# AlphacatPlus/VmambaIR

Measured on AMD Instinct MI355X. Metric: images/sec, x4 SR 64->256 training step (fwd+bwd+Adam+EMA), full VmambaIR UNet, higher is better.
Workload: dtype bf16; 1 GPU; BASELINE.json configs[1]: x4 SR 64x64 LQ, MambaSISR6 dim48 [15,1,1,1]+15, bf16 autocast (scan arithmetic f32), batch 8 per GPU; global_batch=8, per_gpu_batch=8, parallelism=dp1, step_launch=hipGraph replay, vendor_conv_solver_search=True, vendor_conv_solver_records=bench_data/miopen, optimizer=Adam 2e-4 (0.9,0.99) + EMA 0.999, loss=L1, rccl_ranks=1, allreduce_overlapped=False, allreduce_buckets=1, allreduce_bytes=0

## Files before the change

include/vmambair_oss.h:

```cpp
#ifndef VMAMBAIR_OSS_H
#define VMAMBAIR_OSS_H

#include <stddef.h>
#include <stdint.h>

#ifdef __cplusplus
extern "C" {
#endif

#define OSS_OK 0
#define OSS_ERR_NULL (-1)
#define OSS_ERR_SHAPE (-2)
#define OSS_ERR_DSTATE (-3)
#define OSS_ERR_WORKSPACE (-4)

#define OSS_MAX_DSTATE 256

typedef enum {
    OSS_F32 = 0, OSS_F16 = 1, OSS_BF16 = 2,
    OSS_F32_BF16X3 = 3
} oss_dtype;

typedef void *oss_stream_t;

// ... 36 lines not shown
    float *dD;
    float *ddelta_bias;
    void *workspace;
    size_t workspace_bytes;
    int dout_row_mod;
    int reserved_;
    int64_t dBC_group_stride;
    void *ddt;
    float *ddt_weight;
    int64_t ddt_batch_stride, ddt_group_stride, ddt_rank_stride;
    int tune_variant, tune_segments;
    int tune_partials, reserved3_;
    const float *finish_dt_weight;
    int finish_dt_rank, reserved4_;
} oss_scan_bwd_params;

int oss_scan_chunk(void);
int oss_scan_num_chunks(int seqlen);

size_t oss_scan_fwd_workspace_bytes(int batch, int dim, int seqlen, int dstate, int n_groups);
size_t oss_scan_lane_state_floats(int batch, int dim, int seqlen, int dstate);
int oss_scan_fwd(const oss_scan_fwd_params *p, oss_dtype io, oss_stream_t stream);

size_t oss_scan_bwd_workspace_bytes(int batch, int dim, int seqlen, int dstate, int n_groups);
int oss_scan_bwd(const oss_scan_bwd_params *p, oss_dtype io, oss_stream_t stream);

int oss_scan_bwd_finish_dt_ok(int seqlen, int dt_rank);

int oss_scan_fused_dt_ok(oss_dtype io, int batch, int D, int C, int R, int dstate, int seqlen);

void oss_scan_set_variant(int fwd_variant, int bwd_variant);
int oss_scan_last_variant(int which );
void oss_scan_set_segments(int fwd_segments, int bwd_segments);
int oss_scan_last_segments(int which );
void oss_scan_set_carry_split(int split);
int oss_scan_last_lane_states(void);

int oss_dwconv3x3_fwd(oss_dtype io, const void *x, const float *weight, const float *bias, void *y, void *pre_silu, int batch,
                      int channels, int height, int width, int64_t x_batch_stride, int64_t x_channel_stride,
                      int64_t y_batch_stride, int64_t y_channel_stride, int flip, oss_stream_t stream);
int oss_dwconv3x3_wgrad(oss_dtype io, const void *x, const void *dy, float *dweight, float *dbias, float *partials,
                        const void *pre_silu, void *dpre, int batch, int channels, int height, int width,
                        int64_t x_batch_stride, int64_t x_channel_stride, int64_t dy_batch_stride, int64_t dy_channel_stride,
                        oss_stream_t stream);

int oss_dwconv3x3_fused_ok(oss_dtype io, int height, int width, int channels_per_workgroup);
int oss_dwconv3x3_silu_fwd(oss_dtype io, const void *x, const float *weight, const float *bias, void *y, int batch, int channels,
                           int height, int width, int64_t x_batch_stride, int64_t x_channel_stride, int64_t y_batch_stride,
                           int64_t y_channel_stride, oss_stream_t stream);
int oss_dwconv3x3_silu_bwd(oss_dtype io, const void *x, const float *weight, const float *bias, const void *dy, void *dx,
                           float *dweight, float *dbias, float *partials, int batch, int channels, int height, int width,
                           int64_t x_batch_stride, int64_t x_channel_stride, int64_t dy_batch_stride, int64_t dy_channel_stride,
                           int64_t dx_batch_stride, int64_t dx_channel_stride, oss_stream_t stream);
int oss_dwgate_fwd_ok(oss_dtype io, int height, int width);

int oss_effn_fwd_ok(oss_dtype io, int channels, int hidden, int height, int width);
int oss_effn_round_weights(oss_dtype io, const float *project_in, const float *dwconv, const float *project_out, void *w_in, float *w_dw,
                           void *w_out, int channels, int hidden, oss_stream_t stream);
int oss_effn_fwd(oss_dtype io, const void *x, const float *norm_weight, const float *norm_bias, const void *w_in, const float *w_dw,
                 const void *w_out, void *out, int batch, int channels, int hidden, int height, int width, int64_t x_batch_stride,
                 int64_t x_channel_stride, int64_t out_batch_stride, int64_t out_channel_stride, float eps, oss_stream_t stream);
int oss_dwgate_fwd(oss_dtype io, const void *t, const float *weight, const float *bias, void *out, int batch, int hidden,
                   int height, int width, int64_t t_batch_stride, int64_t t_channel_stride, int64_t out_batch_stride,
                   int64_t out_channel_stride, oss_stream_t stream);
int oss_dwgate_bwd(oss_dtype io, const void *t, const float *weight, const float *bias, const void *dout, void *dt,
                   float *dweight, float *dbias, float *partials, int batch, int hidden, int height, int width,
                   int64_t t_batch_stride, int64_t t_channel_stride, int64_t dout_batch_stride, int64_t dout_channel_stride,
                   int64_t dt_batch_stride, int64_t dt_channel_stride, oss_stream_t stream);

int oss_dwconv3x3_flat2_ok(oss_dtype io, int height, int width);
int oss_dwconv3x3_silu_flat2_fwd(oss_dtype io, const void *x, const float *weight, const float *bias, void *x2, int batch, int channels,
                                 int height, int width, int64_t x_batch_stride, int64_t x_channel_stride, oss_stream_t stream);
int oss_dwconv3x3_silu_flat2_bwd(oss_dtype io, const void *x, const float *weight, const float *bias, const void *g2, void *dx,
                                 float *dweight, float *dbias, float *partials, int batch, int channels, int height, int width,
                                 int64_t x_batch_stride, int64_t x_channel_stride, int64_t dx_batch_stride, int64_t dx_channel_stride,
                                 oss_stream_t stream);

int oss_conv1x1_fwd(oss_dtype io, const void *x, const float *weight, const float *bias, const void *residual, void *y,
                    int batch, int cout, int cin, int pixels, int64_t x_batch_stride, int64_t x_channel_stride,
                    oss_stream_t stream);
int oss_conv1x1_dgrad(oss_dtype io, const void *dy, const float *weight, void *dx, int batch, int cout, int cin, int pixels,
                      int64_t dy_batch_stride, int64_t dy_channel_stride, oss_stream_t stream);
size_t oss_conv1x1_wgrad_partial_floats(int batch, int cout, int cin, int pixels);
int oss_conv1x1_wg(oss_dtype io, const void *x, const float *weight, const float *bias, void *y, int batch, int cout, int cin,
                   int pixels, int64_t x_batch_stride, int64_t x_channel_stride, int transposed_weight, oss_stream_t stream);
int oss_ln_conv1x1_ok(oss_dtype io, int cout, int cin, int pixels);
int oss_ln_conv1x1_fwd(oss_dtype io, const void *x, const float *ln_weight, const float *ln_bias, float eps, void *n, float *mean,
                       float *rstd, const float *weight, const float *bias, void *y, int batch, int cout, int cin, int pixels,
                       int64_t x_batch_stride, int64_t x_channel_stride, oss_stream_t stream);
int oss_conv1x1_dgrad_ln_bwd_ok(oss_dtype io, int cout, int cin, int pixels, int batch);
size_t oss_conv1x1_dgrad_ln_bwd_partial_floats(int batch, int cin, int pixels);
int oss_conv1x1_dgrad_ln_bwd(oss_dtype io, const void *dy, const float *weight, const void *x, const float *ln_weight, int ln_has_bias,
                             const float *mean, const float *rstd, const void *skip_grad, void *dx, float *dln_weight, float *dln_bias,
                             float *partials, int batch, int cout, int cin, int pixels, int64_t dy_batch_stride,
                             int64_t dy_channel_stride, oss_stream_t stream);
void oss_conv1x1_set_wg(int on, int pixels);
void oss_conv1x1_wgrad_set_tile(int mode);
void oss_conv1x1_wgrad_set_span(int mult);
int oss_conv1x1_wgrad(oss_dtype io, const void *dy, const void *x, float *dweight, float *dbias, float *partials, int batch,
                      int cout, int cin, int pixels, int64_t dy_batch_stride, int64_t dy_channel_stride,
                      int64_t x_batch_stride, int64_t x_channel_stride, oss_stream_t stream);

int oss_cross_scan2(oss_dtype in_type, oss_dtype out_type, const void *x, void *x2, int batch, int D, int height, int width,
                    int64_t x_batch_stride, int64_t x_channel_stride, oss_stream_t stream);
int oss_cross_merge2(oss_dtype io, const void *g2, void *dx, int batch, int D, int height, int width, oss_stream_t stream);
int oss_proj_fwd(oss_dtype io, const void *x2, const float *x_proj_weight, const float *dt_projs_weight, void *xdbl, void *dts,
                 int batch, int D, int C, int R, int seqlen, oss_stream_t stream);
int oss_proj_dgrad(oss_dtype io, const void *ddts, void *dxdbl, const void *du, const float *x_proj_weight,
                   const float *dt_projs_weight, void *dx2, int batch, int D, int C, int R, int seqlen, oss_stream_t stream);
size_t oss_proj_wgrad_partial_floats(int batch, int D, int C, int R, int seqlen);
void oss_proj_set_path(int force_vector_alu);
int oss_proj_rows_optional_ok(oss_dtype io, int batch, int D, int C, int R, int seqlen);
int oss_proj_wgrad(oss_dtype io, const void *x2, const void *xdbl, const void *dxdbl, const void *ddts, float *dx_proj_weight,
                   float *ddt_projs_weight, float *partials, int batch, int D, int C, int R, int seqlen, oss_stream_t stream);

typedef struct {
    int B, L, dc, Rc, Cc, reserved_;
    const float *pooled;
    const float *cin_w, *cin_b;
    const float *Wxc;
    const float *Wdtc;
    const float *dt_bias;
    const float *A_logs;
    const float *Dsc;
    const float *cout_w, *cout_b;
    const float *cn_w, *cn_b;
    float *zt;
    float *dts;
    float *hs;
    float *y;
    float *yc;
    float *stat;
    float *c;
    const float *pool_part;
    int n_part;
    float pool_scale;
} oss_chan_params;
int oss_chan_fwd(const oss_chan_params *p, oss_stream_t stream);
size_t oss_chan_grad_floats(int L, int dc, int Rc, int Cc);
size_t oss_chan_bwd_scratch_floats(int B, int L, int dc, int Rc, int Cc);
int oss_chan_bwd(const oss_chan_params *p, const float *gc, float *dpooled, float *grads, float *scratch, oss_stream_t stream);
int oss_rowsum(oss_dtype io, const void *a, const void *bmul, float *out, int batch, int channels, int pixels,
               int64_t a_batch_stride, int64_t a_channel_stride, int64_t b_batch_stride, int64_t b_channel_stride, float alpha,
               oss_stream_t stream);
int oss_row_affine(oss_dtype io, const void *x, const float *mul, const float *add, void *y, int batch, int channels,
                   int pixels, int64_t x_batch_stride, int64_t x_channel_stride, float alpha, oss_stream_t stream);

int oss_gelu_gate_fwd(oss_dtype io, const void *h, void *out, int batch, size_t half_elems, int64_t h_batch_stride,
                      oss_stream_t stream);
int oss_gelu_gate_bwd(oss_dtype io, const void *h, const void *dout, void *dh, int batch, size_t half_elems,
                      int64_t h_batch_stride, int64_t dout_batch_stride, oss_stream_t stream);

typedef struct {
    const void *src;
    void *dst;
    int64_t stride;
    int j0, n, K, reserved_;
} oss_sum_chunk;
void oss_set_defer_finish(int on);
size_t oss_deferred_chunks(void);
int oss_flush_finishes(void *host_table, void *device_table, size_t capacity_chunks, oss_stream_t stream);
int oss_flush_finishes_n(void *host_table, void *device_table, size_t capacity_chunks, size_t max_chunks, oss_stream_t stream);

void oss_set_defer_wgrad(int on);
size_t oss_deferred_wgrads(void);
size_t oss_deferred_wgrad_table_bytes(void);
// ... 25 lines not shown
                         const void *gate, void *y, float *mean, float *rstd, float *pool_part, int batch, int channels, int pixels,
                         int64_t x_batch_stride, int64_t x_channel_stride, int64_t gate_batch_stride,
                         int64_t gate_channel_stride, float eps, oss_stream_t stream);
int oss_ln_nchw_bwd(oss_dtype x_type, oss_dtype y_type, const void *x, const float *weight, const float *bias,
                    const void *gate, const void *dy, const float *mean, const float *rstd, void *dx, void *dgate,
                    float *dweight, float *dbias, float *partials, const void *skip_grad, int batch, int channels, int pixels,
                    int64_t x_batch_stride, int64_t x_channel_stride, int64_t gate_batch_stride,
                    int64_t gate_channel_stride, int64_t dgate_batch_stride, oss_stream_t stream);
int oss_ln_nchw_bwd_affine(oss_dtype x_type, oss_dtype y_type, const void *x, const float *weight, const float *bias,
                           const void *gate, const void *dy, const float *dy_mul, const float *dy_add, float add_scale,
                           const float *mean, const float *rstd, void *dx, void *dgate, float *dweight, float *dbias, float *partials,
                           const void *skip_grad, int batch, int channels, int pixels, int64_t x_batch_stride,
                           int64_t x_channel_stride, int64_t gate_batch_stride, int64_t gate_channel_stride,
                           int64_t dgate_batch_stride, oss_stream_t stream);

void oss_prof_enable(int on);
void oss_prof_reset(void);
int oss_prof_collect(int which, int variant, oss_dtype io, double *total_ms, long long *launches,
                     double *algorithmic_bytes);
int oss_prof_collect2(int which, int variant, oss_dtype io, double *total_ms, long long *launches, double *algorithmic_bytes,
                      double *own_bytes);

int oss_hbm_copy(const void *src, void *dst, size_t n_bytes, oss_stream_t stream);

int oss_prof_marker(int which, oss_stream_t stream);

const char *oss_scan_build_id(void);

const char *oss_version(void);

int oss_conv3x3_thin_ok(oss_dtype io, int cin, int cout, int height, int width);
int oss_conv3x3_thin_fwd(oss_dtype io, const void *x, const float *weight, const float *bias, void *y, int batch, int cin, int cout,
                         int height, int width, int64_t x_batch_stride, int64_t x_channel_stride, int64_t y_batch_stride,
                         int64_t y_channel_stride, oss_stream_t stream);
int oss_conv3x3_thin_dgrad(oss_dtype io, const void *dy, const float *weight, void *dx, int batch, int cin, int cout, int height,
                           int width, int64_t dy_batch_stride, int64_t dy_channel_stride, int64_t dx_batch_stride,
                           int64_t dx_channel_stride, oss_stream_t stream);
size_t oss_conv3x3_thin_wgrad_partial_floats(int batch, int cin, int cout);
int oss_conv3x3_thin_wgrad(oss_dtype io, const void *x, const void *dy, float *dweight, float *dbias, float *partial, int batch, int cin,
                           int cout, int height, int width, int64_t x_batch_stride, int64_t x_channel_stride, int64_t dy_batch_stride,
                           int64_t dy_channel_stride, oss_stream_t stream);

int oss_conv3x3_dense_ok(oss_dtype io, int cin, int cout, int height, int width);
int oss_conv3x3_dense_fwd(oss_dtype io, const void *x, const float *weight, const float *bias, void *y, int batch, int cin, int cout,
                          int height, int width, int64_t x_batch_stride, int64_t x_channel_stride, int64_t y_batch_stride,
                          int64_t y_channel_stride, oss_stream_t stream);
int oss_conv3x3_dense_dgrad(oss_dtype io, const void *dy, const float *weight, void *dx, int batch, int cin, int cout, int height,
                            int width, int64_t dy_batch_stride, int64_t dy_channel_stride, int64_t dx_batch_stride,
                            int64_t dx_channel_stride, oss_stream_t stream);
size_t oss_conv3x3_dense_wgrad_partial_floats(int batch, int cin, int cout, int height, int width);
int oss_conv3x3_dense_wgrad(oss_dtype io, const void *x, const void *dy, float *dweight, float *dbias, float *partial, int batch, int cin,
                            int cout, int height, int width, int64_t x_batch_stride, int64_t x_channel_stride, int64_t dy_batch_stride,
                            int64_t dy_channel_stride, oss_stream_t stream);

#define OSS_METRIC_QUANTISE 1
#define OSS_METRIC_Y 2
#define OSS_METRIC_REPLICATE 4
int oss_image_metrics_ok(oss_dtype io, int channels, int height, int width, int crop_border, int flags);
size_t oss_image_metrics_partial_doubles(int batch, int channels, int height, int width, int crop_border);
int oss_image_metrics(oss_dtype io, const void *a, const void *b, double *out, double *partials, int batch, int channels,
                      int height, int width, int64_t a_batch_stride, int64_t a_channel_stride, int64_t a_row_stride,
                      int64_t b_batch_stride, int64_t b_channel_stride, int64_t b_row_stride, int crop_border, int flags,
                      oss_stream_t stream);

#define OSS_PAIRS_HFLIP 1
#define OSS_PAIRS_ROT 2
int oss_pairs_philox(const uint32_t *counter, const uint32_t *key, uint32_t *out);
int oss_pairs_ok(int channels, int scale, int patch_h, int patch_w, int batch);
int oss_pairs_draw(const int64_t *table, int n_pairs, int64_t *counter, int *samples, int batch, int patch, int64_t seed, int rank,
                   int world, int flags, oss_stream_t stream);
int oss_pairs_gather(const void *pool, int64_t pool_bytes, const int64_t *table, int n_pairs, const int *samples, float *lq, float *gt,
                     int *clamped, int batch, int channels, int patch_h, int patch_w, int scale, int swap_rb, oss_stream_t stream);

void oss_prof_family_enable(int on);
int oss_prof_family_count(void);
int oss_prof_family(int family, const char **name, const char **kernel_patterns, double *algorithmic_bytes, long long *calls);

#define OSS_FEATURE_FUSED_DT 1
#define OSS_FEATURE_LANE_STATES 2
int oss_scan_features(void);

int oss_f32_matmul_modes(void);

#define OSS_ABI_VERSION 8
int oss_abi_version(void);
size_t oss_abi_struct_bytes(int which);

#ifdef __cplusplus
}
#endif
#endif
```

vmambair_amd/csrc/oss_capi.hip:

```cpp
#include <atomic>
#include <mutex>
#include <vector>
#include <cstring>
#include <algorithm>
#include "oss_device.h"
#include "oss_host.h"

namespace oss {

static std::atomic<int> g_force_fwd{-1}, g_force_bwd{-1};
static std::atomic<int> g_last_fwd{-1}, g_last_bwd{-1};
static std::atomic<int> g_force_fwd_seg{-1}, g_force_bwd_seg{-1};
std::atomic<int> g_last_fwd_segments{1}, g_last_bwd_segments{1}, g_last_bwd_lane_states{0};

int scan_pick_segments(long wgs, int n_chunks, int seg_req, double ovh) {
    if (seg_req == 0 || seg_req == 1 || n_chunks < 2 || wgs <= 0) return 1;
    if (seg_req > 1) return std::min(std::min(seg_req, n_chunks), kMaxSegments);
    if (wgs >= 256) return 1;
    int best = 1;
    double best_cost = (double)n_chunks;
    for (int s = 2; s <= std::min(n_chunks, 16); ++s) {
        const int cps = (n_chunks + s - 1) / s;
        if ((n_chunks + cps - 1) / cps != s) continue;
        const double rounds = (double)((wgs * s + 255) / 256);
// ... 39 lines not shown
static std::vector<unsigned char> g_wgrad_descs;
static std::vector<unsigned> g_wgrad_blocks;
bool defer_wgrad() { return g_defer_wgrad.load() != 0; }
void defer_wgrad_push(const void *desc, size_t bytes, unsigned blocks) {
    std::lock_guard<std::mutex> lk(g_defer_mu);
    const unsigned char *p = reinterpret_cast<const unsigned char *>(desc);
    g_wgrad_descs.insert(g_wgrad_descs.end(), p, p + bytes);
    g_wgrad_blocks.push_back(blocks);
}

int scan_fwd_pick_variant(int batch, int dim, int seqlen, int dstate, int n_groups, int elem_bytes) {
    (void)dstate; (void)elem_bytes;
    const int rows_per_group = dim / n_groups;
    const long rows = (long)batch * dim;
    if (seqlen <= 256 || rows_per_group < 8) return (rows_per_group >= 16 && rows >= 4096) ? 2 : 4;
    if (rows_per_group % 16 == 0 && rows / 4 >= 2048) return 2;
    if (rows_per_group % 16 == 0 && rows / 2 >= 2048) return 1;
    if (seqlen >= 4096 && rows_per_group % 12 == 0 && (long)batch * n_groups * (rows_per_group / 12) <= 128) return 6;
    if (seqlen >= 1024 && (long)batch * n_groups * ((rows_per_group + 7) / 8) <= 256) return 3;
    if (seqlen >= 1024 && rows_per_group >= 12 && (long)batch * n_groups * ((rows_per_group + 11) / 12) <= 256) return 6;
    return 0;
}

int scan_bwd_pick_variant(int batch, int dim, int seqlen, int dstate, int n_groups) {
    const int rows_per_group = dim / n_groups;
    if (seqlen <= 256 || rows_per_group < 8 || dstate > 64) return 1;
    const long wgs = (long)batch * n_groups * ((rows_per_group + 7) / 8);
    if (seqlen >= 2048 && rows_per_group % 12 == 0 && (long)batch * n_groups * (rows_per_group / 12) < 192) return 10;
    if (wgs <= 128 && rows_per_group % 4 == 0) return 13;
    if (wgs <= 256) return 11;
    return rows_per_group >= 12 ? 10 : 11;
}

constexpr int kProfVariants = 32;
struct ProfBucket {
    std::vector<std::pair<hipEvent_t, hipEvent_t>> pending;
    double ms = 0.0, bytes = 0.0, own = 0.0;
    long long launches = 0;
};
static std::mutex g_prof_mu;
static std::atomic<int> g_prof_on{0};
static ProfBucket g_prof[3][kProfVariants][3];
static std::vector<hipEvent_t> g_event_pool;

static hipEvent_t prof_event() {
    if (!g_event_pool.empty()) { hipEvent_t e = g_event_pool.back(); g_event_pool.pop_back(); return e; }
    hipEvent_t e; (void)hipEventCreate(&e); return e;
}

struct ProfTimer : LaunchTimer {
    bool on; int which, variant, io; double bytes, own; hipEvent_t e0{}, e1{};
    ProfTimer(int which_, int variant_, int io_, double bytes_, double own_ = 0.0)
        : on(g_prof_on.load() != 0 && variant_ >= 0 && variant_ < 16), which(which_), variant(variant_),
          io(io_), bytes(bytes_), own(own_) {}
    void segmented() override { if (variant < 16) variant += 16; }
    void begin(hipStream_t s) override {
        if (!on) return;
        {
            std::lock_guard<std::mutex> lk(g_prof_mu);
            e0 = prof_event(); e1 = prof_event();
        }
        (void)hipEventRecord(e0, s);
    }
    void end(hipStream_t s) override {
        if (!on) return;
        (void)hipEventRecord(e1, s);
        std::lock_guard<std::mutex> lk(g_prof_mu);
        ProfBucket &b = g_prof[which][variant][io];
        b.pending.emplace_back(e0, e1);
        b.bytes += bytes;
        b.own += own;
        b.launches += 1;
    }
};


enum Fam { FAM_CONV1X1 = 0, FAM_WGRAD, FAM_DWCONV, FAM_PROJ, FAM_LN, FAM_CHAN, FAM_MERGE, FAM_GATE, FAM_CONV3X3, FAM_FINISH, FAM_OPTIM, FAM_N };
static const char *const kFamName[FAM_N] = {"conv1x1 forward / input gradient (+ fused LayerNorm)", "1x1 / projection weight gradients",
                                            "depth-wise 3x3 (+ silu / gelu gate / flattenings)", "x_proj / dt_proj forward + input gradient",
                                            "LayerNorm (+ silu gate, pooled sums)", "channel branch (+ rowsum / row_affine)",
                                            "cross-scan / cross-merge / merge4", "gelu gate (unfused)", "thin 3x3 convolutions",
                                            "deferred partial-sum finishing", "Adam(W) + EMA"};
static const char *const kFamKernels[FAM_N] = {"oss_conv1x1_pair_kernel|oss_conv1x1_pairk_kernel|oss_conv1x1_pairw_kernel|oss_conv1x1_wg_kernel|"
                                               "oss_conv1x1_dgrad_lnbwd_kernel|oss_conv1x1_f32_kernel",
                                               "oss_conv1x1_wgrad|oss_rows_f32_wgrad|oss_proj_wgrad",
                                               "oss_dwconv3x3|oss_dwgate|oss_effn",
                                               "oss_proj_fwd|oss_proj_dgrad|oss_dt_fwd|oss_dt_dgrad|oss_proj_valu",
                                               "oss_ln_nchw",
                                               "oss_chan_|oss_rowsum|oss_row_affine",
                                               "oss_merge4|oss_cross_scan2|oss_cross_merge2",
                                               "oss_gelu_gate",
                                               "oss_conv3x3_",
                                               "oss_sum_partials",
                                               "oss_adam"};
static std::atomic<int> g_fam_on{0};
static double g_fam_bytes[FAM_N];
static long long g_fam_calls[FAM_N];
static inline bool is_f32_split(oss_dtype io) { return io == OSS_F32_BF16X3; }
static inline int take_f32_split(oss_dtype &io) {
    if (!is_f32_split(io)) return 0;
    io = OSS_F32;
    return 1;
}
static inline void fam_count(int fam, double bytes) {
    if (!g_fam_on.load(std::memory_order_relaxed)) return;
    std::lock_guard<std::mutex> lk(g_prof_mu);
    g_fam_bytes[fam] += bytes;
    g_fam_calls[fam] += 1;
}

static double fwd_alg_bytes(const oss_scan_fwd_params &p, int s) {
    const double BKL = (double)p.batch * p.dim * p.seqlen, BGNL = (double)p.batch * p.n_groups * p.dstate * p.seqlen;
    const double xb = 4.0 * p.batch * p.dim * oss_scan_num_chunks(p.seqlen) * 2 * p.dstate;
    return s * (3.0 * BKL + 2.0 * BGNL) + 4.0 * ((double)p.dim * p.dstate + 2.0 * p.dim) + xb;
}
static double bwd_alg_bytes(const oss_scan_fwd_params &p, int s) {
    const double BKL = (double)p.batch * p.dim * p.seqlen, BGNL = (double)p.batch * p.n_groups * p.dstate * p.seqlen;
    const double xb = 4.0 * p.batch * p.dim * oss_scan_num_chunks(p.seqlen) * 2 * p.dstate;
    return s * (5.0 * BKL + 4.0 * BGNL) + 4.0 * (2.0 * p.dim * p.dstate + 4.0 * p.dim) + xb;
}

static double fwd_own_bytes(const oss_scan_fwd_params &p, int s) {
    const double full = fwd_alg_bytes(p, s);
    if (p.u_row_mod <= 0) return full;
    return full - (double)s * p.batch * (p.dim - p.u_row_mod) * p.seqlen;
}
static double bwd_own_bytes(const oss_scan_bwd_params &q, int s) {
    const oss_scan_fwd_params &p = q.f;
    double v = bwd_alg_bytes(p, s);
    if (p.u_row_mod > 0) v -= (double)s * p.batch * (p.dim - p.u_row_mod) * p.seqlen;
    if (q.dout_row_mod > 0) v -= (double)s * p.batch * (p.dim - q.dout_row_mod) * p.seqlen;
    return v;
}

static int check_fwd(const oss_scan_fwd_params *p) {
    if (!p || !p->u || !p->delta || !p->A || !p->B || !p->C) return OSS_ERR_NULL;
    if (p->dt_weight && (p->dt_rank < 1 || p->dt_rank > kMaxDtRank)) return OSS_ERR_SHAPE;
    if (p->batch < 0 || p->dim <= 0 || p->seqlen < 0 || p->dstate <= 0 || p->n_groups <= 0) return OSS_ERR_SHAPE;
    if (p->dim % p->n_groups != 0) return OSS_ERR_SHAPE;
    if (p->dstate > OSS_MAX_DSTATE) return OSS_ERR_DSTATE;
    if (p->rev_group_start < 0 || p->u_row_mod < 0 || (p->u_row_mod > 0 && p->dim % p->u_row_mod != 0)) return OSS_ERR_SHAPE;
    return OSS_OK;
}

}

using namespace oss;

extern "C" {

int oss_scan_chunk(void) { return kScanChunk; }
int oss_scan_num_chunks(int seqlen) { return seqlen <= 0 ? 0 : (seqlen + kScanChunk - 1) / kScanChunk; }

int oss_scan_fwd(const oss_scan_fwd_params *p, oss_dtype io, oss_stream_t stream) {
    const int eb = io_bytes(io);
    if (!eb) return OSS_ERR_SHAPE;
    int rc = check_fwd(p);
    if (rc != OSS_OK) return rc;
    if (!p->out || !p->x) return OSS_ERR_NULL;
    if (p->batch == 0 || p->seqlen == 0) return OSS_OK;
    int v = p->tune_variant > 0 ? p->tune_variant - 1 : g_force_fwd.load();
    if (v < 0) v = scan_fwd_pick_variant(p->batch, p->dim, p->seqlen, p->dstate, p->n_groups, eb);
    g_last_fwd.store(v);
    g_last_fwd_segments.store(1);
    const int sr = p->tune_segments > 0 ? p->tune_segments : g_force_fwd_seg.load();
    hipStream_t s = reinterpret_cast<hipStream_t>(stream);
    ProfTimer prof(0, v, (int)io, fwd_alg_bytes(*p, eb), fwd_own_bytes(*p, eb));
// ... 114 lines not shown
    fam_count(FAM_DWCONV, (double)batch * channels * height * width * io_bytes(io) * 4.0 + 80.0 * channels);
    if (!x || !weight || !g2 || !dx || !dweight || !partials) return OSS_ERR_NULL;
    if (batch <= 0 || channels <= 0 || height <= 0 || width <= 0 || channels > 65535 || batch > 65535) return OSS_ERR_SHAPE;
    return dwconv3x3_silu_flat2_bwd(io, x, weight, bias, g2, dx, dweight, dbias, partials, batch, channels, height, width, xsb, xsc, dsb,
                                    dsc, reinterpret_cast<hipStream_t>(stream));
}

int oss_effn_fwd_ok(oss_dtype io, int channels, int hidden, int height, int width) {
    return effn_fwd_ok(io, channels, hidden, height, width);
}

int oss_effn_round_weights(oss_dtype io, const float *project_in, const float *dwconv, const float *project_out, void *w_in, float *w_dw,
                           void *w_out, int channels, int hidden, oss_stream_t stream) {
    if (is_f32_split(io)) return OSS_ERR_SHAPE;
    if (!project_in || !dwconv || !project_out || !w_in || !w_dw || !w_out) return OSS_ERR_NULL;
    return effn_round_weights(io, project_in, dwconv, project_out, w_in, w_dw, w_out, channels, hidden, reinterpret_cast<hipStream_t>(stream));
}

int oss_effn_fwd(oss_dtype io, const void *x, const float *norm_weight, const float *norm_bias, const void *w_in, const float *w_dw,
                 const void *w_out, void *out, int batch, int channels, int hidden, int height, int width, int64_t xsb, int64_t xsc,
                 int64_t osb, int64_t osc, float eps, oss_stream_t stream) {
    if (is_f32_split(io)) return OSS_ERR_SHAPE;
    fam_count(FAM_DWCONV, (double)batch * channels * height * width * io_bytes(io) * 3.0 + (double)hidden * (3.0 * channels * io_bytes(io) + 72.0));
    if (!x || !norm_weight || !w_in || !w_dw || !w_out || !out) return OSS_ERR_NULL;
    if (batch <= 0 || channels <= 0 || hidden <= 0 || height <= 0 || width <= 0) return OSS_ERR_SHAPE;
    return effn_fwd(io, x, norm_weight, norm_bias, w_in, w_dw, w_out, out, batch, channels, hidden, height, width, xsb, xsc, osb, osc, eps,
                    reinterpret_cast<hipStream_t>(stream));
}

int oss_dwgate_fwd_ok(oss_dtype io, int height, int width) {
    return dwgate_fwd_ok(io, height, width);
}

int oss_dwgate_fwd(oss_dtype io, const void *t, const float *weight, const float *bias, void *out, int batch, int hidden,
                   int height, int width, int64_t tsb, int64_t tsc, int64_t osb, int64_t osc, oss_stream_t stream) {
    if (is_f32_split(io)) return OSS_ERR_SHAPE;
    fam_count(FAM_DWCONV, (double)batch * hidden * height * width * io_bytes(io) * 3.0 + 80.0 * hidden);
    if (!t || !weight || !out) return OSS_ERR_NULL;
    if (batch <= 0 || hidden <= 0 || height <= 0 || width <= 0 || hidden > 32767 || batch > 65535) return OSS_ERR_SHAPE;
    return dwgate_fwd(io, t, weight, bias, out, batch, hidden, height, width, tsb, tsc, osb, osc, reinterpret_cast<hipStream_t>(stream));
}

int oss_dwgate_bwd(oss_dtype io, const void *t, const float *weight, const float *bias, const void *dout, void *dt,
                   float *dweight, float *dbias, float *partials, int batch, int hidden, int height, int width, int64_t tsb,
                   int64_t tsc, int64_t gsb, int64_t gsc, int64_t dsb, int64_t dsc, oss_stream_t stream) {
    if (is_f32_split(io)) return OSS_ERR_SHAPE;
    fam_count(FAM_DWCONV, (double)batch * hidden * height * width * io_bytes(io) * 5.0 + 160.0 * hidden);
    if (!t || !weight || !dout || !dt || !dweight || !partials) return OSS_ERR_NULL;
    if (batch <= 0 || hidden <= 0 || height <= 0 || width <= 0 || hidden > 32767 || batch > 65535) return OSS_ERR_SHAPE;
    return dwconv3x3_bwd_fused(io, 1, t, weight, bias, dout, dt, dweight, dbias, partials, batch, 2 * hidden, height, width, tsb,
                               tsc, gsb, gsc, dsb, dsc, reinterpret_cast<hipStream_t>(stream));
}

int oss_dwconv3x3_wgrad(oss_dtype io, const void *x, const void *dy, float *dweight, float *dbias, float *partials,
                        const void *pre_silu, void *dpre, int batch, int channels, int height, int width, int64_t xsb,
                        int64_t xsc, int64_t gsb, int64_t gsc, oss_stream_t stream) {
    if (is_f32_split(io)) return OSS_ERR_SHAPE;
    fam_count(FAM_DWCONV, (double)batch * channels * height * width * io_bytes(io) * (pre_silu ? 4.0 : 2.0));
    if (!x || !dy || !dweight || !partials) return OSS_ERR_NULL;
    if (batch <= 0 || channels <= 0 || height <= 0 || width <= 0 || batch > 65535) return OSS_ERR_SHAPE;
    return dwconv3x3_wgrad(io, x, dy, dweight, dbias, partials, batch, channels, height, width, xsb, xsc, gsb, gsc,
                           reinterpret_cast<hipStream_t>(stream), pre_silu, dpre);
}

int oss_conv1x1_fwd(oss_dtype io, const void *x, const float *weight, const float *bias, const void *residual, void *y,
                    int batch, int cout, int cin, int pixels, int64_t xsb, int64_t xsc, oss_stream_t stream) {
    const int x3 = take_f32_split(io);
    fam_count(FAM_CONV1X1, (double)batch * pixels * io_bytes(io) * ((double)cin + cout + (residual ? cout : 0)) + 4.0 * cin * cout);
    if (!x || !weight || !y) return OSS_ERR_NULL;
    if (batch <= 0 || cout <= 0 || cin <= 0 || pixels <= 0 || batch > 65535 || cout > 32 * 65535) return OSS_ERR_SHAPE;
    return conv1x1(io, x, weight, bias, y, batch, cout, cin, pixels, xsb, xsc, cin, 1, reinterpret_cast<hipStream_t>(stream),
                   residual, x3);
}

int oss_conv1x1_dgrad(oss_dtype io, const void *dy, const float *weight, void *dx, int batch, int cout, int cin, int pixels,
                      int64_t gsb, int64_t gsc, oss_stream_t stream) {
    const int x3 = take_f32_split(io);
    fam_count(FAM_CONV1X1, (double)batch * pixels * io_bytes(io) * ((double)cin + cout) + 4.0 * cin * cout);
    if (!dy || !weight || !dx) return OSS_ERR_NULL;
    if (batch <= 0 || cout <= 0 || cin <= 0 || pixels <= 0 || batch > 65535) return OSS_ERR_SHAPE;
    return conv1x1(io, dy, weight, nullptr, dx, batch, cin, cout, pixels, gsb, gsc, 1, cin, reinterpret_cast<hipStream_t>(stream), nullptr, x3);
}

size_t oss_conv1x1_wgrad_partial_floats(int batch, int cout, int cin, int pixels) {
    if (batch <= 0 || cout <= 0 || cin <= 0 || pixels <= 0) return 0;
    return (size_t)batch * conv1x1_wgrad_slabs(pixels) * cout * (cin + 1);
}

int oss_conv1x1_wgrad(oss_dtype io, const void *dy, const void *x, float *dweight, float *dbias, float *partials, int batch,
                      int cout, int cin, int pixels, int64_t gsb, int64_t gsc, int64_t xsb, int64_t xsc, oss_stream_t stream) {
    const int x3 = take_f32_split(io);
    fam_count(FAM_WGRAD, (double)batch * pixels * io_bytes(io) * ((double)cin + cout) + 4.0 * cin * cout);
    if (!dy || !x || !dweight || !partials) return OSS_ERR_NULL;
    if (batch <= 0 || cout <= 0 || cin <= 0 || pixels <= 0 || batch > 65535) return OSS_ERR_SHAPE;
    return conv1x1_wgrad(io, dy, x, dweight, partials, batch, cout, cin, pixels, gsb, gsc, xsb, xsc,
                         reinterpret_cast<hipStream_t>(stream), 1, 0, 0, 0, 0, dbias, x3);
}

size_t oss_proj_wgrad_partial_floats(int batch, int D, int C, int R, int seqlen) {
    if (batch <= 0 || D <= 0 || C <= 0 || R <= 0 || seqlen <= 0) return 0;
    const size_t slabs = (size_t)batch * conv1x1_wgrad_slabs(seqlen);
    const size_t a = slabs * 2 * (2 * (size_t)C) * D, b = slabs * 4 * (size_t)D * R;
    return a + b;
}

int oss_proj_fwd(oss_dtype io, const void *x2, const float *x_proj_weight, const float *dt_projs_weight, void *xdbl, void *dts,
                 int batch, int D, int C, int R, int seqlen, oss_stream_t stream) {
    const int x3 = take_f32_split(io);
    fam_count(FAM_PROJ, (double)batch * seqlen * io_bytes(io) * (2.0 * D + 4.0 * C + (dts ? 4.0 * R + 4.0 * D : 0.0)) + 16.0 * C * D + 16.0 * D * R);
    if (!x2 || !x_proj_weight || !dt_projs_weight || !xdbl) return OSS_ERR_NULL;
    if (batch <= 0 || D <= 0 || seqlen <= 0 || R <= 0 || C <= R) return OSS_ERR_SHAPE;
    return proj_fwd(io, x2, x_proj_weight, dt_projs_weight, xdbl, dts, batch, D, C, R, seqlen, reinterpret_cast<hipStream_t>(stream), x3);
}

int oss_proj_dgrad(oss_dtype io, const void *ddts, void *dxdbl, const void *du, const float *x_proj_weight,
                   const float *dt_projs_weight, void *dx2, int batch, int D, int C, int R, int seqlen, oss_stream_t stream) {
    const int x3 = take_f32_split(io);
    fam_count(FAM_PROJ, (double)batch * seqlen * io_bytes(io) * ((ddts ? 4.0 * D + 4.0 * R : 0.0) + 4.0 * C + (du ? 4.0 * D : 0.0) + 2.0 * D) + 16.0 * C * D);
    if (!dxdbl || !x_proj_weight || !dt_projs_weight || !dx2) return OSS_ERR_NULL;
    if (batch <= 0 || D <= 0 || seqlen <= 0 || R <= 0 || C <= R) return OSS_ERR_SHAPE;
    return proj_dgrad(io, ddts, dxdbl, du, x_proj_weight, dt_projs_weight, dx2, batch, D, C, R, seqlen,
                      reinterpret_cast<hipStream_t>(stream), x3);
}

void oss_proj_set_path(int force_vector_alu) { proj_force_valu(force_vector_alu); }
int oss_proj_rows_optional_ok(oss_dtype io, int batch, int D, int C, int R, int seqlen) {
    return proj_mfma_ok(io, batch, D, C, R, seqlen) ? 1 : 0;
}
int oss_scan_fused_dt_ok(oss_dtype io, int batch, int D, int C, int R, int dstate, int seqlen) {
    return proj_mfma_ok(io, batch, D, C, R, seqlen) && R >= 1 && R <= kMaxDtRank && dstate <= 64 && seqlen >= 512;
}
int oss_conv1x1_wg(oss_dtype io, const void *x, const float *weight, const float *bias, void *y, int batch, int cout, int cin,
                   int pixels, int64_t xsb, int64_t xsc, int transposed_weight, oss_stream_t stream) {
    if (is_f32_split(io)) return OSS_ERR_SHAPE;
    fam_count(FAM_CONV1X1, (double)batch * pixels * io_bytes(io) * ((double)cin + cout) + 4.0 * cin * cout);
    if (!x || !weight || !y) return OSS_ERR_NULL;
    if (batch <= 0 || batch > 65535) return OSS_ERR_SHAPE;
    return conv1x1_wg(io, x, weight, bias, y, batch, cout, cin, pixels, xsb, xsc, transposed_weight, reinterpret_cast<hipStream_t>(stream));
}

int oss_ln_conv1x1_ok(oss_dtype io, int cout, int cin, int pixels) {
    const void *a = reinterpret_cast<const void *>(uintptr_t(256));
    return conv1x1_wg_ok(io, cout, cin, pixels, (int64_t)cin * pixels, pixels, a, a, reinterpret_cast<const float *>(a), nullptr);
}

int oss_ln_conv1x1_fwd(oss_dtype io, const void *x, const float *ln_weight, const float *ln_bias, float eps, void *n, float *mean,
                       float *rstd, const float *weight, const float *bias, void *y, int batch, int cout, int cin, int pixels,
                       int64_t xsb, int64_t xsc, oss_stream_t stream) {
    if (is_f32_split(io)) return OSS_ERR_SHAPE;
    fam_count(FAM_CONV1X1, (double)batch * pixels * (io_bytes(io) * (2.0 * cin + cout) + 8.0) + 4.0 * cin * cout);
    if (!x || !ln_weight || !n || !mean || !rstd || !weight || !y) return OSS_ERR_NULL;
    if (batch <= 0 || batch > 65535) return OSS_ERR_SHAPE;
    return ln_conv1x1_wg(io, x, ln_weight, ln_bias, eps, n, mean, rstd, weight, bias, y, batch, cout, cin, pixels, xsb, xsc,
                         reinterpret_cast<hipStream_t>(stream));
}

int oss_conv1x1_dgrad_ln_bwd_ok(oss_dtype io, int cout, int cin, int pixels, int batch) {
    return conv1x1_dgrad_lnbwd_ok(io, cin, cout, pixels, batch);
}
size_t oss_conv1x1_dgrad_ln_bwd_partial_floats(int batch, int cin, int pixels) {
    if (batch <= 0 || cin <= 0 || pixels <= 0) return 0;
    return conv1x1_dgrad_lnbwd_partial_floats(batch, cin, pixels);
}
int oss_conv1x1_dgrad_ln_bwd(oss_dtype io, const void *dy, const float *weight, const void *x, const float *ln_weight, int ln_has_bias,
                             const float *mean, const float *rstd, const void *skip_grad, void *dx, float *dln_weight, float *dln_bias,
                             float *partials, int batch, int cout, int cin, int pixels, int64_t gsb, int64_t gsc, oss_stream_t stream) {
    if (is_f32_split(io)) return OSS_ERR_SHAPE;
    fam_count(FAM_CONV1X1, (double)batch * pixels * (io_bytes(io) * ((double)cout + 2.0 * cin + (skip_grad ? cin : 0)) + 8.0) + 4.0 * cin * cout);
    if (!dy || !weight || !x || !ln_weight || !mean || !rstd || !dx || !dln_weight || !partials) return OSS_ERR_NULL;
    if (batch <= 0 || batch > 65535) return OSS_ERR_SHAPE;
    return conv1x1_dgrad_lnbwd(io, dy, weight, x, ln_weight, ln_has_bias, mean, rstd, skip_grad, dx, dln_weight, dln_bias, partials, batch,
                               cin, cout, pixels, gsb, gsc, reinterpret_cast<hipStream_t>(stream));
}

void oss_conv1x1_set_wg(int on, int pixels) { conv1x1_set_wg(on); conv1x1_wg_set_pixels(pixels); }
void oss_conv1x1_wgrad_set_tile(int mode) { conv1x1_wgrad_set_tile(mode); }
void oss_conv1x1_wgrad_set_span(int mult) { conv1x1_wgrad_set_span(mult); }

int oss_proj_wgrad(oss_dtype io, const void *x2, const void *xdbl, const void *dxdbl, const void *ddts, float *dx_proj_weight,
                   float *ddt_projs_weight, float *partials, int batch, int D, int C, int R, int seqlen, oss_stream_t stream) {
    const int x3 = take_f32_split(io);
    fam_count(FAM_WGRAD, (double)batch * seqlen * io_bytes(io) * (2.0 * D + 8.0 * C + (ddts ? 4.0 * D : 0.0)));
    if (!x2 || !xdbl || !dxdbl || !dx_proj_weight || !partials) return OSS_ERR_NULL;
    if (ddts && !ddt_projs_weight) return OSS_ERR_NULL;
    if (batch <= 0 || D <= 0 || seqlen <= 0 || R <= 0 || C <= R) return OSS_ERR_SHAPE;
    hipStream_t s = reinterpret_cast<hipStream_t>(stream);
    const int64_t L = seqlen;
    if (io == OSS_F32) {
        int e = rows_f32_wgrad(reinterpret_cast<const float *>(dxdbl), reinterpret_cast<const float *>(x2), dx_proj_weight, partials, batch,
                               4, 2, C, D, seqlen, 4 * C * L, C * L, L, 2 * D * L, D * L, L, s, nullptr, x3);
        if (e || !ddts) return e;
        float *part2 = partials + (size_t)batch * conv1x1_wgrad_slabs(seqlen) * 2 * (2 * (size_t)C) * D;
        return rows_f32_wgrad(reinterpret_cast<const float *>(ddts), reinterpret_cast<const float *>(xdbl), ddt_projs_weight, part2, batch, 4,
                              4, D, R, seqlen, 4 * D * L, D * L, L, 4 * C * L, C * L, L, s, nullptr, x3);
    }
    int e = conv1x1_wgrad(io, dxdbl, x2, dx_proj_weight, partials, batch, 2 * C, D, seqlen, 4 * C * L, L, 2 * D * L, L, s,
                           2,  C * L,  D * L,  C,  2 * C * L);
    if (e || !ddts) return e;
    float *part2 = partials + (size_t)batch * conv1x1_wgrad_slabs(seqlen) * 2 * (2 * (size_t)C) * D;
    return conv1x1_wgrad(io, ddts, xdbl, ddt_projs_weight, part2, batch, D, R, seqlen, 4 * D * L, L, 4 * C * L, L, s,
                          4,  D * L,  C * L,  D, 0);
}

int oss_cross_scan2(oss_dtype in_type, oss_dtype out_type, const void *x, void *x2, int batch, int D, int height, int width,
                    int64_t x_batch_stride, int64_t x_channel_stride, oss_stream_t stream) {
    if (is_f32_split(in_type) || is_f32_split(out_type)) return OSS_ERR_SHAPE;
    fam_count(FAM_MERGE, (double)batch * D * height * width * (io_bytes(in_type) + 2.0 * io_bytes(out_type)));
    if (!x || !x2) return OSS_ERR_NULL;
    if (batch <= 0 || D <= 0 || height <= 0 || width <= 0) return OSS_ERR_SHAPE;
    return cross_scan2(in_type, out_type, x, x2, batch, D, height, width, x_batch_stride, x_channel_stride,
                       reinterpret_cast<hipStream_t>(stream));
}

int oss_cross_merge2(oss_dtype io, const void *g2, void *dx, int batch, int D, int height, int width, oss_stream_t stream) {
    if (is_f32_split(io)) return OSS_ERR_SHAPE;
    fam_count(FAM_MERGE, (double)batch * D * height * width * io_bytes(io) * 3.0);
    if (!g2 || !dx) return OSS_ERR_NULL;
    if (batch <= 0 || D <= 0 || height <= 0 || width <= 0) return OSS_ERR_SHAPE;
    return cross_merge2(io, g2, dx, batch, D, height, width, reinterpret_cast<hipStream_t>(stream));
}

int oss_chan_fwd(const oss_chan_params *p, oss_stream_t stream) {
    fam_count(FAM_CHAN, p ? 4.0 * p->B * ((double)p->L * (2.0 * p->Cc + 2.0 * p->dc * 18.0 + 3.0) + (p->pool_part ? (double)p->n_part * p->L : p->L)) : 0.0);
    if (!p) return OSS_ERR_NULL;
    return chan_fwd(*p, reinterpret_cast<hipStream_t>(stream));
}

size_t oss_chan_grad_floats(int L, int dc, int Rc, int Cc) { return chan_grad_floats(L, dc, Rc, Cc); }
size_t oss_chan_bwd_scratch_floats(int B, int L, int dc, int Rc, int Cc) { return chan_bwd_scratch_floats(B, L, dc, Rc, Cc); }

int oss_chan_bwd(const oss_chan_params *p, const float *gc, float *dpooled, float *grads, float *scratch, oss_stream_t stream) {
    fam_count(FAM_CHAN, p ? 4.0 * p->B * ((double)p->L * (2.0 * p->Cc + 2.0 * p->dc * 18.0 + 5.0)) : 0.0);
    if (!p) return OSS_ERR_NULL;
    return chan_bwd(*p, gc, dpooled, grads, scratch, reinterpret_cast<hipStream_t>(stream));
}

int oss_rowsum(oss_dtype io, const void *a, const void *bmul, float *out, int batch, int channels, int pixels, int64_t asb,
// ... 393 lines not shown
```

vmambair_amd/csrc/oss_conv1x1.hip:

```cpp
#include <atomic>
#include "oss_device.h"
#include "oss_global_ptr.h"
#include "oss_host.h"
#include "oss_mfma.h"

namespace oss {

template <typename T>
__global__ void __launch_bounds__(256)
oss_conv1x1_kernel(const T *__restrict__ x, const float *__restrict__ w, const float *__restrict__ bias, T *__restrict__ y,
                   int M, int K, int P, int64_t xsb, int64_t xsk, int64_t ws_m, int64_t ws_k, const T *__restrict__ res) {
    const int lane = threadIdx.x & 63, wave = threadIdx.x >> 6;
    const int b = blockIdx.y;
    const int m0 = blockIdx.z * 32;
    const int p0 = (blockIdx.x * 4 + wave) * 32;
    if (p0 >= P) return;
    const int col = lane & 31, kg = lane >> 5;
    const int p = p0 + col;
    const bool pok = p < P;
    const T *xb = x + b * xsb + (pok ? p : 0);
    T *yb = y + (size_t)b * M * P;
    const int mrow = m0 + col;
    const bool mok = mrow < M;
    const float *wrow = w + (mok ? mrow : 0) * ws_m;
// ... 172 lines not shown
        if (row < M && pok) yw[(size_t)row * psw] = pack2<T>(va, vb);
    }
}

template <int KS>
struct WRaw { f32x4 lo[KS], hi[KS]; };

template <int KS, bool WT, bool WVEC>
__device__ __forceinline__ void wraw_issue(WRaw<KS> &r, const float *__restrict__ w, int mrow, int M, int K, int kg) {
    const int mc = mrow < M ? mrow : 0;
#pragma unroll
    for (int ks = 0; ks < KS; ++ks) {
        const int k0 = ks * 16 + kg * 8;
        if constexpr (!WT && WVEC) {
            const float *wp = w + mc * K + (k0 + 8 <= K ? k0 : 0);
            r.lo[ks] = *reinterpret_cast<const f32x4 *>(wp);
            r.hi[ks] = *reinterpret_cast<const f32x4 *>(wp + 4);
        } else {
#pragma unroll
            for (int e = 0; e < 8; ++e) {
                const int k = k0 + e, kc = k < K ? k : K - 1;
                const float v = WT ? w[kc * M + mc] : w[mc * K + kc];
                if (e < 4) r.lo[ks][e] = v; else r.hi[ks][e - 4] = v;
            }
        }
    }
}

template <typename T, int KS, bool WT, bool WVEC>
__device__ __forceinline__ void wraw_narrow(const WRaw<KS> &r, s16x8 (&af)[KS], int mrow, int M, int K, int kg) {
    const bool mok = mrow < M;
#pragma unroll
    for (int ks = 0; ks < KS; ++ks) {
        const int k0 = ks * 16 + kg * 8;
        if constexpr (!WT && WVEC) {
            const s16x8 f = cvt8<T>(r.lo[ks], r.hi[ks]);
            af[ks] = (mok && k0 + 8 <= K) ? f : s16x8{0, 0, 0, 0, 0, 0, 0, 0};
        } else {
            f32x4 lo = r.lo[ks], hi = r.hi[ks];
#pragma unroll
            for (int e = 0; e < 4; ++e) {
                lo[e] = (mok && k0 + e < K) ? lo[e] : 0.f;
                hi[e] = (mok && k0 + 4 + e < K) ? hi[e] : 0.f;
            }
            af[ks] = cvt8<T>(lo, hi);
        }
    }
}

template <int KS>
__device__ __forceinline__ void wflat_issue(WRaw<KS> &r, const float *__restrict__ w, int m0, int M, int K, int lane) {
    const int lim = min(M - m0, 32) * K - 4;
    const float *base = w + (size_t)m0 * K;
#pragma unroll
    for (int i = 0; i < 2 * KS; ++i) {
        const f32x4 q = *reinterpret_cast<const f32x4 *>(base + min(256 * i + 4 * lane, lim));
        if (i < KS) r.lo[i] = q; else r.hi[i - KS] = q;
    }
}
template <typename T, int KS>
__device__ __forceinline__ void wflat_frags(const WRaw<KS> &r, T *__restrict__ myl, s16x8 (&af)[KS], int m0, int M, int K,
                                            int col, int kg, int row0, int k0, int sr, int sk) {
    constexpr int RS = 16 * KS + 8;
    const int nl = K >> 3;
    int rr = row0, kk = k0;
#pragma unroll
    for (int i = 0; i < 2 * KS; ++i) {
        const f32x4 q = i < KS ? r.lo[i] : r.hi[i < KS ? 0 : i - KS];
        if (i < nl) *reinterpret_cast<u32x2 *>(myl + rr * RS + kk) = u32x2{pack2<T>(q.x, q.y), pack2<T>(q.z, q.w)};
        kk += sk;
        rr += sr;
        if (kk >= K) { kk -= K; ++rr; }
    }
    __builtin_amdgcn_wave_barrier();
    const bool mok = m0 + col < M;
#pragma unroll
    for (int ks = 0; ks < KS; ++ks) {
        const u32x4 f = *reinterpret_cast<const u32x4 *>(myl + col * RS + ks * 16 + kg * 8);
        af[ks] = (mok && ks * 16 + kg * 8 + 8 <= K) ? __builtin_bit_cast(s16x8, f) : s16x8{0, 0, 0, 0, 0, 0, 0, 0};
    }
    __builtin_amdgcn_wave_barrier();
}

template <typename T, int KS, bool WT, bool WVEC, bool RES, bool PF>
__global__ void __launch_bounds__(256)
oss_conv1x1_pair_kernel(const T *__restrict__ x, const float *__restrict__ w, const float *__restrict__ bias,
                        T *__restrict__ y, int M, int K, int P, int64_t xsb, int xsk, int mt_per_wave, const T *__restrict__ res) {
    const int lane = threadIdx.x & 63, wave = threadIdx.x >> 6;
    const int b = blockIdx.y;
    const int p0 = (blockIdx.x * 4 + wave) * 64;
    if (p0 >= P) return;
    const int col = lane & 31, kg = lane >> 5;
    const int p = p0 + 2 * col;
    const bool pok = p < P;
    const int pc = pok ? p : 0;
    const uint32_t *xw = reinterpret_cast<const uint32_t *>(x + b * xsb + pc);
    const int xsw = xsk >> 1;
    const int psw = P >> 1;
    uint32_t *yw = reinterpret_cast<uint32_t *>(y + (size_t)b * M * P + pc);
    const uint32_t *rp = RES ? reinterpret_cast<const uint32_t *>(res + (size_t)b * M * P + pc) : nullptr;
    const float *bp = bias ? bias : w;
    const int ksteps = (K + 15) >> 4;
    const int mt_total = (M + 31) >> 5;
    const int mt_begin = blockIdx.z * mt_per_wave, mt_end = min(mt_total, mt_begin + mt_per_wave);
    if (mt_begin >= mt_end) return;

    constexpr bool WLDS = !WT && WVEC;
    __shared__ __attribute__((aligned(16))) T wlds[WLDS ? 4 * 32 * (16 * KS + 8) : 8];
    T *myl = wlds + (WLDS ? wave * 32 * (16 * KS + 8) : 0);
    const int wf_row0 = WLDS ? (4 * lane) / K : 0, wf_k0 = WLDS ? (4 * lane) % K : 0, wf_sr = WLDS ? 256 / K : 0, wf_sk = WLDS ? 256 % K : 0;
    WRaw<KS> wr;
    float bl;
    uint32_t rw[16];
    auto issue = [&](int mt) {
        const int m0 = mt * 32;
        if constexpr (WLDS) wflat_issue<KS>(wr, w, m0, M, K, lane);
        else                wraw_issue<KS, WT, WVEC>(wr, w, m0 + col, M, K, kg);
        bl = bp[min(m0 + col, M - 1)];
        if constexpr (RES) {
#pragma unroll
            for (int r = 0; r < 16; ++r) rw[r] = rp[(size_t)min(m0 + (r & 3) + 8 * (r >> 2) + 4 * kg, M - 1) * psw];
        }
    };
    issue(mt_begin);

    s16x8 bfa[KS], bfb[KS];
#pragma unroll
    for (int ks = 0; ks < KS; ++ks) {
#pragma unroll
        for (int e = 0; e < 8; ++e) {
            const int k = ks * 16 + kg * 8 + e;
            const bool kok = k < K;
            const uint32_t raw = xw[(kok ? k : K - 1) * xsw];
            const uint32_t v = (pok && kok) ? raw : 0u;
            bfa[ks][e] = (short)(v & 0xffffu);
            bfb[ks][e] = (short)(v >> 16);
        }
    }

    for (int mt = mt_begin; mt < mt_end; ++mt) {
        const int m0 = mt * 32;
        s16x8 af[KS];
        if constexpr (WLDS) wflat_frags<T, KS>(wr, myl, af, m0, M, K, col, kg, wf_row0, wf_k0, wf_sr, wf_sk);
        else                wraw_narrow<T, KS, WT, WVEC>(wr, af, m0 + col, M, K, kg);
        const float bcur = bias ? bl : 0.f;
        uint32_t rcur[16];
        if constexpr (RES) {
#pragma unroll
            for (int r = 0; r < 16; ++r) rcur[r] = rw[r];
        }
        if constexpr (PF) issue(min(mt + 1, mt_total - 1));
        f32x16 acca, accb;
#pragma unroll
        for (int r = 0; r < 16; ++r) { acca[r] = 0.f; accb[r] = 0.f; }
#pragma unroll
        for (int ks = 0; ks < KS; ++ks) {
            if (ks < ksteps) {
                acca = Mfma<T>::run(af[ks], bfa[ks], acca);
                accb = Mfma<T>::run(af[ks], bfb[ks], accb);
            }
        }
#pragma unroll
        for (int r = 0; r < 16; ++r) {
            const int rin = (r & 3) + 8 * (r >> 2) + 4 * kg, row = m0 + rin;
            const float bv = __int_as_float(__builtin_amdgcn_ds_bpermute(rin << 2, __float_as_int(bcur)));
            float va = acca[r] + bv, vb = accb[r] + bv;
            if constexpr (RES) {
                float r0, r1;
                unpack2<T>(rcur[r], r0, r1);
                va += r0;
                vb += r1;
            }
            if (row < M && pok) yw[(size_t)row * psw] = pack2<T>(va, vb);
        }
        if constexpr (!PF) {
            if (mt + 1 < mt_end) issue(mt + 1);
        }
    }
}

template <typename T>
__global__ void __launch_bounds__(256)
oss_conv1x1_pairw_kernel(const T *__restrict__ x, const float *__restrict__ w, const float *__restrict__ bias,
                         T *__restrict__ y, int M, int K, int P, int64_t xsb, int xsk, const T *__restrict__ res) {
    constexpr int KS = 8, CH = KS * 16, KMAX = 512, NI = 32 * KMAX / 4 / 256;
    __shared__ __attribute__((aligned(16))) T wl[32 * (KMAX + 8)];
    const int tid = threadIdx.x, lane = tid & 63, wave = tid >> 6;
    const int b = blockIdx.y;
    const int p0 = (blockIdx.x * 4 + wave) * 64;
    const bool active = p0 < P;
    const int col = lane & 31, kg = lane >> 5;
    const int p = p0 + 2 * col;
    const bool pok = active && p < P;
    const uint32_t *xw = reinterpret_cast<const uint32_t *>(x + b * xsb + (pok ? p : 0));
    const int xsw = xsk >> 1;
    const int m0 = blockIdx.z * 32;
    const int RS = ((K + 7) & ~7) + 8;

    auto load_x = [&](int kc, s16x8 (&fa)[KS], s16x8 (&fb)[KS]) {
#pragma unroll
        for (int ks = 0; ks < KS; ++ks) {
#pragma unroll
            for (int e = 0; e < 8; ++e) {
                const int k = kc + ks * 16 + kg * 8 + e;
                const bool kok = k < K;
                const uint32_t raw = xw[(kok ? k : K - 1) * xsw];
                const uint32_t v = (pok && kok) ? raw : 0u;
                fa[ks][e] = (short)(v & 0xffffu);
                fb[ks][e] = (short)(v >> 16);
            }
        }
    };
    s16x8 fa[KS], fb[KS];
    load_x(0, fa, fb);

    const int have = min(M - m0, 32) * K, total = 32 * K, lim = max(have - 4, 0);
    const float *base = w + (size_t)m0 * K;
    f32x4 q[NI];
#pragma unroll
    for (int i = 0; i < NI; ++i) q[i] = *reinterpret_cast<const f32x4 *>(base + min(4 * (i * 256 + tid), lim));
    int r = (4 * tid) / K, k = (4 * tid) - r * K;
    const int sr = 1024 / K, sk = 1024 - sr * K;
#pragma unroll
    for (int i = 0; i < NI; ++i) {
        const int off = 4 * (i * 256 + tid);
        if (off < total) {
            const int d = max(off - lim, 0);
            float v4[4] = {q[i][0], q[i][1], q[i][2], q[i][3]};
            if (d == 1) { v4[0] = v4[1]; v4[1] = v4[2]; v4[2] = v4[3]; }
            else if (d == 2) { v4[0] = v4[2]; v4[1] = v4[3]; }
            else if (d >= 3) { v4[0] = v4[3]; }
            int rr = r, kk = k;
#pragma unroll
            for (int e = 0; e < 4; ++e) {
                if (rr < 32 && off + e < have) wl[rr * RS + kk] = from_f32<T>(v4[e]);
                if (++kk == K) { kk = 0; ++rr; }
            }
        }
        k += sk;
        r += sr;
        if (k >= K) { k -= K; ++r; }
    }
    __syncthreads();
    if (!active) return;

    f32x16 acca, accb;
#pragma unroll
    for (int r = 0; r < 16; ++r) { acca[r] = 0.f; accb[r] = 0.f; }
    const bool mok = m0 + col < M;
    for (int kc = 0; kc < K; kc += CH) {
        if (kc) load_x(kc, fa, fb);
        s16x8 af[KS];
#pragma unroll
        for (int ks = 0; ks < KS; ++ks) {
            const int k0 = kc + ks * 16 + kg * 8;
            const u32x4 f = *reinterpret_cast<const u32x4 *>(wl + col * RS + min(k0, RS - 8));
            s16x8 v = __builtin_bit_cast(s16x8, f);
#pragma unroll
            for (int e = 0; e < 8; ++e) v[e] = (mok && k0 + e < K) ? v[e] : (short)0;
            af[ks] = v;
        }
#pragma unroll
        for (int ks = 0; ks < KS; ++ks) {
            if (kc + ks * 16 < K) {
                acca = Mfma<T>::run(af[ks], fa[ks], acca);
                accb = Mfma<T>::run(af[ks], fb[ks], accb);
            }
        }
    }
    T *yb = y + (size_t)b * M * P;
    pair_epilogue<T>(acca, accb, bias, res ? res + (size_t)b * M * P + (pok ? p : 0) : nullptr, yb + p, m0, kg, M, P, pok);
}

template <typename T, int KS, int MT, bool WT, bool WVEC>
__global__ void __launch_bounds__(256)
oss_conv1x1_pairk_kernel(const T *__restrict__ x, const float *__restrict__ w, const float *__restrict__ bias,
                        T *__restrict__ y, int M, int K, int P, int64_t xsb, int xsk, const T *__restrict__ res) {
    const int lane = threadIdx.x & 63, wave = threadIdx.x >> 6;
    const int b = blockIdx.y;
    const int p0 = (blockIdx.x * 4 + wave) * 64;
    if (p0 >= P) return;
    const int col = lane & 31, kg = lane >> 5;
    const int p = p0 + 2 * col;
    const bool pok = p < P;
    const uint32_t *xw = reinterpret_cast<const uint32_t *>(x + b * xsb + (pok ? p : 0));
    const int xsw = xsk >> 1;
    T *yb = y + (size_t)b * M * P;
    const int mt0 = blockIdx.z * MT;
    f32x16 acca[MT], accb[MT];
#pragma unroll
    for (int t = 0; t < MT; ++t)
#pragma unroll
        for (int r = 0; r < 16; ++r) { acca[t][r] = 0.f; accb[t][r] = 0.f; }

    for (int kc = 0; kc < K; kc += KS * 16) {
        s16x8 bfa[KS], bfb[KS];
#pragma unroll
        for (int ks = 0; ks < KS; ++ks) {
#pragma unroll
            for (int e = 0; e < 8; ++e) {
                const int k = kc + ks * 16 + kg * 8 + e;
                const bool kok = k < K;
                const uint32_t raw = xw[(kok ? k : K - 1) * xsw];
                const uint32_t v = (pok && kok) ? raw : 0u;
                bfa[ks][e] = (short)(v & 0xffffu);
                bfb[ks][e] = (short)(v >> 16);
            }
        }
#pragma unroll
        for (int t = 0; t < MT; ++t) {
            s16x8 af[KS];
#pragma unroll
            for (int ks = 0; ks < KS; ++ks) af[ks] = load_wfrag<T, WT, WVEC>(w, (mt0 + t) * 32 + col, M, K, kc + ks * 16 + kg * 8);
            if ((mt0 + t) * 32 < M) {
#pragma unroll
                for (int ks = 0; ks < KS; ++ks) {
                    if (kc + ks * 16 < K) {
                        acca[t] = Mfma<T>::run(af[ks], bfa[ks], acca[t]);
                        accb[t] = Mfma<T>::run(af[ks], bfb[ks], accb[t]);
                    }
                }
            }
        }
    }
#pragma unroll
    for (int t = 0; t < MT; ++t)
        pair_epilogue<T>(acca[t], accb[t], bias, res ? res + (size_t)b * M * P + (pok ? p : 0) : nullptr, yb + p, (mt0 + t) * 32, kg, M, P, pok);
}

constexpr int kWgradSlab = 512;
template <typename T>
__device__ __forceinline__ void
wgrad_body(const T *__restrict__ dy, const T *__restrict__ x, float *__restrict__ part, int M, int N, int P,
           int64_t gsb, int64_t gsm, int64_t xsb, int64_t xsn, int G, int64_t gsg, int64_t xsg, int Mh,
           int64_t gs_hi, int NB ,
           int slab, int nslabs, int by, int bz, int span ) {
    const int lane = threadIdx.x & 63, wave = threadIdx.x >> 6;
    const int b = by / G, g = by - b * G;
    const int pbeg = slab * span, pend = min(P, pbeg + span);
    const int col = lane & 31, kg = lane >> 5;
    const int mt = (M + 31) >> 5, nt = (NB + 31) >> 5;
    const T *gb = dy + b * gsb + g * gsg;
    const T *xb = x + b * xsb + g * xsg;
    const size_t pvec = (size_t)G * M * N + (NB > N ? M : 0);
    float *pb = part + (size_t)(b * nslabs + slab) * pvec;
    const short kOne = (short)from_f32<T>(1.0f).v;
    const s16x8 zero8 = {0, 0, 0, 0, 0, 0, 0, 0}, ones8 = {kOne, kOne, kOne, kOne, kOne, kOne, kOne, kOne};
    const bool aligned = (((reinterpret_cast<uintptr_t>(gb) | reinterpret_cast<uintptr_t>(xb)) & 15u) == 0) &&
                         (gsm % 8 == 0) && (xsn % 8 == 0) && (pbeg % 8 == 0) && (gs_hi % 8 == 0);
    {
        const int tile = bz * 4 + wave;
        if (tile >= mt * nt) return;
        const int m0 = (tile / nt) * 32, n0 = (tile % nt) * 32;
        const int mrow = m0 + col, nrow = n0 + col;
        const bool mok = mrow < M, nok = nrow < N, one = nrow == N && NB > N;
        const int mr = mok ? mrow : 0;
        const T *ga = gb + (mr / Mh) * gs_hi + (mr % Mh) * gsm;
        const T *xa = xb + (nok ? nrow : 0) * xsn;
        f32x16 acc;
#pragma unroll
        for (int r = 0; r < 16; ++r) acc[r] = 0.f;

        int pk = pbeg;
        for (; aligned && pend - pk >= kWgradSlab; pk += kWgradSlab) {
            constexpr int PIECES = kWgradSlab / 64, RS = 72;
            __shared__ __attribute__((aligned(16))) T stage[4][2][32 * RS];
            T *sa = stage[wave][0], *sb = stage[wave][1];
            const int r8 = lane >> 3, q = lane & 7;
            const T *pa[4], *px[4];
#pragma unroll
            for (int j = 0; j < 4; ++j) {
                const int mr2 = min(m0 + r8 + 8 * j, M - 1), nr2 = min(n0 + r8 + 8 * j, N - 1);
                pa[j] = gb + (mr2 / Mh) * gs_hi + (mr2 % Mh) * gsm + pk + q * 8;
                px[j] = xb + nr2 * xsn + pk + q * 8;
            }
            constexpr int WIN = PIECES < 4 ? PIECES : 4;
            u32x4 qa[WIN][4], qb[WIN][4];
#pragma unroll
            for (int pc = 0; pc < WIN; ++pc)
#pragma unroll
                for (int j = 0; j < 4; ++j) {
                    qa[pc][j] = *reinterpret_cast<const u32x4 *>(pa[j] + pc * 64);
                    qb[pc][j] = *reinterpret_cast<const u32x4 *>(px[j] + pc * 64);
                }
#pragma unroll
            for (int pc = 0; pc < PIECES; ++pc) {
#pragma unroll
                for (int j = 0; j < 4; ++j) {
                    *reinterpret_cast<u32x4 *>(sa + (r8 + 8 * j) * RS + q * 8) = qa[pc % WIN][j];
                    *reinterpret_cast<u32x4 *>(sb + (r8 + 8 * j) * RS + q * 8) = qb[pc % WIN][j];
                }
                if (pc + WIN < PIECES) {
#pragma unroll
                    for (int j = 0; j < 4; ++j) {
                        qa[pc % WIN][j] = *reinterpret_cast<const u32x4 *>(pa[j] + (pc + WIN) * 64);
                        qb[pc % WIN][j] = *reinterpret_cast<const u32x4 *>(px[j] + (pc + WIN) * 64);
// ... 49 lines not shown
                    af[e] = (mok && kok) ? av : (short)0;
                    bf[e] = kok ? (nok ? bv : (one ? kOne : (short)0)) : (short)0;
                }
            }
            acc = Mfma<T>::run(af, bf, acc);
        }
#pragma unroll
        for (int r = 0; r < 16; ++r) {
            const int row = m0 + (r & 3) + 8 * (r >> 2) + 4 * kg;
            const int cn = n0 + col;
            if (row < M && cn < NB) {
                const size_t drow = ((size_t)(row / Mh) * G + g) * Mh + row % Mh;
                if (cn < N) pb[drow * N + cn] = acc[r];
                else pb[(size_t)G * M * N + row] = acc[r];
            }
        }
    }
}

template <typename T>
__global__ void __launch_bounds__(256)
oss_conv1x1_wgrad_kernel(const T *__restrict__ dy, const T *__restrict__ x, float *__restrict__ part, int M, int N, int P,
                         int64_t gsb, int64_t gsm, int64_t xsb, int64_t xsn, int G, int64_t gsg, int64_t xsg, int Mh,
                         int64_t gs_hi, int NB) {
    wgrad_body<T>(dy, x, part, M, N, P, gsb, gsm, xsb, xsn, G, gsg, xsg, Mh, gs_hi, NB, (int)blockIdx.x, (int)gridDim.x, (int)blockIdx.y,
                  (int)blockIdx.z, kWgradSlab);
}

struct WgradDesc {
    const void *dy, *x;
    float *part;
    int64_t gsb, gsm, xsb, xsn, gsg, xsg, gs_hi;
    int M, N, P, G, Mh, NB, slabs, bgs ;
    unsigned first_block;
    int io;
    int span, reserved_;
};
template <typename T>
__global__ void __launch_bounds__(256)
oss_conv1x1_wgrad_grouped_kernel(const WgradDesc *__restrict__ descs, const uint16_t *__restrict__ block_problem) {
    const WgradDesc d = descs[block_problem[blockIdx.x]];
    const unsigned local = blockIdx.x - d.first_block;
    const int slab = (int)(local % (unsigned)d.slabs);
    const unsigned r = local / (unsigned)d.slabs;
    const int by = (int)(r % (unsigned)d.bgs), bz = (int)(r / (unsigned)d.bgs);
    const WgradDesc *dt = descs + block_problem[blockIdx.x];
    wgrad_body<T>(table_ptr<const T>(&dt->dy), table_ptr<const T>(&dt->x), table_ptr<float>(&dt->part), d.M, d.N, d.P, d.gsb, d.gsm, d.xsb,
                  d.xsn, d.G, d.gsg, d.xsg, d.Mh, d.gs_hi, d.NB, slab, d.slabs, by, bz, d.span);
}

__global__ void __launch_bounds__(256)
oss_conv1x1_wgrad_finish(const float *__restrict__ part, float *__restrict__ dw, float *__restrict__ db, int nslab, size_t pvec,
                         size_t nw) {
    __shared__ float red[4][64];
    const int colx = threadIdx.x & 63, slice = threadIdx.x >> 6;
    const size_t i = (size_t)blockIdx.x * 64 + colx;
    float s = 0.f;
    if (i < pvec) {
        const float *pp = part + i;
        int k = slice;
        float s0 = 0.f, s1 = 0.f, s2 = 0.f, s3 = 0.f;
        for (; k + 12 < nslab; k += 16) {
            s0 += pp[(size_t)k * pvec];
            s1 += pp[(size_t)(k + 4) * pvec];
            s2 += pp[(size_t)(k + 8) * pvec];
            s3 += pp[(size_t)(k + 12) * pvec];
        }
        for (; k < nslab; k += 4) s0 += pp[(size_t)k * pvec];
        s = (s0 + s1) + (s2 + s3);
    }
    red[slice][colx] = s;
    __syncthreads();
    if (slice == 0 && i < pvec) {
        const float t = (red[0][colx] + red[1][colx]) + (red[2][colx] + red[3][colx]);
        if (i < nw) dw[i] = t;
        else db[i - nw] = t;
    }
}

constexpr long kConv1x1TargetWaves = 1024;

template <typename T>
static void conv1x1_launch(const T *x, const float *w, const float *bias, T *y, int B, int M, int K, int P, int64_t xsb,
                           int64_t xsk, int64_t ws_m, int64_t ws_k, hipStream_t s, const T *res) {
    const int pblocks = (P + 127) / 128, mt = (M + 31) / 32;
    const bool wt = (ws_m == 1 && ws_k == M);
    const bool plain = (ws_k == 1 && ws_m == K);
    const bool pair_ok = P % 2 == 0 && xsk % 2 == 0 && xsb % 2 == 0 && xsk < (1 << 24) && (size_t)M * K < (1u << 30) &&
                         (wt || plain) && ((reinterpret_cast<uintptr_t>(x) | reinterpret_cast<uintptr_t>(y)) & 3u) == 0;
    if (pair_ok) {
        const bool wvec = plain && K % 8 == 0 && (reinterpret_cast<uintptr_t>(w) & 15u) == 0;
        const int pb = (P + 255) / 256;
        const long waves_p = (long)B * ((P + 63) / 64);
        const int xk = (int)xsk;
        if (plain && !wvec && K > 16 * 3 && K <= 512 && (reinterpret_cast<uintptr_t>(w) & 15u) == 0) {
            hipLaunchKernelGGL(oss_conv1x1_pairw_kernel<T>, dim3(pb, B, mt), dim3(256), 0, s, x, w, bias, y, M, K, P, xsb, xk, res);
            return;
        }
        if (K <= 16 * 12) {
            int split = (int)((kConv1x1TargetWaves + waves_p - 1) / waves_p);
            if (split < 1) split = 1;
            if (split > mt) split = mt;
            const int per = (mt + split - 1) / split;
            dim3 grid(pb, B, (mt + per - 1) / per);
#define OSS_PAIR2(KS_, WT_, WV_, PF_) do { if (res) hipLaunchKernelGGL((oss_conv1x1_pair_kernel<T, KS_, WT_, WV_, true, PF_>), grid, dim3(256), 0, s, x, w, bias, y, M, K, P, xsb, xk, per, res); \
                                           else     hipLaunchKernelGGL((oss_conv1x1_pair_kernel<T, KS_, WT_, WV_, false, PF_>), grid, dim3(256), 0, s, x, w, bias, y, M, K, P, xsb, xk, per, res); } while (0)
#define OSS_PAIR(KS_, PF_) do { if (wt) OSS_PAIR2(KS_, true, false, PF_); else if (wvec) OSS_PAIR2(KS_, false, true, PF_); else OSS_PAIR2(KS_, false, false, PF_); } while (0)
            if (K <= 16 * 3)      OSS_PAIR(3, true);
            else if (K <= 16 * 6) OSS_PAIR(6, true);
            else if (K <= 16 * 8) OSS_PAIR(8, false);
            else                  OSS_PAIR(12, false);
#undef OSS_PAIR2
#undef OSS_PAIR
#undef OSS_PAIR1
        } else {
            int per = 3;
            while (per > 1 && waves_p * ((mt + per - 1) / per) < 4096) --per;
            if (per > mt) per = mt;
            if (per == 1 && K <= 512 && (reinterpret_cast<uintptr_t>(w) & 15u) == 0 && plain) {
                hipLaunchKernelGGL(oss_conv1x1_pairw_kernel<T>, dim3(pb, B, mt), dim3(256), 0, s, x, w, bias, y, M, K, P, xsb, xk, res);
                return;
            }
            dim3 grid(pb, B, (mt + per - 1) / per);
#define OSS_PAIR1(MT_, WT_, WV_) hipLaunchKernelGGL((oss_conv1x1_pairk_kernel<T, 8, MT_, WT_, WV_>), grid, dim3(256), 0, s, x, w, bias, y, M, K, P, xsb, xk, res)
#define OSS_PAIR(MT_) do { if (wt) OSS_PAIR1(MT_, true, false); else if (wvec) OSS_PAIR1(MT_, false, true); else OSS_PAIR1(MT_, false, false); } while (0)
            if (per == 1) OSS_PAIR(1); else if (per == 2) OSS_PAIR(2); else OSS_PAIR(3);
#undef OSS_PAIR
#undef OSS_PAIR1
        }
        return;
    }
    const bool reuse_ok = K <= 16 * 12 && xsk < (1 << 24) && (size_t)M * K < (1u << 30) &&
                          (wt || (plain && K % 8 == 0 && (reinterpret_cast<uintptr_t>(w) & 15u) == 0));
    if (reuse_ok) {
        const long waves_p = (long)B * ((P + 31) / 32);
        int split = (int)((2048 + waves_p - 1) / waves_p);
        if (split < 1) split = 1;
        if (split > mt) split = mt;
        const int per = (mt + split - 1) / split;
        dim3 grid(pblocks, B, (mt + per - 1) / per);
        const int xk = (int)xsk;
        if (K <= 16 * 6) {
            if (wt) hipLaunchKernelGGL((oss_conv1x1_reuse_kernel<T, 6, true>), grid, dim3(256), 0, s, x, w, bias, y, M, K, P, xsb, xk, per, res);
            else    hipLaunchKernelGGL((oss_conv1x1_reuse_kernel<T, 6, false>), grid, dim3(256), 0, s, x, w, bias, y, M, K, P, xsb, xk, per, res);
        } else {
            if (wt) hipLaunchKernelGGL((oss_conv1x1_reuse_kernel<T, 12, true>), grid, dim3(256), 0, s, x, w, bias, y, M, K, P, xsb, xk, per, res);
            else    hipLaunchKernelGGL((oss_conv1x1_reuse_kernel<T, 12, false>), grid, dim3(256), 0, s, x, w, bias, y, M, K, P, xsb, xk, per, res);
        }
    } else {
        dim3 grid(pblocks, B, mt);
        hipLaunchKernelGGL(oss_conv1x1_kernel<T>, grid, dim3(256), 0, s, x, w, bias, y, M, K, P, xsb, xsk, ws_m, ws_k, res);
    }
}

static std::atomic<int> g_conv_wg{1};

void conv1x1_set_wg(int on) { g_conv_wg.store(on ? 1 : 0); }

int conv1x1(oss_dtype io, const void *x, const float *w, const float *bias, void *y, int B, int M, int K, int P, int64_t xsb,
            int64_t xsk, int64_t ws_m, int64_t ws_k, hipStream_t s, const void *res, int f32_split) {
    {
        const bool wt = (ws_m == 1 && ws_k == M), plain = (ws_k == 1 && ws_m == K);
        if ((wt || plain) && g_conv_wg.load() != 0 && conv1x1_wg_ok(io, M, K, P, xsb, xsk, x, y, w, res))
            return conv1x1_wg(io, x, w, bias, y, B, M, K, P, xsb, xsk, wt ? 1 : 0, s, res);
    }
    return io_dispatch(io, [&](auto tag) {
        using T = typename decltype(tag)::type;
        const T *xp = reinterpret_cast<const T *>(x), *rp = reinterpret_cast<const T *>(res);
        T *yp = reinterpret_cast<T *>(y);
        if constexpr (sizeof(T) == 4) {
            return conv1x1_f32(xp, w, bias, yp, B, M, K, P, xsb, xsk, ws_m, ws_k, s, rp, f32_split);
        } else {
            conv1x1_launch<T>(xp, w, bias, yp, B, M, K, P, xsb, xsk, ws_m, ws_k, s, rp);
            return (int)hipGetLastError();
        }
    });
}

template <typename T, int TM, int TN>
__global__ void __launch_bounds__(256)
oss_conv1x1_wgrad_tiles_kernel(const T *__restrict__ dy, const T *__restrict__ x, float *__restrict__ part, int M, int N, int P,
                               int64_t gsb, int64_t gsm, int64_t xsb, int64_t xsn, int G, int64_t gsg, int64_t xsg, int Mh,
                               int64_t gs_hi, int NB) {
    const int lane = threadIdx.x & 63, wave = threadIdx.x >> 6;
    const int b = blockIdx.y / G, g = blockIdx.y - b * G, slab = blockIdx.x;
    const int pbeg = slab * kWgradSlab, pend = min(P, pbeg + kWgradSlab);
    const int col = lane & 31, kg = lane >> 5;
    const int mt = (M + 32 * TM - 1) / (32 * TM), nt = (NB + 32 * TN - 1) / (32 * TN);
    const T *gb = dy + b * gsb + g * gsg;
    const T *xb = x + b * xsb + g * xsg;
    const size_t pvec = (size_t)G * M * N + (NB > N ? M : 0);
    float *pb = part + (size_t)(b * gridDim.x + slab) * pvec;
    const short kOne = (short)from_f32<T>(1.0f).v;
    const s16x8 zero8 = {0, 0, 0, 0, 0, 0, 0, 0}, ones8 = {kOne, kOne, kOne, kOne, kOne, kOne, kOne, kOne};
    const bool aligned = (((reinterpret_cast<uintptr_t>(gb) | reinterpret_cast<uintptr_t>(xb)) & 15u) == 0) &&
                         (gsm % 8 == 0) && (xsn % 8 == 0) && (pbeg % 8 == 0) && (gs_hi % 8 == 0);
    const int tile = blockIdx.z * 4 + wave;
    if (tile >= mt * nt) return;
    const int m0 = (tile / nt) * 32 * TM, n0 = (tile % nt) * 32 * TN;
    const T *ga[TM];
    const T *xa[TN];
    bool mok[TM], nok[TN], one[TN];
#pragma unroll
    for (int i = 0; i < TM; ++i) {
        const int mrow = m0 + 32 * i + col;
        mok[i] = mrow < M;
        const int mr = mok[i] ? mrow : 0;
        ga[i] = gb + (mr / Mh) * gs_hi + (mr % Mh) * gsm;
    }
#pragma unroll
    for (int j = 0; j < TN; ++j) {
        const int nrow = n0 + 32 * j + col;
        nok[j] = nrow < N;
        one[j] = nrow == N && NB > N;
        xa[j] = xb + (nok[j] ? nrow : 0) * xsn;
    }
    f32x16 acc[TM][TN];
#pragma unroll
    for (int i = 0; i < TM; ++i)
#pragma unroll
        for (int j = 0; j < TN; ++j)
#pragma unroll
            for (int r = 0; r < 16; ++r) acc[i][j][r] = 0.f;

    auto frag = [&](const T *row, int k0, bool ok, bool ones, bool fast) -> s16x8 {
        if (fast) {
            const u32x4 q = *reinterpret_cast<const u32x4 *>(row + k0);
            return ok ? __builtin_bit_cast(s16x8, q) : (ones ? ones8 : zero8);
        }
        s16x8 f;
#pragma unroll
        for (int e = 0; e < 8; ++e) {
            const bool kok = (k0 + e) < pend;
            const int kc = kok ? k0 + e : pend - 1;
            const short v = (short)row[kc].v;
            f[e] = kok ? (ok ? v : (ones ? kOne : (short)0)) : (short)0;
        }
        return f;
    };
    int pk = pbeg;
    if (aligned && pend - pbeg == kWgradSlab) {
        constexpr int IT = kWgradSlab / 16;
        u32x4 qa[IT][TM], qb[IT][TN];
#pragma unroll
        for (int u = 0; u < IT; ++u) {
#pragma unroll
            for (int i = 0; i < TM; ++i) qa[u][i] = *reinterpret_cast<const u32x4 *>(ga[i] + pbeg + u * 16 + kg * 8);
#pragma unroll
            for (int j = 0; j < TN; ++j) qb[u][j] = *reinterpret_cast<const u32x4 *>(xa[j] + pbeg + u * 16 + kg * 8);
        }
#pragma unroll
        for (int u = 0; u < IT; ++u)
#pragma unroll
            for (int i = 0; i < TM; ++i)
#pragma unroll
                for (int j = 0; j < TN; ++j) {
                    const s16x8 af = mok[i] ? __builtin_bit_cast(s16x8, qa[u][i]) : zero8;
                    const s16x8 bf = nok[j] ? __builtin_bit_cast(s16x8, qb[u][j]) : (one[j] ? ones8 : zero8);
// ... 130 lines not shown
```

vmambair_amd/csrc/oss_conv1x1_wg.hip:

```cpp
#include <algorithm>
#include <atomic>
#include <type_traits>
#include "oss_device.h"
#include "oss_host.h"
#include "oss_mfma.h"

namespace oss {

typedef short s16x4 __attribute__((ext_vector_type(4)));

template <typename T, int K, int PT, int PITCH, int GROUP = 6>
__device__ __forceinline__ void copy_tile_to_lds(const T *__restrict__ src, int64_t xsk, T *__restrict__ dst, int tid) {
    constexpr int CPR = PT / 8, TOTAL = K * CPR, NCP = (TOTAL + 255) / 256;
#pragma unroll
    for (int i0 = 0; i0 < NCP; i0 += GROUP) {
        u32x4 q[GROUP];
#pragma unroll
        for (int i = 0; i < GROUP; ++i) {
            if (i0 + i < NCP) {
                const int idx = min(tid + (i0 + i) * 256, TOTAL - 1);
                const int c = idx / CPR, pc = idx - c * CPR;
                q[i] = *reinterpret_cast<const u32x4 *>(src + c * xsk + 8 * pc);
            }
        }
#pragma unroll
        for (int i = 0; i < GROUP; ++i) {
            if (i0 + i < NCP) {
                const int idx = tid + (i0 + i) * 256;
                const int c = idx / CPR, pc = idx - c * CPR;
                if (TOTAL % 256 == 0 || idx < TOTAL) *reinterpret_cast<u32x4 *>(dst + c * PITCH + 8 * pc) = q[i];
            }
        }
    }
}

template <typename T>
struct WgLnArgs {
    const float *w, *b;
    T *n;
    float *mean, *rstd;
    float eps;
};

template <typename T, int KS, bool WT, int PT, bool RES, bool PF, bool LN>
__global__ void __launch_bounds__(256)
oss_conv1x1_wg_kernel(const T *__restrict__ x, const float *__restrict__ w, const float *__restrict__ bias, T *__restrict__ y,
                      int M, int P, int64_t xsb, int64_t xsk, const T *__restrict__ res, WgLnArgs<T> ln) {
    constexpr int K = 16 * KS, NCT = PT / 32;
    constexpr int PX = PT + 32;
    constexpr bool kPairEpi = !RES && PT == 128;
    constexpr int PITCH = kPairEpi ? PT + 16 : PT + 8;
    using OT = typename std::conditional<RES, float, T>::type;
    extern __shared__ __attribute__((aligned(16))) unsigned char wg_smem[];
    T *xs = reinterpret_cast<T *>(wg_smem);
    OT *os = reinterpret_cast<OT *>(xs + K * PX);
    const int tid = threadIdx.x, lane = tid & 63, wave = tid >> 6;
    const int b = blockIdx.y, p0 = blockIdx.x * PT;
    const T *xb = x + b * xsb + p0;
    const int col = lane & 31, kg = lane >> 5;
    const int mt_total = (M + 31) >> 5;
    struct WRaw { f32x4 lo[KS], hi[KS]; float bl; };
    auto issue = [&](int mt, WRaw &r) {
        const int mrow = min(mt * 32 + col, M - 1);
#pragma unroll
        for (int ks = 0; ks < KS; ++ks) {
            const int k0 = ks * 16 + kg * 8;
            if constexpr (!WT) {
                r.lo[ks] = *reinterpret_cast<const f32x4 *>(w + (size_t)mrow * K + k0);
                r.hi[ks] = *reinterpret_cast<const f32x4 *>(w + (size_t)mrow * K + k0 + 4);
            } else {
#pragma unroll
                for (int e = 0; e < 4; ++e) {
                    r.lo[ks][e] = w[(size_t)(k0 + e) * M + mrow];
                    r.hi[ks][e] = w[(size_t)(k0 + 4 + e) * M + mrow];
                }
            }
        }
        r.bl = bias ? bias[mrow] : 0.f;
    };
    WRaw cur;
    const int nz = gridDim.z, zi = blockIdx.z;
    if (wave * nz + zi < mt_total) issue(wave * nz + zi, cur);
    float *lnw_s = reinterpret_cast<float *>(os + 4 * 32 * PITCH), *lnb_s = lnw_s + K;
    float lnw_r = 0.f, lnb_r = 0.f;
    if constexpr (LN) {
        const int c = min(tid, K - 1);
        lnw_r = ln.w[c];
        lnb_r = ln.b ? ln.b[c] : 0.f;
    }
    constexpr int CPR = PT / 8;
    copy_tile_to_lds<T, K, PT, PX>(xb, xsk, xs, tid);
    if constexpr (LN) {
        if (tid < K) { lnw_s[tid] = lnw_r; lnb_s[tid] = lnb_r; }
    }
    __syncthreads();
    if constexpr (LN) {
        constexpr int QPT = PT / 4, NPART = 256 / QPT, CPT = (K + NPART - 1) / NPART;
        float *red = reinterpret_cast<float *>(os);
        const int quad = tid % QPT, part = tid / QPT, px = 4 * quad;
        float v[CPT][4];
#pragma unroll
        for (int i = 0; i < CPT; ++i) {
            const int c = part + i * NPART;
            if (c < K) {
                const u32x2 q = *reinterpret_cast<const u32x2 *>(xs + c * PX + px);
                unpack2<T>(q.x, v[i][0], v[i][1]); unpack2<T>(q.y, v[i][2], v[i][3]);
            } else {
                v[i][0] = v[i][1] = v[i][2] = v[i][3] = 0.f;
            }
        }
        float sum[4] = {0.f, 0.f, 0.f, 0.f};
#pragma unroll
        for (int i = 0; i < CPT; ++i)
#pragma unroll
            for (int u = 0; u < 4; ++u) sum[u] += v[i][u];
        *reinterpret_cast<f32x4 *>(red + part * PT + px) = f32x4{sum[0], sum[1], sum[2], sum[3]};
        __syncthreads();
        float mu[4] = {0.f, 0.f, 0.f, 0.f};
#pragma unroll
        for (int q = 0; q < NPART; ++q) {
            const f32x4 t = *reinterpret_cast<const f32x4 *>(red + q * PT + px);
            mu[0] += t.x; mu[1] += t.y; mu[2] += t.z; mu[3] += t.w;
        }
#pragma unroll
        for (int u = 0; u < 4; ++u) mu[u] /= (float)K;
        __syncthreads();
        float sq[4] = {0.f, 0.f, 0.f, 0.f};
#pragma unroll
        for (int i = 0; i < CPT; ++i) {
            if (part + i * NPART < K) {
#pragma unroll
                for (int u = 0; u < 4; ++u) { const float d = v[i][u] - mu[u]; sq[u] = __builtin_fmaf(d, d, sq[u]); }
            }
        }
        *reinterpret_cast<f32x4 *>(red + part * PT + px) = f32x4{sq[0], sq[1], sq[2], sq[3]};
        __syncthreads();
        float rstd[4] = {0.f, 0.f, 0.f, 0.f};
#pragma unroll
        for (int q = 0; q < NPART; ++q) {
            const f32x4 t = *reinterpret_cast<const f32x4 *>(red + q * PT + px);
            rstd[0] += t.x; rstd[1] += t.y; rstd[2] += t.z; rstd[3] += t.w;
        }
#pragma unroll
        for (int u = 0; u < 4; ++u) rstd[u] = 1.0f / sqrtf(rstd[u] / (float)K + ln.eps);
        if (part == 0 && zi == 0) {
            *reinterpret_cast<f32x4 *>(ln.mean + (size_t)b * P + p0 + px) = f32x4{mu[0], mu[1], mu[2], mu[3]};
            *reinterpret_cast<f32x4 *>(ln.rstd + (size_t)b * P + p0 + px) = f32x4{rstd[0], rstd[1], rstd[2], rstd[3]};
        }
        const bool with_bias = ln.b != nullptr;
        float mu_c[4];
#pragma unroll
        for (int u = 0; u < 4; ++u) mu_c[u] = with_bias ? mu[u] : 0.f;
#pragma unroll
        for (int i = 0; i < CPT; ++i) {
            const int c = part + i * NPART;
            if (c < K) {
                const float wc = lnw_s[c], bc = lnb_s[c];
                float o[4];
#pragma unroll
                for (int u = 0; u < 4; ++u) o[u] = (v[i][u] - mu_c[u]) * rstd[u] * wc + bc;
                *reinterpret_cast<u32x2 *>(xs + c * PX + px) = u32x2{pack2<T>(o[0], o[1]), pack2<T>(o[2], o[3])};
            }
        }
        __syncthreads();
        T *nb = ln.n + (size_t)b * K * P + p0;
        for (int idx = tid; zi == 0 && idx < K * CPR; idx += 256) {
            const int c = idx / CPR, pc = idx - c * CPR;
            *reinterpret_cast<u32x4 *>(nb + (size_t)c * P + 8 * pc) = *reinterpret_cast<const u32x4 *>(xs + c * PX + 8 * pc);
        }
    }
    const int i16 = lane & 15, g = lane >> 4;
    const int tr_off = (8 * (g >> 1) + (i16 >> 2)) * PX + 16 * (g & 1) + 4 * (i16 & 3);
    OT *ow = os + wave * 32 * PITCH;
    for (int mt = wave * nz + zi; mt < mt_total; mt += 4 * nz) {
        const int m0 = mt * 32;
        WRaw nxt;
        if constexpr (PF) { if (mt + 4 * nz < mt_total) issue(mt + 4 * nz, nxt); }
        f32x16 acc[NCT];
#pragma unroll
        for (int ct = 0; ct < NCT; ++ct)
#pragma unroll
            for (int r = 0; r < 16; ++r) acc[ct][r] = 0.f;
#pragma unroll
        for (int ks = 0; ks < KS; ++ks) {
            const s16x8 af = m0 + col < M ? cvt8<T>(cur.lo[ks], cur.hi[ks]) : s16x8{0, 0, 0, 0, 0, 0, 0, 0};
#pragma unroll
            for (int ct = 0; ct < NCT; ++ct) {
                const T *bp = xs + ks * 16 * PX + ct * 32 + tr_off;
                const s16x4 lo = __builtin_amdgcn_ds_read_tr16_b64_v4i16((__attribute__((address_space(3))) s16x4 *)(bp));
                const s16x4 hi = __builtin_amdgcn_ds_read_tr16_b64_v4i16((__attribute__((address_space(3))) s16x4 *)(bp + 4 * PX));
                const s16x8 bf = {lo.x, lo.y, lo.z, lo.w, hi.x, hi.y, hi.z, hi.w};
                acc[ct] = Mfma<T>::run(af, bf, acc[ct]);
            }
        }
        if constexpr (!kPairEpi) {
#pragma unroll
            for (int r = 0; r < 16; ++r) {
                const int row = (r & 3) + 8 * (r >> 2) + 4 * kg;
                const float bv = __int_as_float(__builtin_amdgcn_ds_bpermute(row << 2, __float_as_int(cur.bl)));
#pragma unroll
                for (int ct = 0; ct < NCT; ++ct) {
                    if constexpr (RES) ow[row * PITCH + ct * 32 + col] = acc[ct][r] + bv;
                    else               ow[row * PITCH + ct * 32 + col] = from_f32<T>(acc[ct][r] + bv);
                }
            }
        } else {
            const bool odd = lane & 1;
#pragma unroll
            for (int rr = 0; rr < 8; ++rr) {
                const int r = (rr & 1) + 4 * (rr >> 1);
                constexpr int kPairStep = 2;
                const int rowA = (r & 3) + 8 * (r >> 2) + 4 * kg, rowB = rowA + 2;
                const float bvA = __int_as_float(__builtin_amdgcn_ds_bpermute(rowA << 2, __float_as_int(cur.bl)));
                const float bvB = __int_as_float(__builtin_amdgcn_ds_bpermute(rowB << 2, __float_as_int(cur.bl)));
                T *dst = ow + (odd ? rowB : rowA) * PITCH + (col & ~1);
#pragma unroll
                for (int ct = 0; ct < NCT; ++ct) {
                    const float va = acc[ct][r] + bvA, vb = acc[ct][r + kPairStep] + bvB;
                    const float give = odd ? va : vb;
                    const float recv = __int_as_float(__builtin_amdgcn_update_dpp(0, __float_as_int(give), 0xB1, 0xf, 0xf, false));
                    *reinterpret_cast<uint32_t *>(dst + ct * 32) = odd ? pack2<T>(recv, vb) : pack2<T>(va, recv);
                }
            }
        }
        __builtin_amdgcn_wave_barrier();
#pragma unroll
        for (int q = 0; q < 32 * CPR / 64; ++q) {
            const int chunk = q * 64 + lane, row = chunk / CPR;
            const int pc = kPairEpi ? ((chunk - row * CPR) - 2 * row) & (CPR - 1) : chunk - row * CPR;
            if (m0 + row < M) {
                const size_t o = ((size_t)b * M + m0 + row) * P + p0 + 8 * pc;
                if constexpr (RES) {
                    const f32x4 v0 = *reinterpret_cast<const f32x4 *>(ow + row * PITCH + 8 * pc);
                    const f32x4 v1 = *reinterpret_cast<const f32x4 *>(ow + row * PITCH + 8 * pc + 4);
                    const u32x4 rq = *reinterpret_cast<const u32x4 *>(res + o);
                    float r8[8];
                    unpack2<T>(rq.x, r8[0], r8[1]); unpack2<T>(rq.y, r8[2], r8[3]); unpack2<T>(rq.z, r8[4], r8[5]); unpack2<T>(rq.w, r8[6], r8[7]);
                    *reinterpret_cast<u32x4 *>(y + o) = u32x4{pack2<T>(v0.x + r8[0], v0.y + r8[1]), pack2<T>(v0.z + r8[2], v0.w + r8[3]),
                                                              pack2<T>(v1.x + r8[4], v1.y + r8[5]), pack2<T>(v1.z + r8[6], v1.w + r8[7])};
                } else {
                    *reinterpret_cast<u32x4 *>(y + o) = *reinterpret_cast<const u32x4 *>(ow + row * PITCH + 8 * pc);
                }
            }
        }
        __builtin_amdgcn_wave_barrier();
        if constexpr (PF) { cur = nxt; } else { if (mt + 4 * nz < mt_total) issue(mt + 4 * nz, cur); }
    }
}

constexpr int kWgXPad = 32;
static size_t wg_lds_bytes(int K, int pt, bool res) { return (size_t)K * 2 * (pt + kWgXPad) + (size_t)4 * 32 * (res ? 4 : 2) * (pt + 16) + 2 * (size_t)K * sizeof(float); }
static std::atomic<int> g_wg_pixels{0};
void conv1x1_wg_set_pixels(int pt) { g_wg_pixels.store(pt == 64 || pt == 128 ? pt : 0); }
static void wg_shape(int B, int M, int K, int P, int &pt, int &nz) {
    const int f = g_wg_pixels.load();
    const long t128 = (long)B * (P / 128);
    pt = f ? f : ((K <= 48 && t128 < 1024) || t128 < 256 ? 64 : 128);
    const long wgs = (long)B * (P / pt);
    const int groups = ((M + 31) / 32 + 3) / 4;
    nz = (int)std::min<long>(groups, (256 + wgs - 1) / wgs);
    if (nz < 1) nz = 1;
}

static constexpr bool wg_ks_built(int ks) { return ks == 1 || ks == 2 || ks == 3 || ks == 4 || ks == 6 || ks == 8 || ks == 12; }
int conv1x1_wg_ok(oss_dtype io, int M, int K, int P, int64_t xsb, int64_t xsk, const void *x, const void *y, const float *w,
                  const void *res) {
    if (res) return 0;
    if (!io_ok<IO_16>(io)) return 0;
    if (K % 16 != 0 || K < 16 || K > 192 || P % 128 != 0 || M < 1) return 0;
    if (!wg_ks_built(K / 16)) return 0;
    if (xsb % 8 != 0 || xsk % 8 != 0) return 0;
    if ((reinterpret_cast<uintptr_t>(x) | reinterpret_cast<uintptr_t>(y) | reinterpret_cast<uintptr_t>(w) | reinterpret_cast<uintptr_t>(res)) & 15u)
        return 0;
    return wg_lds_bytes(K, 128, res != nullptr) <= kMaxLdsBytes ? 1 : 0;
}

template <typename T, bool WT, bool LN = false>
static int wg_launch(const T *x, const float *w, const float *bias, T *y, int B, int M, int K, int P, int64_t xsb, int64_t xsk,
                     const T *res, hipStream_t s, WgLnArgs<T> ln = WgLnArgs<T>{}) {
    int pt, nz;
    wg_shape(B, M, K, P, pt, nz);
    const size_t smem = wg_lds_bytes(K, pt, res != nullptr);
    dim3 grid(P / pt, B, nz);
#define OSS_WG3(KS_, PT_, RES_)                                                                                      \
    do {                                                                                                             \
        static LdsGate gate;                                                                                         \
        auto kern = oss_conv1x1_wg_kernel<T, KS_, WT, PT_, RES_, (KS_ <= 6), LN>;                                        \
        if (const int e = gate.ensure(reinterpret_cast<const void *>(kern), smem)) return e;                         \
        hipLaunchKernelGGL(kern, grid, dim3(256), smem, s, x, w, bias, y, M, P, xsb, xsk, res, ln);                      \
    } while (0)
#define OSS_WG(KS_)                                                                                                  \
    do {                                                                                                             \
        if (pt == 128) OSS_WG3(KS_, 128, false); else OSS_WG3(KS_, 64, false);                                       \
    } while (0)
    switch (K / 16) {
        case 1: OSS_WG(1); break;
        case 2: OSS_WG(2); break;
        case 3: OSS_WG(3); break;
        case 4: OSS_WG(4); break;
        case 6: OSS_WG(6); break;
        case 8: OSS_WG(8); break;
        case 12: OSS_WG(12); break;
        default: return OSS_ERR_SHAPE;
    }
#undef OSS_WG
#undef OSS_WG3
    return (int)hipGetLastError();
}

int conv1x1_wg(oss_dtype io, const void *x, const float *w, const float *bias, void *y, int B, int M, int K, int P, int64_t xsb,
               int64_t xsk, int wt, hipStream_t s, const void *res) {
    if (!conv1x1_wg_ok(io, M, K, P, xsb, xsk, x, y, w, res)) return OSS_ERR_SHAPE;
    return io_dispatch<IO_16>(io, [&](auto tag) {
        using T = typename decltype(tag)::type;
        const T *xp = reinterpret_cast<const T *>(x), *rp = reinterpret_cast<const T *>(res);
        T *yp = reinterpret_cast<T *>(y);
        return wt ? wg_launch<T, true>(xp, w, bias, yp, B, M, K, P, xsb, xsk, rp, s)
                  : wg_launch<T, false>(xp, w, bias, yp, B, M, K, P, xsb, xsk, rp, s);
    });
}

template <typename T>
struct WgLnBwdArgs {
    const T *x;
    const float *w;
    const float *mean, *rstd;
    const T *skip;
    T *dx;
    float *part;
    int with_bias;
};

template <typename T, int PT>
__device__ __forceinline__ void wg_lnbwd_stage(const WgLnBwdArgs<T> &a, const T *os, const T *xt, const T *st, float *red, int M, int P,
                                               int b, int p0, int tid, int lane) {
    constexpr int PITCH = PT + 8;
    constexpr int QPT = PT / 4, NPART = 256 / QPT, CMAX = (128 + NPART - 1) / NPART;
    const int quad = tid % QPT, part = tid / QPT, px = 4 * quad;
    const bool with_bias = a.with_bias != 0, has_skip = a.skip != nullptr;
    float mu[4], rs[4];
    {
        const f32x4 m4 = *reinterpret_cast<const f32x4 *>(a.mean + (size_t)b * P + p0 + px);
        const f32x4 r4 = *reinterpret_cast<const f32x4 *>(a.rstd + (size_t)b * P + p0 + px);
        mu[0] = m4.x; mu[1] = m4.y; mu[2] = m4.z; mu[3] = m4.w;
        rs[0] = r4.x; rs[1] = r4.y; rs[2] = r4.z; rs[3] = r4.w;
    }
    float gv[CMAX][4], xv[CMAX][4], s1[4] = {0.f, 0.f, 0.f, 0.f}, s2[4] = {0.f, 0.f, 0.f, 0.f};
    float wcs[CMAX];
#pragma unroll
    for (int i = 0; i < CMAX; ++i) wcs[i] = a.w[min(part + i * NPART, M - 1)];
    float *pw = a.part + (size_t)(blockIdx.y * gridDim.x + blockIdx.x) * 2 * M;
#pragma unroll
    for (int i = 0; i < CMAX; ++i) {
        const int c = part + i * NPART;
        float aw = 0.f, ab = 0.f;
        if (c < M) {
            const u32x2 gq = *reinterpret_cast<const u32x2 *>(os + ((c >> 5) * 32 + (c & 31)) * PITCH + px);
            const u32x2 xq2 = *reinterpret_cast<const u32x2 *>(xt + c * PITCH + px);
            unpack2<T>(gq.x, gv[i][0], gv[i][1]); unpack2<T>(gq.y, gv[i][2], gv[i][3]);
            unpack2<T>(xq2.x, xv[i][0], xv[i][1]); unpack2<T>(xq2.y, xv[i][2], xv[i][3]);
            const float wc = wcs[i];
#pragma unroll
            for (int u = 0; u < 4; ++u) {
                const float xh = with_bias ? (xv[i][u] - mu[u]) * rs[u] : xv[i][u] * rs[u];
                const float gg = gv[i][u];
                aw = __builtin_fmaf(gg, xh, aw);
                ab += gg;
                const float gw = gg * wc;
                s1[u] += gw;
                s2[u] = __builtin_fmaf(gw, with_bias ? xh : xv[i][u], s2[u]);
            }
        } else {
#pragma unroll
            for (int u = 0; u < 4; ++u) { gv[i][u] = 0.f; xv[i][u] = 0.f; }
        }
        const float tw = segment_sum_to_last<QPT>(aw), tb = segment_sum_to_last<QPT>(ab);
        if ((lane & (QPT - 1)) == QPT - 1 && c < M) { pw[c] = tw; pw[M + c] = tb; }
    }
    *reinterpret_cast<f32x4 *>(red + part * PT + px) = f32x4{s1[0], s1[1], s1[2], s1[3]};
    *reinterpret_cast<f32x4 *>(red + (NPART + part) * PT + px) = f32x4{s2[0], s2[1], s2[2], s2[3]};
    __syncthreads();
    float m1[4] = {0.f, 0.f, 0.f, 0.f}, m2[4] = {0.f, 0.f, 0.f, 0.f};
#pragma unroll
    for (int q = 0; q < NPART; ++q) {
        const f32x4 t1 = *reinterpret_cast<const f32x4 *>(red + q * PT + px), t2 = *reinterpret_cast<const f32x4 *>(red + (NPART + q) * PT + px);
        m1[0] += t1.x; m1[1] += t1.y; m1[2] += t1.z; m1[3] += t1.w;
        m2[0] += t2.x; m2[1] += t2.y; m2[2] += t2.z; m2[3] += t2.w;
    }
#pragma unroll
    for (int u = 0; u < 4; ++u) { m1[u] /= (float)M; m2[u] /= (float)M; }
    T *dxb = a.dx + (size_t)b * M * P + p0;
#pragma unroll
    for (int i = 0; i < CMAX; ++i) {
        const int c = part + i * NPART;
        if (c < M) {
            const float wc = wcs[i];
            float sk[4] = {0.f, 0.f, 0.f, 0.f};
            if (has_skip) {
                const u32x2 s2q = *reinterpret_cast<const u32x2 *>(st + c * PITCH + px);
                unpack2<T>(s2q.x, sk[0], sk[1]); unpack2<T>(s2q.y, sk[2], sk[3]);
            }
// ... 79 lines not shown
    __syncthreads();
    T *xt = xs, *st = xs + M * PITCH;
#pragma unroll
    for (int q = 0; q < NLD; ++q) {
        const int idx = q * 256 + tid;
        if (idx < M * CPR) {
            const int c = idx / CPR, pc = idx - c * CPR;
            *reinterpret_cast<u32x4 *>(xt + c * PITCH + 8 * pc) = xq[q];
            *reinterpret_cast<u32x4 *>(st + c * PITCH + 8 * pc) = sq[q];
        }
    }
    __syncthreads();
    wg_lnbwd_stage<T, PT>(a, os, xt, st, red, M, P, b, p0, tid, lane);
}

__global__ void __launch_bounds__(256)
oss_wg_lnbwd_finish(const float *__restrict__ part, float *__restrict__ dw, float *__restrict__ db, int nblk, int C) {
    const int i = blockIdx.x * 256 + threadIdx.x;
    if (i >= 2 * C) return;
    float sum = 0.f;
    for (int k = 0; k < nblk; ++k) sum += part[(size_t)k * 2 * C + i];
    if (i < C) dw[i] = sum;
    else if (db) db[i - C] = sum;
}

size_t conv1x1_dgrad_lnbwd_partial_floats(int B, int M, int P) { return (size_t)B * (P / 64) * 2 * M; }

int conv1x1_dgrad_lnbwd_ok(oss_dtype io, int M, int K, int P, int B) {
    if (!io_ok<IO_16>(io)) return 0;
    if (K % 16 != 0 || K < 2 * M || K > 192 || M < 1 || M > 128 || P % 128 != 0) return 0;
    const int ks = K / 16;
    return (ks == 2 || ks == 3 || ks == 4 || ks == 6 || ks == 8 || ks == 12) ? 1 : 0;
}

template <typename T>
static int lnbwd_launch(const T *dy, const float *w, int B, int M, int K, int P, int64_t xsb, int64_t xsk, WgLnBwdArgs<T> a, float *dlw,
                        float *dlb, hipStream_t s) {
    const int pt = (long)B * (P / 128) >= 256 ? 128 : 64;
    const size_t smem = sizeof(uint16_t) * ((size_t)K + 4 * 32) * (pt + 8) + sizeof(float) * 2 * 8 * 128;
    dim3 grid(P / pt, B);
#define OSS_LNB(KS_, PT_)                                                                                   \
    do {                                                                                                    \
        static LdsGate gate;                                                                                \
        auto kern = oss_conv1x1_dgrad_lnbwd_kernel<T, KS_, PT_>;                                            \
        if (const int e = gate.ensure(reinterpret_cast<const void *>(kern), smem)) return e;                \
        hipLaunchKernelGGL(kern, grid, dim3(256), smem, s, dy, w, M, P, xsb, xsk, a);                       \
    } while (0)
#define OSS_LNB2(KS_) do { if (pt == 128) OSS_LNB(KS_, 128); else OSS_LNB(KS_, 64); } while (0)
    switch (K / 16) {
        case 2: OSS_LNB2(2); break;
        case 3: OSS_LNB2(3); break;
        case 4: OSS_LNB2(4); break;
        case 6: OSS_LNB2(6); break;
        case 8: OSS_LNB2(8); break;
        case 12: OSS_LNB2(12); break;
        default: return OSS_ERR_SHAPE;
    }
#undef OSS_LNB2
#undef OSS_LNB
    const int nblk = (int)(grid.x * grid.y);
    if (defer_finish())
        defer_sum(a.part, nblk, (size_t)2 * M, (size_t)(dlb ? 2 : 1) * M, dlw, (size_t)M, dlb);
    else
        hipLaunchKernelGGL(oss_wg_lnbwd_finish, dim3((2 * M + 255) / 256), dim3(256), 0, s, a.part, dlw, dlb, nblk, M);
    return (int)hipGetLastError();
}

int conv1x1_dgrad_lnbwd(oss_dtype io, const void *dy, const float *w, const void *x, const float *ln_w, int with_bias, const float *mean,
                        const float *rstd, const void *skip, void *dx, float *dlw, float *dlb, float *part, int B, int M, int K, int P,
                        int64_t xsb, int64_t xsk, hipStream_t s) {
    if (!conv1x1_dgrad_lnbwd_ok(io, M, K, P, B) || xsb % 8 != 0 || xsk % 8 != 0) return OSS_ERR_SHAPE;
    if ((reinterpret_cast<uintptr_t>(dy) | reinterpret_cast<uintptr_t>(x) | reinterpret_cast<uintptr_t>(skip) | reinterpret_cast<uintptr_t>(dx) |
         reinterpret_cast<uintptr_t>(mean) | reinterpret_cast<uintptr_t>(rstd)) & 15u)
        return OSS_ERR_SHAPE;
    return io_dispatch<IO_16>(io, [&](auto tag) {
        using T = typename decltype(tag)::type;
        WgLnBwdArgs<T> a{reinterpret_cast<const T *>(x), ln_w, mean, rstd, reinterpret_cast<const T *>(skip), reinterpret_cast<T *>(dx), part,
                         with_bias};
        return lnbwd_launch<T>(reinterpret_cast<const T *>(dy), w, B, M, K, P, xsb, xsk, a, dlw, dlb, s);
    });
}

int ln_conv1x1_wg(oss_dtype io, const void *x, const float *ln_w, const float *ln_b, float eps, void *n, float *mean, float *rstd,
                  const float *w, const float *bias, void *y, int B, int M, int K, int P, int64_t xsb, int64_t xsk, hipStream_t s) {
    if (!conv1x1_wg_ok(io, M, K, P, xsb, xsk, x, y, w, nullptr) || (reinterpret_cast<uintptr_t>(n) & 15u)) return OSS_ERR_SHAPE;
    return io_dispatch<IO_16>(io, [&](auto tag) {
        using T = typename decltype(tag)::type;
        WgLnArgs<T> a{ln_w, ln_b, reinterpret_cast<T *>(n), mean, rstd, eps};
        return wg_launch<T, false, true>(reinterpret_cast<const T *>(x), w, bias, reinterpret_cast<T *>(y), B, M, K, P, xsb, xsk, nullptr, s, a);
    });
}

}
```

vmambair_amd/csrc/oss_host.h:

```cpp
#pragma once
#include <hip/hip_runtime.h>
#include "../../include/vmambair_oss.h"

#include <atomic>
#include <initializer_list>

namespace oss {
struct bf16_t;
struct f16_t;

template <typename T> struct IoTag { using type = T; };
enum IoSet { IO_ALL, IO_16 };
template <IoSet S = IO_ALL, typename F> int io_dispatch(oss_dtype io, F &&f) {
    switch ((int)io) {
        case OSS_F32: if constexpr (S == IO_ALL) return f(IoTag<float>{}); else break;
        case OSS_F16: return f(IoTag<f16_t>{});
        case OSS_BF16: return f(IoTag<bf16_t>{});
    }
    return OSS_ERR_SHAPE;
}
template <IoSet S = IO_ALL> bool io_ok(oss_dtype io) { return io_dispatch<S>(io, [](auto) { return 0; }) == 0; }
inline int io_bytes(oss_dtype io) { return io == OSS_F32 ? 4 : io_ok<IO_16>(io) ? 2 : 0; }

constexpr size_t kMaxLdsBytes = 160 * 1024;
// ... 18 lines not shown
constexpr int kMaxSegments = 64;
int scan_pick_segments(long wgs, int n_chunks, int seg_req, double ovh);
inline size_t scan_carry_bytes(int batch, int dim, int dstate, int n_seg) {
    return sizeof(float) * 2 * (size_t)batch * dim * dstate * n_seg;
}
extern std::atomic<int> g_last_fwd_segments, g_last_bwd_segments, g_last_bwd_lane_states;
int scan_carry_split(long wgs, int n_seg, int cps, int n_chunks, int per_call = 0);
inline bool scan_finish_dt_ok(int seqlen, int rank) { return seqlen > 0 && seqlen % 4 == 0 && rank >= 1 && rank <= 8; }
template <typename T> int scan_fwd_dispatch(const oss_scan_fwd_params &p, int variant, int seg_req, hipStream_t stream);
struct LaunchTimer {
    virtual void begin(hipStream_t) = 0;
    virtual void end(hipStream_t) = 0;
    virtual void segmented() {}
    virtual ~LaunchTimer() = default;
};
template <typename T>
int scan_bwd_dispatch(const oss_scan_bwd_params &p, int variant, int seg_req, hipStream_t stream, LaunchTimer *timer,
                      LaunchTimer *finish_timer = nullptr);

int scan_bwd_rows_per_wg(int variant);
int scan_bwd_pick_variant(int batch, int dim, int seqlen, int dstate, int n_groups);
int dwconv3x3(oss_dtype io, const void *x, const float *w, const float *bias, void *y, int B, int C, int H, int W,
              int64_t xsb, int64_t xsc, int64_t ysb, int64_t ysc, int flip, hipStream_t s, void *pre = nullptr, int act = 0);
int dwconv3x3_fused_ok(oss_dtype io, int H, int W, int nch);
int effn_fwd_ok(oss_dtype io, int D, int hidden, int H, int W);
int effn_round_weights(oss_dtype io, const float *pin, const float *pdw, const float *pout, void *w_in, float *w_dw, void *w_out, int D,
                       int hidden, hipStream_t s);
int effn_fwd(oss_dtype io, const void *x, const float *ln_w, const float *ln_b, const void *w_in, const float *w_dw, const void *w_out,
             void *out, int B, int D, int hidden, int H, int W, int64_t xsb, int64_t xsc, int64_t osb, int64_t osc, float eps,
             hipStream_t s);
int dwgate_fwd_ok(oss_dtype io, int H, int W);
int dwgate_fwd(oss_dtype io, const void *t, const float *w, const float *bias, void *out, int B, int Hd, int H, int W,
               int64_t tsb, int64_t tsc, int64_t osb, int64_t osc, hipStream_t s);
int dwconv3x3_bwd_fused(oss_dtype io, int mode, const void *x, const float *w, const float *bias, const void *dy, void *dx,
                        float *dw, float *db, float *part, int B, int C, int H, int W, int64_t xsb, int64_t xsc, int64_t gsb,
                        int64_t gsc, int64_t dsb, int64_t dsc, hipStream_t s);
int dwconv3x3_flat2_ok(oss_dtype io, int H, int W);
int dwconv3x3_silu_flat2_fwd(oss_dtype io, const void *x, const float *w, const float *bias, void *x2, int B, int C, int H, int W,
                             int64_t xsb, int64_t xsc, hipStream_t s);
int dwconv3x3_silu_flat2_bwd(oss_dtype io, const void *x, const float *w, const float *bias, const void *g2, void *dx, float *dw,
                             float *db, float *part, int B, int C, int H, int W, int64_t xsb, int64_t xsc, int64_t dsb, int64_t dsc,
                             hipStream_t s);
int dwconv3x3_wgrad(oss_dtype io, const void *x, const void *dy, float *dw, float *db, float *part, int B, int C, int H,
                    int W, int64_t xsb, int64_t xsc, int64_t gsb, int64_t gsc, hipStream_t s, const void *pre = nullptr,
                    void *dpre = nullptr);
int conv1x1_f32(const float *x, const float *w, const float *bias, float *y, int B, int M, int K, int P, int64_t xsb, int64_t xsk,
                int64_t wsm, int64_t wsk, hipStream_t s, const float *res, int split = 0);
int proj_f32_ok(int B, int D, int C, int R, int L, std::initializer_list<const void *> ptrs);
int proj_fwd_f32(const float *x2, const float *Wx, const float *Wdt, float *xdbl, float *dts, int B, int D, int C, int R, int L,
                 hipStream_t s, int split = 0);
int proj_dgrad_f32(const float *ddts, float *dxdbl, const float *du, const float *Wx, const float *Wdt, float *dx2, int B, int D, int C,
                   int R, int L, hipStream_t s, int split = 0);
size_t rows_f32_wgrad_partial_floats(int B, int G, int M, int N, int P);
int rows_f32_wgrad(const float *a, const float *bm, float *out, float *part, int B, int G, int GB, int M, int N, int P, int64_t asb,
                   int64_t asg, int64_t asm_, int64_t bsb, int64_t bsg, int64_t bsn, hipStream_t s, float *db = nullptr, int split = 0);
int conv3x3_thin_ok(oss_dtype io, int Cin, int Cout, int H, int W);
int conv3x3_thin_fwd(oss_dtype io, const void *x, const float *w, const float *bias, void *y, int B, int Cin, int Cout, int H, int W,
                     int64_t xsb, int64_t xsc, int64_t ysb, int64_t ysc, hipStream_t s);
int conv3x3_thin_dgrad(oss_dtype io, const void *dy, const float *w, void *dx, int B, int Cin, int Cout, int H, int W, int64_t gsb,
                       int64_t gsc, int64_t dsb, int64_t dsc, hipStream_t s);
size_t conv3x3_thin_wgrad_partial_floats(int B, int Cin, int Cout);
int conv3x3_thin_wgrad(oss_dtype io, const void *x, const void *dy, float *dw, float *db, float *part, int B, int Cin, int Cout, int H,
                       int W, int64_t xsb, int64_t xsc, int64_t gsb, int64_t gsc, hipStream_t s);
int conv3x3_dense_ok(oss_dtype io, int Cin, int Cout, int H, int W);
int conv3x3_dense_fwd(oss_dtype io, const void *x, const float *w, const float *bias, void *y, int B, int Cin, int Cout, int H, int W,
                      int64_t xsb, int64_t xsc, int64_t ysb, int64_t ysc, hipStream_t s);
int conv3x3_dense_dgrad(oss_dtype io, const void *dy, const float *w, void *dx, int B, int Cin, int Cout, int H, int W, int64_t gsb,
                        int64_t gsc, int64_t dsb, int64_t dsc, hipStream_t s);
size_t conv3x3_dense_wgrad_partial_floats(int B, int Cin, int Cout, int H, int W);
int conv3x3_dense_wgrad(oss_dtype io, const void *x, const void *dy, float *dw, float *db, float *part, int B, int Cin, int Cout, int H,
                        int W, int64_t xsb, int64_t xsc, int64_t gsb, int64_t gsc, hipStream_t s);
int ln_nchw_fwd(oss_dtype xt, oss_dtype yt, const void *x, const float *w, const float *bias, const void *gate, void *y,
                float *mean, float *rstd, int B, int C, int P, int64_t xsb, int64_t xsc, int64_t gsb, int64_t gsc, float eps,
                hipStream_t s, float *pool_part = nullptr);
int ln_nchw_fwd_pool_tiles(int C, int P, int64_t xsb, int64_t xsc, int64_t gsb, int64_t gsc);
size_t ln_nchw_bwd_partial_floats(int B, int C, int P);
int ln_nchw_bwd(oss_dtype xt, oss_dtype yt, const void *x, const float *w, const float *bias, const void *gate,
                const void *dy, const float *mean, const float *rstd, void *dx, void *dgate, float *dw, float *db,
                float *part, int B, int C, int P, int64_t xsb, int64_t xsc, int64_t gsb, int64_t gsc, hipStream_t s,
                const void *res = nullptr, int64_t dgsb = 0, const float *dy_mul = nullptr, const float *dy_add = nullptr,
                float add_scale = 1.f);
int merge4(oss_dtype io, const void *out, float *y, int B, int D, int H, int W, hipStream_t s);
int ln_conv1x1_wg(oss_dtype io, const void *x, const float *ln_w, const float *ln_b, float eps, void *n, float *mean, float *rstd,
                  const float *w, const float *bias, void *y, int B, int M, int K, int P, int64_t xsb, int64_t xsk, hipStream_t s);
size_t conv1x1_dgrad_lnbwd_partial_floats(int B, int M, int P);
int conv1x1_dgrad_lnbwd_ok(oss_dtype io, int M, int K, int P, int B);
int conv1x1_dgrad_lnbwd(oss_dtype io, const void *dy, const float *w, const void *x, const float *ln_w, int with_bias, const float *mean,
                        const float *rstd, const void *skip, void *dx, float *dlw, float *dlb, float *part, int B, int M, int K, int P,
                        int64_t xsb, int64_t xsk, hipStream_t s);
void conv1x1_set_wg(int on);
void conv1x1_wg_set_pixels(int pt);
int conv1x1_wg_ok(oss_dtype io, int M, int K, int P, int64_t xsb, int64_t xsk, const void *x, const void *y, const float *w,
                  const void *res = nullptr);
int conv1x1_wg(oss_dtype io, const void *x, const float *w, const float *bias, void *y, int B, int M, int K, int P, int64_t xsb,
               int64_t xsk, int wt, hipStream_t s, const void *res = nullptr);
int conv1x1(oss_dtype io, const void *x, const float *w, const float *bias, void *y, int B, int M, int K, int P, int64_t xsb,
            int64_t xsk, int64_t ws_m, int64_t ws_k, hipStream_t s, const void *res = nullptr, int f32_split = 0);
int conv1x1_wgrad_slabs(int P);
void conv1x1_wgrad_set_tile(int mode);
void conv1x1_wgrad_set_span(int mult);
int conv1x1_wgrad(oss_dtype io, const void *dy, const void *x, float *dw, float *part, int B, int M, int N, int P,
                  int64_t gsb, int64_t gsm, int64_t xsb, int64_t xsn, hipStream_t s, int G = 1, int64_t gsg = 0, int64_t xsg = 0,
                  int Mh = 0, int64_t gs_hi = 0, float *db = nullptr, int f32_split = 0);
int proj_fwd(oss_dtype io, const void *x2, const float *Wx, const float *Wdt, void *xdbl, void *dts, int B, int D, int C, int R,
             int L, hipStream_t s, int f32_split = 0);
int proj_dgrad(oss_dtype io, const void *ddts, void *dxdbl, const void *du, const float *Wx, const float *Wdt, void *dx2, int B,
               int D, int C, int R, int L, hipStream_t s, int f32_split = 0);
void proj_force_valu(int on);
bool proj_mfma_ok(oss_dtype io, int B, int D, int C, int R, int L);
int cross_scan2(oss_dtype it, oss_dtype ot, const void *x, void *x2, int B, int D, int H, int W, int64_t xsb, int64_t xsc,
                hipStream_t s);
int cross_merge2(oss_dtype io, const void *g2, void *dx, int B, int D, int H, int W, hipStream_t s);
size_t chan_grad_floats(int L, int dc, int Rc, int Cc);
size_t chan_bwd_scratch_floats(int B, int L, int dc, int Rc, int Cc);
int chan_fwd(const oss_chan_params &p, hipStream_t s);
int chan_bwd(const oss_chan_params &p, const float *gc, float *dpool, float *gsum, float *scratch, hipStream_t s);
int rowsum(oss_dtype io, const void *a, const void *bmul, float *out, int B, int C, int P, int64_t asb, int64_t asc, int64_t bsb,
           int64_t bsc, float alpha, hipStream_t s);
int row_affine(oss_dtype io, const void *x, const float *mul, const float *add, void *y, int B, int C, int P, int64_t xsb,
               int64_t xsc, float alpha, hipStream_t s);
int gelu_gate_fwd(oss_dtype io, const void *h, void *out, int B, size_t n, int64_t hsb, hipStream_t s);
int gelu_gate_bwd(oss_dtype io, const void *h, const void *dout, void *dh, int B, size_t n, int64_t hsb, int64_t gsb, hipStream_t s);
bool defer_wgrad();
void defer_wgrad_push(const void *desc, size_t bytes, unsigned blocks);
size_t wgrad_desc_bytes();
int wgrad_grouped_launch(int io, const void *d_descs, const void *d_map, unsigned total_blocks, hipStream_t s);
void wgrad_desc_set_first_block(void *desc, unsigned first);
int wgrad_desc_io(const void *desc);
bool defer_finish();
void defer_sum(const float *src, int K, size_t stride, size_t V, float *dst0, size_t n0, float *dst1);
int sum_partials_multi(const oss_sum_chunk *chunks, int n_chunks, hipStream_t s);
int adam_ema_step(const oss_adam_chunk *chunks, int n_chunks, float *state, float lr, float beta1, float beta2, float eps,
                  float ema_decay, hipStream_t s, float weight_decay = 0.f, const float *grad_scale = nullptr);
int image_metrics_ok(oss_dtype io, int C, int H, int W, int crop, int flags);
size_t image_metrics_partial_doubles(int B, int C, int H, int W, int crop);
int image_metrics(oss_dtype io, const void *a, const void *b, double *out, double *part, int B, int C, int H, int W, int64_t asb,
                  int64_t asc, int64_t ars, int64_t bsb, int64_t bsc, int64_t brs, int crop, int flags, hipStream_t s);
int scan_fwd_pick_variant(int batch, int dim, int seqlen, int dstate, int n_groups, int elem_bytes);
}
```

vmambair_amd/ops/pointwise.py:

```python
from __future__ import annotations

import contextlib
import os
from typing import List, Optional

import torch

from .. import _capi, _precision
from ._common import (_keep_operands, _recorded_before,
                      _DT, _LIB, _check, _f32c, _fork_for_wgrad, _keep, _keep_views, _planes, _ptr)


def conv1x1_fwd(x: torch.Tensor, weight: torch.Tensor, bias: Optional[torch.Tensor],
                residual: Optional[torch.Tensor] = None) -> torch.Tensor:
    _check(x.is_cuda and x.dim() == 4 and x.dtype in _DT, "conv1x1: x must be bf16 / fp16 / fp32 on the GPU")
    B, Cin, H, W = x.shape
    Cout = weight.shape[0]
    _check(tuple(weight.shape) == (Cout, Cin, 1, 1), "conv1x1: weight must be (Cout, Cin, 1, 1)")
    x = _planes(x)
    if x.dtype == torch.float32 and not f32_ok(x):
        x = x.contiguous()
    w = weight.detach().float().reshape(Cout, Cin).contiguous()
    b = None if bias is None else bias.detach().float().contiguous()
    if residual is not None:
        _check(tuple(residual.shape) == (B, Cout, H, W), "conv1x1: residual must have the output's shape")
        residual = residual.to(x.dtype).contiguous()
    if x.dtype == torch.float32 and CONV1X1_F32_WGRAD_ONLY:
        y = torch.nn.functional.conv2d(x, weight.detach().float(), b)
        return y if residual is None else y + residual
    y = torch.empty((B, Cout, H, W), dtype=x.dtype, device=x.device)
    if x.numel() == 0:
        return y
    lib = _capi.load()
    with torch.cuda.device(x.device):
        _capi.check(lib.oss_conv1x1_fwd(_precision.io_code(x.dtype), x.data_ptr(), w.data_ptr(), _ptr(b), _ptr(residual), y.data_ptr(), B, Cout, Cin,
                                        H * W, x.stride(0), x.stride(1), torch.cuda.current_stream().cuda_stream), "oss_conv1x1_fwd")
    return y


def conv1x1_bwd(x: torch.Tensor, weight: torch.Tensor, dy: torch.Tensor, has_bias: bool = False) -> List[torch.Tensor]:
    B, Cin, H, W = x.shape
    Cout = weight.shape[0]
    P = H * W
    x, dy = _planes(x), _planes(dy)
    if dy.dtype != x.dtype:
        dy = dy.to(x.dtype)
    f32 = x.dtype == torch.float32
    if f32:
        x = x if f32_ok(x) else x.contiguous()
        dy = dy if f32_ok(dy) else dy.contiguous()
    w = weight.detach().float().reshape(Cout, Cin).contiguous()
    dx = torch.empty((B, Cin, H, W), dtype=x.dtype, device=x.device)
    lib = _capi.load()
    with torch.cuda.device(x.device):
        with _fork_for_wgrad(x, dy):
            dw = torch.empty((Cout, Cin), dtype=torch.float32, device=x.device)
            db = torch.empty((Cout,), dtype=torch.float32, device=x.device) if has_bias else None
            part = torch.empty(int(lib.oss_conv1x1_wgrad_partial_floats(B, Cout, Cin, P)), dtype=torch.float32, device=x.device)
            rec0 = _recorded_before()
            _capi.check(lib.oss_conv1x1_wgrad(_precision.io_code(x.dtype), dy.data_ptr(), x.data_ptr(), dw.data_ptr(), _ptr(db), part.data_ptr(), B,
                                              Cout, Cin, P, dy.stride(0), dy.stride(1), x.stride(0), x.stride(1),
                                              torch.cuda.current_stream().cuda_stream), "oss_conv1x1_wgrad")
            _keep(part, dw, db)
            _keep_operands(rec0, dy, x)
        if f32 and CONV1X1_F32_WGRAD_ONLY:
            dx = torch.nn.functional.conv_transpose2d(dy, weight.detach().float())
        else:
            _capi.check(lib.oss_conv1x1_dgrad(_precision.io_code(x.dtype), dy.data_ptr(), w.data_ptr(), dx.data_ptr(), B, Cout, Cin, P,
                                              dy.stride(0), dy.stride(1), torch.cuda.current_stream().cuda_stream), "oss_conv1x1_dgrad")
    return [dx, dw.view(Cout, Cin, 1, 1), db if db is not None else x.new_empty(0, dtype=torch.float32)]


_LIB.define("conv1x1_fwd(Tensor x, Tensor weight, Tensor? bias, Tensor? residual) -> Tensor")
_LIB.define("conv1x1_bwd(Tensor x, Tensor weight, Tensor dy, bool has_bias) -> Tensor[]")
_LIB.impl("conv1x1_fwd", conv1x1_fwd, "CUDA")
_LIB.impl("conv1x1_bwd", conv1x1_bwd, "CUDA")


class Conv1x1Fn(torch.autograd.Function):
    @staticmethod
    def forward(ctx, x, weight, bias, residual=None):
        ctx.has_bias, ctx.has_res = bias is not None, residual is not None
        ctx.save_for_backward(x, weight)
        return torch.ops.vmambair.conv1x1_fwd(x, weight, bias, residual)

    @staticmethod
    def backward(ctx, dy):
        x, weight = ctx.saved_tensors
        dx, dw, db = torch.ops.vmambair.conv1x1_bwd(x, weight, dy, ctx.has_bias)
        return dx, dw.to(weight.dtype), (db if ctx.has_bias else None), (dy if ctx.has_res else None)


def f32_ok(t: torch.Tensor) -> bool:
    return (t.shape[2] * t.shape[3]) % 4 == 0 and t.data_ptr() % 16 == 0 and t.stride(0) % 4 == 0 and t.stride(1) % 4 == 0


CONV1X1_F32 = os.environ.get("VMAMBAIR_CONV1X1_F32", "1") != "0"
CONV1X1_F32_WGRAD_ONLY = os.environ.get("VMAMBAIR_CONV1X1_F32", "1") == "wgrad"

CONV1X1_IMPL = os.environ.get("VMAMBAIR_CONV1X1", "mfma")


def conv1x1(x: torch.Tensor, conv: torch.nn.Conv2d, residual: Optional[torch.Tensor] = None) -> torch.Tensor:
    if CONV1X1_IMPL == "mfma" and x.is_cuda:
        if torch.is_autocast_enabled("cuda") and x.dtype == torch.float32:
            x = x.to(torch.get_autocast_dtype("cuda"))
        if x.dtype in (torch.bfloat16, torch.float16) or (x.dtype == torch.float32 and CONV1X1_F32 and x.dim() == 4 and
                                                          (x.shape[2] * x.shape[3]) % 4 == 0 and not torch.is_autocast_enabled("cuda")):
            if residual is not None and residual.dtype != x.dtype:
                return residual + Conv1x1Fn.apply(x, conv.weight, conv.bias, None)
            return Conv1x1Fn.apply(x, conv.weight, conv.bias, residual)
    y = conv(x)
    return y if residual is None else residual + y


LN_CONV_FUSED = os.environ.get("VMAMBAIR_LN_CONV_FUSED", "1") == "1"


def ln_conv1x1_ok(x: torch.Tensor, weight: torch.Tensor) -> bool:
    if not (LN_CONV_FUSED and CONV1X1_IMPL == "mfma" and x.is_cuda and x.dim() == 4 and x.dtype in (torch.bfloat16, torch.float16)
            and x.numel() and weight.dim() == 4 and weight.shape[2] == 1 and weight.shape[3] == 1):
        return False
    B, Cin, H, W = x.shape
    if not (x.stride(3) == 1 and x.stride(2) == W and x.stride(1) % 8 == 0 and x.stride(0) % 8 == 0 and x.data_ptr() % 16 == 0):
        return False
    return bool(_capi.load().oss_ln_conv1x1_ok(_DT[x.dtype], weight.shape[0], Cin, H * W))


def ln_conv1x1_fwd(x: torch.Tensor, ln_weight: torch.Tensor, ln_bias: Optional[torch.Tensor], weight: torch.Tensor,
                   bias: Optional[torch.Tensor]) -> List[torch.Tensor]:
    B, Cin, H, W = x.shape
    Cout, P = weight.shape[0], H * W
    w = weight.detach().float().reshape(Cout, Cin).contiguous()
    b = None if bias is None else bias.detach().float().contiguous()
    lw = ln_weight.detach().float().contiguous()
    lb = None if ln_bias is None else ln_bias.detach().float().contiguous()
    y = torch.empty((B, Cout, H, W), dtype=x.dtype, device=x.device)
    n = torch.empty((B, Cin, H, W), dtype=x.dtype, device=x.device)
    mean = torch.empty((B, P), dtype=torch.float32, device=x.device)
    rstd = torch.empty((B, P), dtype=torch.float32, device=x.device)
    with torch.cuda.device(x.device):
        _capi.check(_capi.load().oss_ln_conv1x1_fwd(_DT[x.dtype], x.data_ptr(), lw.data_ptr(), _ptr(lb), 1e-5, n.data_ptr(), mean.data_ptr(),
                                                    rstd.data_ptr(), w.data_ptr(), _ptr(b), y.data_ptr(), B, Cout, Cin, P, x.stride(0),
                                                    x.stride(1), torch.cuda.current_stream().cuda_stream), "oss_ln_conv1x1_fwd")
    return [y, n, mean, rstd]


_LIB.define("ln_conv1x1_fwd(Tensor x, Tensor ln_weight, Tensor? ln_bias, Tensor weight, Tensor? bias) -> Tensor[]")
_LIB.impl("ln_conv1x1_fwd", ln_conv1x1_fwd, "CUDA")


class LNConv1x1Fn(torch.autograd.Function):

    @staticmethod
    def forward(ctx, x, ln_weight, ln_bias, weight, bias):
        y, n, mean, rstd = torch.ops.vmambair.ln_conv1x1_fwd(x, ln_weight, ln_bias, weight, bias)
        ctx.has_bias, ctx.has_lnb = bias is not None, ln_bias is not None
        ctx.save_for_backward(x, ln_weight, ln_bias, n, mean, rstd, weight)
        return y, x.view_as(x)

    @staticmethod
    def backward(ctx, dy, dskip=None):
        x, ln_weight, ln_bias, n, mean, rstd, weight = ctx.saved_tensors
        if dy is None:
            return dskip, None, None, None, None
        dx, dlw, dlb, dw, db = torch.ops.vmambair.ln_conv1x1_bwd(x, ln_weight, ln_bias, n, mean, rstd, weight, dy, dskip, ctx.has_bias)
        return (dx, dlw.to(ln_weight.dtype), dlb.to(ln_bias.dtype) if ctx.has_lnb else None, dw.to(weight.dtype),
                db if ctx.has_bias else None)


LN_BWD_FUSED = os.environ.get("VMAMBAIR_LN_BWD_FUSED", "1") == "1"


def ln_conv1x1_bwd(x: torch.Tensor, ln_weight: torch.Tensor, ln_bias: Optional[torch.Tensor], n: torch.Tensor, mean: torch.Tensor,
                   rstd: torch.Tensor, weight: torch.Tensor, dy: torch.Tensor, dskip: Optional[torch.Tensor],
                   has_bias: bool) -> List[torch.Tensor]:
    B, Cin, H, W = x.shape
    Cout, P = weight.shape[0], H * W
    lib = _capi.load()
    dyp = _planes(dy)
    if dyp.dtype != x.dtype:
        dyp = dyp.to(x.dtype)
    fused = LN_BWD_FUSED and x.is_contiguous() and (dskip is None or dskip.dtype == x.dtype) and dyp.data_ptr() % 16 == 0 and \
        dyp.stride(0) % 8 == 0 and dyp.stride(1) % 8 == 0 and bool(lib.oss_conv1x1_dgrad_ln_bwd_ok(_DT[x.dtype], Cout, Cin, P, B))
    if not fused:
        dn, dw, db = conv1x1_bwd(n, weight, dyp, has_bias)
        from .layernorm import ln_nchw_bwd
        dx, _, dlw, dlb = ln_nchw_bwd(x, ln_weight, ln_bias, None, dn, mean, rstd, dskip, None)
        return [dx, dlw, dlb, dw, db]
    w = weight.detach().float().reshape(Cout, Cin).contiguous()
    lw = ln_weight.detach().float().contiguous()
    n = _planes(n)
    if dskip is not None:
        dskip = dskip.contiguous()
    dx = torch.empty((B, Cin, H, W), dtype=x.dtype, device=x.device)
    f = dict(dtype=torch.float32, device=x.device)
    with torch.cuda.device(x.device):
        with _fork_for_wgrad(n, dyp):
            dw = torch.empty((Cout, Cin), **f)
            db = torch.empty((Cout,), **f) if has_bias else None
            part = torch.empty(int(lib.oss_conv1x1_wgrad_partial_floats(B, Cout, Cin, P)), **f)
            rec0 = _recorded_before()
            _capi.check(lib.oss_conv1x1_wgrad(_DT[x.dtype], dyp.data_ptr(), n.data_ptr(), dw.data_ptr(), _ptr(db), part.data_ptr(), B,
                                              Cout, Cin, P, dyp.stride(0), dyp.stride(1), n.stride(0), n.stride(1),
                                              torch.cuda.current_stream().cuda_stream), "oss_conv1x1_wgrad")
            _keep(part, dw, db)
            _keep_operands(rec0, dyp, n)
        dlw = torch.empty((Cin,), **f)
        dlb = torch.empty((Cin,), **f) if ln_bias is not None else None
        lpart = torch.empty(int(lib.oss_conv1x1_dgrad_ln_bwd_partial_floats(B, Cin, P)), **f)
        _capi.check(lib.oss_conv1x1_dgrad_ln_bwd(_DT[x.dtype], dyp.data_ptr(), w.data_ptr(), x.data_ptr(), lw.data_ptr(),
                                                 1 if ln_bias is not None else 0, mean.data_ptr(), rstd.data_ptr(), _ptr(dskip),
                                                 dx.data_ptr(), dlw.data_ptr(), _ptr(dlb), lpart.data_ptr(), B, Cout, Cin, P,
                                                 dyp.stride(0), dyp.stride(1), torch.cuda.current_stream().cuda_stream),
                    "oss_conv1x1_dgrad_ln_bwd")
        _keep(lpart, dlw, dlb)
    e = x.new_empty(0, dtype=torch.float32)
    return [dx, dlw, dlb if dlb is not None else e, dw.view(Cout, Cin, 1, 1), db if db is not None else e]


_LIB.define("ln_conv1x1_bwd(Tensor x, Tensor ln_weight, Tensor? ln_bias, Tensor n, Tensor mean, Tensor rstd, Tensor weight, Tensor dy, "
            "Tensor? dskip, bool has_bias) -> Tensor[]")
_LIB.impl("ln_conv1x1_bwd", ln_conv1x1_bwd, "CUDA")


def ln_conv1x1(x: torch.Tensor, ln_weight: torch.Tensor, ln_bias: Optional[torch.Tensor], conv: torch.nn.Conv2d):
    return LNConv1x1Fn.apply(x, ln_weight, ln_bias, conv.weight, conv.bias)
# ... 1 lines not shown
```

vmambair_amd/train_graph.py:

```python
from __future__ import annotations

import os

from typing import Callable, Optional

import torch
import torch.distributed as dist

from . import ops as _ops


class GraphedTrainStep:
    def __init__(self, net: torch.nn.Module, lr: float = 2e-4, betas=(0.9, 0.99), ema_decay: float = 0.999,
                 autocast_dtype: Optional[torch.dtype] = torch.bfloat16,
                 loss_fn: Callable = torch.nn.functional.l1_loss, warmup: int = 3, shadow_weights: bool = True,
                 fused_optimizer: bool = True, split_graphs: bool = False, overlap_wgrads: bool = False,
                 defer_finishes: bool = True, micro_streams: int = 1, weight_decay: float = 0.0,
                 clip_grad_norm: Optional[float] = None, multi_shape: bool = False, grad_buckets: int = 1,
                 allreduce_via_host: bool = False):
        self.net = net
        self.params = [p for p in net.parameters() if p.requires_grad]
        self.device = self.params[0].device
        assert self.device.type == "cuda", "graph capture needs a GPU"
        self.world = dist.get_world_size() if (dist.is_available() and dist.is_initialized()) else 1
        self.multi_shape = multi_shape
        self.nbuckets = max(1, int(grad_buckets))
        self.allreduce_via_host = bool(allreduce_via_host)
        self.split = self.world > 1 or split_graphs or multi_shape or self.nbuckets > 1
        self._flat = None
        self.autocast_dtype = autocast_dtype
        self.loss_fn = loss_fn
        self.ema_decay = ema_decay
        self.warmup = warmup
        self.shadow = {}
        if shadow_weights and autocast_dtype is not None:
            mods = dict(net.named_modules())
            for name, p in net.named_parameters():
                owner, leaf = name.rsplit(".", 1) if "." in name else ("", name)
                m = mods.get(owner)
                if ".conv_cin." in name or ".conv_cout." in name:
                    continue
                dense_conv = isinstance(m, torch.nn.Conv2d) and m.groups == 1
                if dense_conv and m.kernel_size == (1, 1) and _ops.pointwise.CONV1X1_IMPL == "mfma" and owner.rsplit(".", 1)[-1] in (
                        "in_conv", "out_conv", "project_in", "project_out", "reduce_chan_level2", "reduce_chan_level3"):
                    continue
                if dense_conv and m.kernel_size == (3, 3) and min(m.in_channels, m.out_channels) <= 4 and _ops.conv3x3.THIN_IMPL:
                    continue
                if dense_conv and m.kernel_size == (3, 3) and _ops.conv3x3.DENSE_IMPL and m.in_channels % 16 == 0 and m.out_channels >= 5 \
                        and m.stride == (1, 1) and m.padding == (1, 1) and m.dilation == (1, 1) and m.padding_mode == "zeros":
                    continue
                fused_proj = getattr(m, "fused_core", False) and getattr(m, "omni", False)
                if dense_conv or (leaf in ("x_proj_weight", "dt_projs_weight") and not fused_proj):
                    self.shadow[name] = (p, torch.empty_like(p, dtype=autocast_dtype).requires_grad_())
        self._masters = [m for m, _ in self.shadow.values()]
        self._shadows = [s for _, s in self.shadow.values()]
        self._master_grads = [torch.zeros_like(m) for m in self._masters]
        self._shadow_map = {n: s for n, (_, s) in self.shadow.items()}
        self.ema = [p.detach().clone() for p in self.params] if ema_decay > 0 else None
        self.fopt = None
        self.opt = None
        if fused_optimizer and all(p.dtype == torch.float32 and p.is_contiguous() for p in self.params):
            from .optim import FusedAdamEMA
            self.fopt = FusedAdamEMA(self.params, self.ema, lr=lr, betas=betas, ema_decay=ema_decay,
                                     weight_decay=weight_decay, clip_grad_norm=clip_grad_norm)
        else:
            assert clip_grad_norm is None, "gradient clipping is implemented in the fused optimizer launch only"
            cls = torch.optim.AdamW if weight_decay > 0 else torch.optim.Adam
            kw = dict(weight_decay=weight_decay) if weight_decay > 0 else {}
            self.opt = cls(self.params, lr=torch.tensor(float(lr), dtype=torch.float32, device=self.device), betas=betas,
                           fused=True, capturable=True, **kw)
        self.lr = float(lr)
        self.iteration = 0
        self.wside = torch.cuda.Stream(device=self.device) if overlap_wgrads else None
        self.defer = defer_finishes
        self.nmicro = max(1, int(micro_streams))
        assert not (self.nmicro > 1 and overlap_wgrads), "micro_streams and overlap_wgrads are alternatives"
        self.mstreams = [torch.cuda.Stream(device=self.device) for _ in range(self.nmicro)] if self.nmicro > 1 else []
        self._names = [n for n, p in net.named_parameters() if p.requires_grad]
        self._leaf_sets = []
        if self.nmicro > 1:
            named = dict(net.named_parameters())
            for _ in range(self.nmicro):
                self._leaf_sets.append({n: self._shadow_map.get(n, named[n]).detach().requires_grad_() for n in self._names})
            self._shadow_tmp = [torch.zeros_like(m) for m in self._masters]
        self.ftables = [None] * self.nmicro
        self.wtables = [None] * self.nmicro
        self.wgrad_stats = None
        if self.nbuckets > 1:
            assert self.nmicro == 1 and not overlap_wgrads and defer_finishes, "grad_buckets needs the deferred single-branch step"
            assert not multi_shape, "grad_buckets: the bucket cuts are record counts of ONE input shape (use grad_buckets=1 with multi_shape)"
            self.warmup = max(self.warmup, 2)
        self._cuts = None
        self._defer_ctx = None
        self._flushed = (0, 0)
        self.btables = None
        self.graph_flush = []
        self.ar_stream = torch.cuda.Stream(device=self.device) if self.nbuckets > 1 else None
        self.graph_fb: Optional[torch.cuda.CUDAGraph] = None
        self.graph_opt: Optional[torch.cuda.CUDAGraph] = None
        self.static_lq = self.static_gt = self.static_loss = None
        self._shapes = {}
        self._active = None
        self.allreduce_ms = None

    def _backward_open(self, loss, leaves):
        assert self._defer_ctx is None, "the previous step's buckets were not all flushed"
        marks, handles = [], []
        if self._cuts is None:
            from . import _capi
            lib = _capi.load()
            owner = {id(p): i for i, p in enumerate(self.params)}
            for name, (m, sh) in self.shadow.items():
                owner[id(sh)] = owner[id(m)]
            for t in leaves:
                handles.append(t.register_post_accumulate_grad_hook(
                    lambda t_, i=owner[id(t)]: marks.append((i, int(lib.oss_deferred_wgrads()), int(lib.oss_deferred_chunks())))))
        self._defer_ctx = _ops.deferred_finishes(wgrad_flusher=None)
        self._defer_ctx.__enter__()
        self._flushed = (0, 0)
        try:
            loss.backward()
        except BaseException:
            self._defer_ctx.__exit__(None, None, None)
            self._defer_ctx = None
            raise
        finally:
            for h in handles:
                h.remove()
        if self._cuts is None:
            self._probe = marks

    def _make_buckets(self):
        from .ddp import FlatGrads
        seen, order, at = set(), [], {}
        for i, nw, nc in self._probe:
            if i not in seen:
# ... 27 lines not shown
            if _ops.pending_wgrads():
                need = _ops.pending_wgrad_table_bytes()
                if wt is None or wt.capacity < need:
                    assert not torch.cuda.is_current_stream_capturing(), "the weight-gradient tables must exist before the capture"
                    wt = self.btables[k][0] = _ops.WgradTable(self.device, need)
                _ops.flush_wgrads(wt, count=nw)
        if last or nc > 0:
            n = _ops.pending_finish_chunks()
            if n:
                if ft is None or ft.capacity < n:
                    assert not torch.cuda.is_current_stream_capturing(), "the finish tables must exist before the capture"
                    ft = self.btables[k][1] = _ops.FinishTable(self.device, n)
                _ops.flush_finishes(ft, count=nc)
        if not last:
            self._flushed = (self._cuts[k][0], self._cuts[k][1])
        trip = self._bucket_shadows[k]
        if trip:
            with torch.no_grad():
                torch._foreach_copy_([g for _, _, g in trip], [sh.grad for _, sh, _ in trip])
            for m, _, g in trip:
                m.grad = g
        self._flat.pack_bucket(k)
        if last:
            self._defer_ctx.__exit__(None, None, None)
            self._defer_ctx = None

    def _allreduce_bucket(self, k: int):
        if self.world == 1:
            return
        ev = torch.cuda.Event()
        ev.record()
        with torch.cuda.stream(self.ar_stream):
            self.ar_stream.wait_event(ev)
            if self.allreduce_ms is not None:
                e0, e1 = torch.cuda.Event(enable_timing=True), torch.cuda.Event(enable_timing=True)
                e0.record()
                self._flat.allreduce_bucket(k)
                e1.record()
                self._ar_events.append((e0, e1))
            else:
                self._flat.allreduce_bucket(k)

    def _backward(self, loss, leaves, slot: int = 0):
        if self.nbuckets > 1:
            return self._backward_open(loss, leaves)
        if not self.defer:
            with _ops.wgrad_side_stream(self.wside):
                loss.backward()
            return
        tables = self.wtables[slot] if self.wtables[slot] is not None else []
        self.wtables[slot] = tables
        used = [0]

        def flush_wgrads_now():
            nb = _ops.pending_wgrad_table_bytes()
            k = used[0]
            if k == len(tables):
                tables.append(None)
            if tables[k] is None or tables[k].capacity < nb:
                assert not torch.cuda.is_current_stream_capturing(), "the weight-gradient tables must exist before the capture"
                tables[k] = _ops.WgradTable(self.device, nb)
            _ops.flush_wgrads(tables[k])
            used[0] = k + 1

        with _ops.deferred_finishes(wgrad_flusher=flush_wgrads_now if self.wside is None else None):
            with _ops.wgrad_side_stream(self.wside):
                loss.backward()
            if self.wside is not None:
                torch.cuda.current_stream().wait_stream(self.wside)
            if not torch.cuda.is_current_stream_capturing():
                lost = _ops.orphaned_deferred_outputs(leaves)
                if lost:
                    raise RuntimeError(f"{lost} deferred weight gradients were copied before the flush (see ops.py CONTRACT)")
            if _ops.pending_wgrads():
                flush_wgrads_now()
            self.wgrad_stats = dict(_ops.WGRAD_STATS, grouped_launches=used[0])
            n = _ops.pending_finish_chunks()
            if self.ftables[slot] is None or self.ftables[slot].capacity < n:
                assert not torch.cuda.is_current_stream_capturing(), "the finish table must exist before the capture"
                self.ftables[slot] = _ops.FinishTable(self.device, n)
            _ops.flush_finishes(self.ftables[slot])

    def _fwd_bwd(self):
        if self.nmicro > 1:
            return self._fwd_bwd_micro()
        for p in self.params:
            p.grad = None
        for s_ in self._shadows:
            s_.grad = None
        if self._shadows:
            with torch.no_grad():
                torch._foreach_copy_(self._shadows, self._masters)
        with torch.autocast("cuda", dtype=self.autocast_dtype, enabled=self.autocast_dtype is not None):
            if self._shadows:
                out = torch.func.functional_call(self.net, self._shadow_map, (self.static_lq,))
            else:
                out = self.net(self.static_lq)
        loss = self.loss_fn(out.float(), self.static_gt)
        self._backward(loss, list(self.params) + self._shadows)
        if self.nbuckets > 1:
            return loss.detach()
        if self.wside is not None:
            torch.cuda.current_stream().wait_stream(self.wside)
        if self._shadows:
            with torch.no_grad():
                torch._foreach_copy_(self._master_grads, [s_.grad for s_ in self._shadows])
            for m, g in zip(self._masters, self._master_grads):
                m.grad = g
        if self.split:
            self._pack_grads()
        return loss.detach()

    def _fwd_bwd_micro(self):
        cur = torch.cuda.current_stream()
        M = self.nmicro
        B = self.static_lq.shape[0]
        assert B % M == 0, f"batch {B} does not split into {M} micro-batches"
        mb = B // M
        if self._shadows:
            with torch.no_grad():
                torch._foreach_copy_(self._shadows, self._masters)
        losses = []
        for m, st in enumerate(self.mstreams):
            leaves = self._leaf_sets[m]
            for t in leaves.values():
                t.grad = None
            st.wait_stream(cur)
            with torch.cuda.stream(st):
                lq, gt = self.static_lq[m * mb:(m + 1) * mb], self.static_gt[m * mb:(m + 1) * mb]
                with torch.autocast("cuda", dtype=self.autocast_dtype, enabled=self.autocast_dtype is not None):
                    out = torch.func.functional_call(self.net, leaves, (lq,))
                loss = self.loss_fn(out.float(), gt) / M
                self._backward(loss, list(leaves.values()), m)
                losses.append(loss.detach())
        for st in self.mstreams:
            cur.wait_stream(st)
        shadowed = set(self._shadow_map)
        with torch.no_grad():
            plain = [n for n in self._names if n not in shadowed]
            g0 = [self._leaf_sets[0][n].grad for n in plain]
            for m in range(1, M):
                torch._foreach_add_(g0, [self._leaf_sets[m][n].grad for n in plain])
            if self._shadows:
                sn = list(self._shadow_map)
                torch._foreach_copy_(self._master_grads, [self._leaf_sets[0][n].grad for n in sn])
                for m in range(1, M):
                    torch._foreach_copy_(self._shadow_tmp, [self._leaf_sets[m][n].grad for n in sn])
                    torch._foreach_add_(self._master_grads, self._shadow_tmp)
            total = losses[0]
            for l_ in losses[1:]:
                total = total + l_
        named = dict(zip(plain, g0))
        mg = dict(zip(self._shadow_map, self._master_grads))
        for n, p in zip(self._names, self.params):
            p.grad = mg[n] if n in mg else named[n]
        if self.split:
            self._pack_grads()
        return total

    def _first_bucket_pass(self):
        wt = _ops.WgradTable(self.device, _ops.pending_wgrad_table_bytes()) if _ops.pending_wgrads() else None
        if wt is not None:
            _ops.flush_wgrads(wt)
        n = _ops.pending_finish_chunks()
        if n:
            _ops.flush_finishes(_ops.FinishTable(self.device, n))
        self._defer_ctx.__exit__(None, None, None)
        self._defer_ctx = None
# ... 220 lines not shown
```

Measured before the change: 244.5 images/s.

## Pre-pack 1x1 conv weights into MFMA fragment images once per step

Adds a per-step packing kernel that converts the fp32 1x1 conv weights into 16-bit, MFMA-fragment-ordered images for both the forward and the input-gradient directions. The pair/pairk conv kernels and the fused LN+conv1x1 forward then load fragments straight from these images, skipping the per-block fp32-to-16-bit conversion, LDS staging and transposed loads. The trainer builds the pack table at init and refreshes it before every fwd/bwd. The cost is one extra launch per step and extra memory for the images.

```diff
diff --git a/include/vmambair_oss.h b/include/vmambair_oss.h
--- a/include/vmambair_oss.h
+++ b/include/vmambair_oss.h
@@ -142,6 +142,21 @@
 int oss_conv1x1_dgrad(oss_dtype io, const void *dy, const float *weight, void *dx, int batch, int cout, int cin, int pixels,
                       int64_t dy_batch_stride, int64_t dy_channel_stride, oss_stream_t stream);
 size_t oss_conv1x1_wgrad_partial_floats(int batch, int cout, int cin, int pixels);
+size_t oss_conv1x1_fwd_image_bytes(int cout, int cin);
+size_t oss_conv1x1_dgrad_image_bytes(int cout, int cin);
+size_t oss_conv1x1_pack_row_bytes(void);
+int oss_conv1x1_pack_rows(int cout, int cin);
+int oss_conv1x1_pack_fill(void *rows, const float *weight, void *fwd_image, void *dgrad_image, int cout, int cin);
+int oss_conv1x1_pack_weights(oss_dtype io, const void *table, int n_rows, oss_stream_t stream);
+int oss_conv1x1_fwd_packed(oss_dtype io, const void *x, const float *weight, const void *fwd_image, const float *bias,
+                           const void *residual, void *y, int batch, int cout, int cin, int pixels, int64_t x_batch_stride,
+                           int64_t x_channel_stride, oss_stream_t stream);
+int oss_conv1x1_dgrad_packed(oss_dtype io, const void *dy, const float *weight, const void *dgrad_image, void *dx, int batch,
+                             int cout, int cin, int pixels, int64_t dy_batch_stride, int64_t dy_channel_stride,
+                             oss_stream_t stream);
+int oss_ln_conv1x1_fwd_packed(oss_dtype io, const void *x, const float *ln_weight, const float *ln_bias, float eps, void *n, float *mean,
+                              float *rstd, const float *weight, const void *fwd_image, const float *bias, void *y, int batch, int cout,
+                              int cin, int pixels, int64_t x_batch_stride, int64_t x_channel_stride, oss_stream_t stream);
 int oss_conv1x1_wg(oss_dtype io, const void *x, const float *weight, const float *bias, void *y, int batch, int cout, int cin,
                    int pixels, int64_t x_batch_stride, int64_t x_channel_stride, int transposed_weight, oss_stream_t stream);
 int oss_ln_conv1x1_ok(oss_dtype io, int cout, int cin, int pixels);
@@ -333,7 +348,7 @@
 
 int oss_f32_matmul_modes(void);
 
-#define OSS_ABI_VERSION 8
+#define OSS_ABI_VERSION 9
 int oss_abi_version(void);
 size_t oss_abi_struct_bytes(int which);
 
diff --git a/vmambair_amd/csrc/oss_capi.hip b/vmambair_amd/csrc/oss_capi.hip
--- a/vmambair_amd/csrc/oss_capi.hip
+++ b/vmambair_amd/csrc/oss_capi.hip
@@ -145,7 +145,7 @@
                                             "cross-scan / cross-merge / merge4", "gelu gate (unfused)", "thin 3x3 convolutions",
                                             "deferred partial-sum finishing", "Adam(W) + EMA"};
 static const char *const kFamKernels[FAM_N] = {"oss_conv1x1_pair_kernel|oss_conv1x1_pairk_kernel|oss_conv1x1_pairw_kernel|oss_conv1x1_wg_kernel|"
-                                               "oss_conv1x1_dgrad_lnbwd_kernel|oss_conv1x1_f32_kernel",
+                                               "oss_conv1x1_dgrad_lnbwd_kernel|oss_conv1x1_f32_kernel|oss_conv1x1_pack_kernel",
                                                "oss_conv1x1_wgrad|oss_rows_f32_wgrad|oss_proj_wgrad",
                                                "oss_dwconv3x3|oss_dwgate|oss_effn",
                                                "oss_proj_fwd|oss_proj_dgrad|oss_dt_fwd|oss_dt_dgrad|oss_proj_valu",
@@ -426,6 +426,45 @@
     return conv1x1(io, dy, weight, nullptr, dx, batch, cin, cout, pixels, gsb, gsc, 1, cin, reinterpret_cast<hipStream_t>(stream), nullptr, x3);
 }
 
+size_t oss_conv1x1_fwd_image_bytes(int cout, int cin) { return cout > 0 && cin > 0 ? conv1x1_image_bytes(cout, cin) : 0; }
+size_t oss_conv1x1_dgrad_image_bytes(int cout, int cin) { return cout > 0 && cin > 0 ? conv1x1_image_bytes(cin, cout) : 0; }
+size_t oss_conv1x1_pack_row_bytes(void) { return conv1x1_pack_row_bytes(); }
+int oss_conv1x1_pack_rows(int cout, int cin) { return cout > 0 && cin > 0 ? conv1x1_pack_rows(cout, cin) : 0; }
+int oss_conv1x1_pack_fill(void *rows, const float *weight, void *fwd_image, void *dgrad_image, int cout, int cin) {
+    if (!rows || !weight || !fwd_image || !dgrad_image) return OSS_ERR_NULL;
+    if (cout <= 0 || cin <= 0 || (size_t)cout * cin >= (1u << 30)) return OSS_ERR_SHAPE;
+    if ((reinterpret_cast<uintptr_t>(fwd_image) | reinterpret_cast<uintptr_t>(dgrad_image)) & 15u) return OSS_ERR_SHAPE;
+    return conv1x1_pack_fill(rows, weight, fwd_image, dgrad_image, cout, cin);
+}
+int oss_conv1x1_pack_weights(oss_dtype io, const void *table, int n_rows, oss_stream_t stream) {
+    if (is_f32_split(io)) return OSS_ERR_SHAPE;
+    fam_count(FAM_CONV1X1, (double)n_rows * 256.0 * 16.0 * 3.0);
+    if (!table) return OSS_ERR_NULL;
+    if (n_rows <= 0) return OSS_ERR_SHAPE;
+    return conv1x1_pack(io, table, n_rows, reinterpret_cast<hipStream_t>(stream));
+}
+int oss_conv1x1_fwd_packed(oss_dtype io, const void *x, const float *weight, const void *fwd_image, const float *bias,
+                           const void *residual, void *y, int batch, int cout, int cin, int pixels, int64_t xsb, int64_t xsc,
+                           oss_stream_t stream) {
+    if (!fwd_image || !io_ok<IO_16>(io)) return oss_conv1x1_fwd(io, x, weight, bias, residual, y, batch, cout, cin, pixels, xsb, xsc, stream);
+    fam_count(FAM_CONV1X1, (double)batch * pixels * io_bytes(io) * ((double)cin + cout + (residual ? cout : 0)) + 2.0 * cin * cout);
+    if (!x || !weight || !y) return OSS_ERR_NULL;
+    if (batch <= 0 || cout <= 0 || cin <= 0 || pixels <= 0 || batch > 65535 || cout > 32 * 65535) return OSS_ERR_SHAPE;
+    if (reinterpret_cast<uintptr_t>(fwd_image) & 15u) return OSS_ERR_SHAPE;
+    return conv1x1(io, x, weight, bias, y, batch, cout, cin, pixels, xsb, xsc, cin, 1, reinterpret_cast<hipStream_t>(stream),
+                   residual, 0, fwd_image);
+}
+int oss_conv1x1_dgrad_packed(oss_dtype io, const void *dy, const float *weight, const void *dgrad_image, void *dx, int batch,
+                             int cout, int cin, int pixels, int64_t gsb, int64_t gsc, oss_stream_t stream) {
+    if (!dgrad_image || !io_ok<IO_16>(io)) return oss_conv1x1_dgrad(io, dy, weight, dx, batch, cout, cin, pixels, gsb, gsc, stream);
+    fam_count(FAM_CONV1X1, (double)batch * pixels * io_bytes(io) * ((double)cin + cout) + 2.0 * cin * cout);
+    if (!dy || !weight || !dx) return OSS_ERR_NULL;
+    if (batch <= 0 || cout <= 0 || cin <= 0 || pixels <= 0 || batch > 65535) return OSS_ERR_SHAPE;
+    if (reinterpret_cast<uintptr_t>(dgrad_image) & 15u) return OSS_ERR_SHAPE;
+    return conv1x1(io, dy, weight, nullptr, dx, batch, cin, cout, pixels, gsb, gsc, 1, cin, reinterpret_cast<hipStream_t>(stream), nullptr, 0,
+                   dgrad_image);
+}
+
 size_t oss_conv1x1_wgrad_partial_floats(int batch, int cout, int cin, int pixels) {
     if (batch <= 0 || cout <= 0 || cin <= 0 || pixels <= 0) return 0;
     return (size_t)batch * conv1x1_wgrad_slabs(pixels) * cout * (cin + 1);
@@ -497,6 +536,19 @@
     if (batch <= 0 || batch > 65535) return OSS_ERR_SHAPE;
     return ln_conv1x1_wg(io, x, ln_weight, ln_bias, eps, n, mean, rstd, weight, bias, y, batch, cout, cin, pixels, xsb, xsc,
                          reinterpret_cast<hipStream_t>(stream));
+}
+
+int oss_ln_conv1x1_fwd_packed(oss_dtype io, const void *x, const float *ln_weight, const float *ln_bias, float eps, void *n, float *mean,
+                              float *rstd, const float *weight, const void *fwd_image, const float *bias, void *y, int batch, int cout,
+                              int cin, int pixels, int64_t xsb, int64_t xsc, oss_stream_t stream) {
+    if (!fwd_image)
+        return oss_ln_conv1x1_fwd(io, x, ln_weight, ln_bias, eps, n, mean, rstd, weight, bias, y, batch, cout, cin, pixels, xsb, xsc, stream);
+    if (is_f32_split(io)) return OSS_ERR_SHAPE;
+    fam_count(FAM_CONV1X1, (double)batch * pixels * (io_bytes(io) * (2.0 * cin + cout) + 8.0) + 2.0 * cin * cout);
+    if (!x || !ln_weight || !n || !mean || !rstd || !weight || !y) return OSS_ERR_NULL;
+    if (batch <= 0 || batch > 65535) return OSS_ERR_SHAPE;
+    return ln_conv1x1_wg(io, x, ln_weight, ln_bias, eps, n, mean, rstd, weight, bias, y, batch, cout, cin, pixels, xsb, xsc,
+                         reinterpret_cast<hipStream_t>(stream), fwd_image);
 }
 
 int oss_conv1x1_dgrad_ln_bwd_ok(oss_dtype io, int cout, int cin, int pixels, int batch) {
diff --git a/vmambair_amd/csrc/oss_conv1x1.hip b/vmambair_amd/csrc/oss_conv1x1.hip
--- a/vmambair_amd/csrc/oss_conv1x1.hip
+++ b/vmambair_amd/csrc/oss_conv1x1.hip
@@ -278,10 +278,11 @@
     __builtin_amdgcn_wave_barrier();
 }
 
-template <typename T, int KS, bool WT, bool WVEC, bool RES, bool PF>
+template <typename T, int KS, bool WT, bool WVEC, bool RES, bool PF, bool WIMG = false>
 __global__ void __launch_bounds__(256)
 oss_conv1x1_pair_kernel(const T *__restrict__ x, const float *__restrict__ w, const float *__restrict__ bias,
-                        T *__restrict__ y, int M, int K, int P, int64_t xsb, int xsk, int mt_per_wave, const T *__restrict__ res) {
+                        T *__restrict__ y, int M, int K, int P, int64_t xsb, int xsk, int mt_per_wave, const T *__restrict__ res,
+                        const u32x4 *__restrict__ wimg = nullptr) {
     const int lane = threadIdx.x & 63, wave = threadIdx.x >> 6;
     const int b = blockIdx.y;
     const int p0 = (blockIdx.x * 4 + wave) * 64;
@@ -301,16 +302,20 @@
     const int mt_begin = blockIdx.z * mt_per_wave, mt_end = min(mt_total, mt_begin + mt_per_wave);
     if (mt_begin >= mt_end) return;
 
-    constexpr bool WLDS = !WT && WVEC;
+    constexpr bool WLDS = !WIMG && !WT && WVEC;
     __shared__ __attribute__((aligned(16))) T wlds[WLDS ? 4 * 32 * (16 * KS + 8) : 8];
     T *myl = wlds + (WLDS ? wave * 32 * (16 * KS + 8) : 0);
     const int wf_row0 = WLDS ? (4 * lane) / K : 0, wf_k0 = WLDS ? (4 * lane) % K : 0, wf_sr = WLDS ? 256 / K : 0, wf_sk = WLDS ? 256 % K : 0;
-    WRaw<KS> wr;
+    WRaw<WIMG ? 1 : KS> wr;
+    u32x4 wq[WIMG ? KS : 1];
     float bl;
     uint32_t rw[16];
     auto issue = [&](int mt) {
         const int m0 = mt * 32;
-        if constexpr (WLDS) wflat_issue<KS>(wr, w, m0, M, K, lane);
+        if constexpr (WIMG) {
+#pragma unroll
+            for (int ks = 0; ks < KS; ++ks) wq[ks] = wimg[((size_t)mt * ksteps + min(ks, ksteps - 1)) * 64 + lane];
+        } else if constexpr (WLDS) wflat_issue<KS>(wr, w, m0, M, K, lane);
         else                wraw_issue<KS, WT, WVEC>(wr, w, m0 + col, M, K, kg);
         bl = bp[min(m0 + col, M - 1)];
         if constexpr (RES) {
@@ -337,7 +342,10 @@
     for (int mt = mt_begin; mt < mt_end; ++mt) {
         const int m0 = mt * 32;
         s16x8 af[KS];
-        if constexpr (WLDS) wflat_frags<T, KS>(wr, myl, af, m0, M, K, col, kg, wf_row0, wf_k0, wf_sr, wf_sk);
+        if constexpr (WIMG) {
+#pragma unroll
+            for (int ks = 0; ks < KS; ++ks) af[ks] = __builtin_bit_cast(s16x8, wq[ks]);
+        } else if constexpr (WLDS) wflat_frags<T, KS>(wr, myl, af, m0, M, K, col, kg, wf_row0, wf_k0, wf_sr, wf_sk);
         else                wraw_narrow<T, KS, WT, WVEC>(wr, af, m0 + col, M, K, kg);
         const float bcur = bias ? bl : 0.f;
         uint32_t rcur[16];
@@ -468,10 +476,11 @@
     pair_epilogue<T>(acca, accb, bias, res ? res + (size_t)b * M * P + (pok ? p : 0) : nullptr, yb + p, m0, kg, M, P, pok);
 }
 
-template <typename T, int KS, int MT, bool WT, bool WVEC>
+template <typename T, int KS, int MT, bool WT, bool WVEC, bool WIMG = false>
 __global__ void __launch_bounds__(256)
 oss_conv1x1_pairk_kernel(const T *__restrict__ x, const float *__restrict__ w, const float *__restrict__ bias,
-                        T *__restrict__ y, int M, int K, int P, int64_t xsb, int xsk, const T *__restrict__ res) {
+                        T *__restrict__ y, int M, int K, int P, int64_t xsb, int xsk, const T *__restrict__ res,
+                        const u32x4 *__restrict__ wimg = nullptr) {
     const int lane = threadIdx.x & 63, wave = threadIdx.x >> 6;
     const int b = blockIdx.y;
     const int p0 = (blockIdx.x * 4 + wave) * 64;
@@ -506,8 +515,15 @@
 #pragma unroll
         for (int t = 0; t < MT; ++t) {
             s16x8 af[KS];
-#pragma unroll
-            for (int ks = 0; ks < KS; ++ks) af[ks] = load_wfrag<T, WT, WVEC>(w, (mt0 + t) * 32 + col, M, K, kc + ks * 16 + kg * 8);
+            if constexpr (WIMG) {
+                const int ksteps = (K + 15) >> 4;
+                const u32x4 *wt_ = wimg + (size_t)min(mt0 + t, ((M + 31) >> 5) - 1) * ksteps * 64 + lane;
+#pragma unroll
+                for (int ks = 0; ks < KS; ++ks) af[ks] = __builtin_bit_cast(s16x8, wt_[(size_t)min((kc >> 4) + ks, ksteps - 1) * 64]);
+            } else {
+#pragma unroll
+                for (int ks = 0; ks < KS; ++ks) af[ks] = load_wfrag<T, WT, WVEC>(w, (mt0 + t) * 32 + col, M, K, kc + ks * 16 + kg * 8);
+            }
             if ((mt0 + t) * 32 < M) {
 #pragma unroll
                 for (int ks = 0; ks < KS; ++ks) {
@@ -723,7 +739,7 @@
 
 template <typename T>
 static void conv1x1_launch(const T *x, const float *w, const float *bias, T *y, int B, int M, int K, int P, int64_t xsb,
-                           int64_t xsk, int64_t ws_m, int64_t ws_k, hipStream_t s, const T *res) {
+                           int64_t xsk, int64_t ws_m, int64_t ws_k, hipStream_t s, const T *res, const void *wimg = nullptr) {
     const int pblocks = (P + 127) / 128, mt = (M + 31) / 32;
     const bool wt = (ws_m == 1 && ws_k == M);
     const bool plain = (ws_k == 1 && ws_m == K);
@@ -734,7 +750,8 @@
         const int pb = (P + 255) / 256;
         const long waves_p = (long)B * ((P + 63) / 64);
         const int xk = (int)xsk;
-        if (plain && !wvec && K > 16 * 3 && K <= 512 && (reinterpret_cast<uintptr_t>(w) & 15u) == 0) {
+        const u32x4 *img = reinterpret_cast<const u32x4 *>(wimg);
+        if (!img && plain && !wvec && K > 16 * 3 && K <= 512 && (reinterpret_cast<uintptr_t>(w) & 15u) == 0) {
             hipLaunchKernelGGL(oss_conv1x1_pairw_kernel<T>, dim3(pb, B, mt), dim3(256), 0, s, x, w, bias, y, M, K, P, xsb, xk, res);
             return;
         }
@@ -747,25 +764,36 @@
 #define OSS_PAIR2(KS_, WT_, WV_, PF_) do { if (res) hipLaunchKernelGGL((oss_conv1x1_pair_kernel<T, KS_, WT_, WV_, true, PF_>), grid, dim3(256), 0, s, x, w, bias, y, M, K, P, xsb, xk, per, res); \
                                            else     hipLaunchKernelGGL((oss_conv1x1_pair_kernel<T, KS_, WT_, WV_, false, PF_>), grid, dim3(256), 0, s, x, w, bias, y, M, K, P, xsb, xk, per, res); } while (0)
 #define OSS_PAIR(KS_, PF_) do { if (wt) OSS_PAIR2(KS_, true, false, PF_); else if (wvec) OSS_PAIR2(KS_, false, true, PF_); else OSS_PAIR2(KS_, false, false, PF_); } while (0)
-            if (K <= 16 * 3)      OSS_PAIR(3, true);
+#define OSS_PAIRI(KS_, PF_) do { if (res) hipLaunchKernelGGL((oss_conv1x1_pair_kernel<T, KS_, false, false, true, PF_, true>), grid, dim3(256), 0, s, x, w, bias, y, M, K, P, xsb, xk, per, res, img); \
+                                 else     hipLaunchKernelGGL((oss_conv1x1_pair_kernel<T, KS_, false, false, false, PF_, true>), grid, dim3(256), 0, s, x, w, bias, y, M, K, P, xsb, xk, per, res, img); } while (0)
+            if (img) {
+                if (K <= 16 * 3)      OSS_PAIRI(3, true);
+                else if (K <= 16 * 6) OSS_PAIRI(6, true);
+                else if (K <= 16 * 8) OSS_PAIRI(8, true);
+                else                  OSS_PAIRI(12, false);
+            }
+            else if (K <= 16 * 3) OSS_PAIR(3, true);
             else if (K <= 16 * 6) OSS_PAIR(6, true);
             else if (K <= 16 * 8) OSS_PAIR(8, false);
             else                  OSS_PAIR(12, false);
+#undef OSS_PAIRI
 #undef OSS_PAIR2
 #undef OSS_PAIR
-#undef OSS_PAIR1
         } else {
             int per = 3;
             while (per > 1 && waves_p * ((mt + per - 1) / per) < 4096) --per;
             if (per > mt) per = mt;
-            if (per == 1 && K <= 512 && (reinterpret_cast<uintptr_t>(w) & 15u) == 0 && plain) {
+            if (!img && per == 1 && K <= 512 && (reinterpret_cast<uintptr_t>(w) & 15u) == 0 && plain) {
                 hipLaunchKernelGGL(oss_conv1x1_pairw_kernel<T>, dim3(pb, B, mt), dim3(256), 0, s, x, w, bias, y, M, K, P, xsb, xk, res);
                 return;
             }
             dim3 grid(pb, B, (mt + per - 1) / per);
 #define OSS_PAIR1(MT_, WT_, WV_) hipLaunchKernelGGL((oss_conv1x1_pairk_kernel<T, 8, MT_, WT_, WV_>), grid, dim3(256), 0, s, x, w, bias, y, M, K, P, xsb, xk, res)
 #define OSS_PAIR(MT_) do { if (wt) OSS_PAIR1(MT_, true, false); else if (wvec) OSS_PAIR1(MT_, false, true); else OSS_PAIR1(MT_, false, false); } while (0)
-            if (per == 1) OSS_PAIR(1); else if (per == 2) OSS_PAIR(2); else OSS_PAIR(3);
+#define OSS_PAIRI(MT_) hipLaunchKernelGGL((oss_conv1x1_pairk_kernel<T, 8, MT_, false, false, true>), grid, dim3(256), 0, s, x, w, bias, y, M, K, P, xsb, xk, res, img)
+            if (img) { if (per == 1) OSS_PAIRI(1); else if (per == 2) OSS_PAIRI(2); else OSS_PAIRI(3); }
+            else if (per == 1) OSS_PAIR(1); else if (per == 2) OSS_PAIR(2); else OSS_PAIR(3);
+#undef OSS_PAIRI
 #undef OSS_PAIR
 #undef OSS_PAIR1
         }
@@ -799,11 +827,11 @@
 void conv1x1_set_wg(int on) { g_conv_wg.store(on ? 1 : 0); }
 
 int conv1x1(oss_dtype io, const void *x, const float *w, const float *bias, void *y, int B, int M, int K, int P, int64_t xsb,
-            int64_t xsk, int64_t ws_m, int64_t ws_k, hipStream_t s, const void *res, int f32_split) {
+            int64_t xsk, int64_t ws_m, int64_t ws_k, hipStream_t s, const void *res, int f32_split, const void *wimg) {
     {
         const bool wt = (ws_m == 1 && ws_k == M), plain = (ws_k == 1 && ws_m == K);
         if ((wt || plain) && g_conv_wg.load() != 0 && conv1x1_wg_ok(io, M, K, P, xsb, xsk, x, y, w, res))
-            return conv1x1_wg(io, x, w, bias, y, B, M, K, P, xsb, xsk, wt ? 1 : 0, s, res);
+            return conv1x1_wg(io, x, w, bias, y, B, M, K, P, xsb, xsk, wt ? 1 : 0, s, res, wimg);
     }
     return io_dispatch(io, [&](auto tag) {
         using T = typename decltype(tag)::type;
@@ -812,9 +840,68 @@
         if constexpr (sizeof(T) == 4) {
             return conv1x1_f32(xp, w, bias, yp, B, M, K, P, xsb, xsk, ws_m, ws_k, s, rp, f32_split);
         } else {
-            conv1x1_launch<T>(xp, w, bias, yp, B, M, K, P, xsb, xsk, ws_m, ws_k, s, rp);
+            conv1x1_launch<T>(xp, w, bias, yp, B, M, K, P, xsb, xsk, ws_m, ws_k, s, rp, wimg);
             return (int)hipGetLastError();
         }
+    });
+}
+
+struct PackRow {
+    const float *w;
+    void *img;
+    int M, K;
+    int wt;
+    int first;
+};
+constexpr int kPackPieces = 256;
+
+template <typename T>
+__global__ void __launch_bounds__(256)
+oss_conv1x1_pack_kernel(const PackRow *__restrict__ rows) {
+    const PackRow r = rows[blockIdx.x];
+    const float *w = table_ptr<const float>(&rows[blockIdx.x].w);
+    u32x4 *img = table_ptr<u32x4>(&rows[blockIdx.x].img);
+    const int ksteps = (r.K + 15) >> 4, total = ((r.M + 31) >> 5) * ksteps * 64;
+    const int q = r.first + (int)threadIdx.x;
+    if (q >= total) return;
+    const int l = q & 63, unit = q >> 6, t = unit / ksteps, s = unit - t * ksteps;
+    const int m = 32 * t + (l & 31), k0 = 16 * s + 8 * (l >> 5);
+    const bool mok = m < r.M;
+    const int mc = mok ? m : 0;
+    float v[8];
+#pragma unroll
+    for (int e = 0; e < 8; ++e) {
+        const int k = k0 + e;
+        const bool kok = k < r.K;
+        const int kc = kok ? k : r.K - 1;
+        const float wv = r.wt ? w[(size_t)kc * r.M + mc] : w[(size_t)mc * r.K + kc];
+        v[e] = (mok && kok) ? wv : 0.f;
+    }
+    img[q] = __builtin_bit_cast(u32x4, cvt8<T>(f32x4{v[0], v[1], v[2], v[3]}, f32x4{v[4], v[5], v[6], v[7]}));
+}
+
+size_t conv1x1_image_bytes(int M, int K) { return (size_t)((M + 31) / 32) * ((K + 15) / 16) * 1024; }
+size_t conv1x1_pack_row_bytes() { return sizeof(PackRow); }
+int conv1x1_pack_rows(int cout, int cin) {
+    const size_t per = (size_t)kPackPieces * 16;
+    return (int)((conv1x1_image_bytes(cout, cin) + per - 1) / per + (conv1x1_image_bytes(cin, cout) + per - 1) / per);
+}
+int conv1x1_pack_fill(void *rows, const float *w, void *fwd_img, void *dgrad_img, int cout, int cin) {
+    PackRow *out = reinterpret_cast<PackRow *>(rows);
+    int n = 0;
+    for (int dir = 0; dir < 2; ++dir) {
+        const int M = dir ? cin : cout, K = dir ? cout : cin;
+        const int total = (int)(conv1x1_image_bytes(M, K) / 16);
+        for (int first = 0; first < total; first += kPackPieces)
+            out[n++] = PackRow{w, dir ? dgrad_img : fwd_img, M, K, dir, first};
+    }
+    return n;
+}
+int conv1x1_pack(oss_dtype io, const void *table, int n_rows, hipStream_t s) {
+    return io_dispatch<IO_16>(io, [&](auto tag) {
+        hipLaunchKernelGGL(oss_conv1x1_pack_kernel<typename decltype(tag)::type>, dim3(n_rows), dim3(256), 0, s,
+                           reinterpret_cast<const PackRow *>(table));
+        return (int)hipGetLastError();
     });
 }
 
diff --git a/vmambair_amd/csrc/oss_conv1x1_wg.hip b/vmambair_amd/csrc/oss_conv1x1_wg.hip
--- a/vmambair_amd/csrc/oss_conv1x1_wg.hip
+++ b/vmambair_amd/csrc/oss_conv1x1_wg.hip
@@ -42,10 +42,11 @@
     float eps;
 };
 
-template <typename T, int KS, bool WT, int PT, bool RES, bool PF, bool LN>
+template <typename T, int KS, bool WT, int PT, bool RES, bool PF, bool LN, bool WIMG = false>
 __global__ void __launch_bounds__(256)
 oss_conv1x1_wg_kernel(const T *__restrict__ x, const float *__restrict__ w, const float *__restrict__ bias, T *__restrict__ y,
-                      int M, int P, int64_t xsb, int64_t xsk, const T *__restrict__ res, WgLnArgs<T> ln) {
+                      int M, int P, int64_t xsb, int64_t xsk, const T *__restrict__ res, WgLnArgs<T> ln,
+                      const u32x4 *__restrict__ wimg = nullptr) {
     constexpr int K = 16 * KS, NCT = PT / 32;
     constexpr int PX = PT + 32;
     constexpr bool kPairEpi = !RES && PT == 128;
@@ -59,13 +60,15 @@
     const T *xb = x + b * xsb + p0;
     const int col = lane & 31, kg = lane >> 5;
     const int mt_total = (M + 31) >> 5;
-    struct WRaw { f32x4 lo[KS], hi[KS]; float bl; };
+    struct WRaw { f32x4 lo[WIMG ? 1 : KS], hi[WIMG ? 1 : KS]; u32x4 q[WIMG ? KS : 1]; float bl; };
     auto issue = [&](int mt, WRaw &r) {
         const int mrow = min(mt * 32 + col, M - 1);
 #pragma unroll
         for (int ks = 0; ks < KS; ++ks) {
             const int k0 = ks * 16 + kg * 8;
-            if constexpr (!WT) {
+            if constexpr (WIMG) {
+                r.q[ks] = wimg[((size_t)mt * KS + ks) * 64 + lane];
+            } else if constexpr (!WT) {
                 r.lo[ks] = *reinterpret_cast<const f32x4 *>(w + (size_t)mrow * K + k0);
                 r.hi[ks] = *reinterpret_cast<const f32x4 *>(w + (size_t)mrow * K + k0 + 4);
             } else {
@@ -183,7 +186,9 @@
             for (int r = 0; r < 16; ++r) acc[ct][r] = 0.f;
 #pragma unroll
         for (int ks = 0; ks < KS; ++ks) {
-            const s16x8 af = m0 + col < M ? cvt8<T>(cur.lo[ks], cur.hi[ks]) : s16x8{0, 0, 0, 0, 0, 0, 0, 0};
+            s16x8 af;
+            if constexpr (WIMG) af = __builtin_bit_cast(s16x8, cur.q[ks]);
+            else af = m0 + col < M ? cvt8<T>(cur.lo[ks], cur.hi[ks]) : s16x8{0, 0, 0, 0, 0, 0, 0, 0};
 #pragma unroll
             for (int ct = 0; ct < NCT; ++ct) {
                 const T *bp = xs + ks * 16 * PX + ct * 32 + tr_off;
@@ -277,21 +282,23 @@
 
 template <typename T, bool WT, bool LN = false>
 static int wg_launch(const T *x, const float *w, const float *bias, T *y, int B, int M, int K, int P, int64_t xsb, int64_t xsk,
-                     const T *res, hipStream_t s, WgLnArgs<T> ln = WgLnArgs<T>{}) {
+                     const T *res, hipStream_t s, WgLnArgs<T> ln = WgLnArgs<T>{}, const void *wimg = nullptr) {
     int pt, nz;
     wg_shape(B, M, K, P, pt, nz);
     const size_t smem = wg_lds_bytes(K, pt, res != nullptr);
     dim3 grid(P / pt, B, nz);
-#define OSS_WG3(KS_, PT_, RES_)                                                                                      \
+    const u32x4 *img = reinterpret_cast<const u32x4 *>(wimg);
+#define OSS_WG3(KS_, PT_, RES_, IMG_)                                                                                \
     do {                                                                                                             \
         static LdsGate gate;                                                                                         \
-        auto kern = oss_conv1x1_wg_kernel<T, KS_, WT, PT_, RES_, (KS_ <= 6), LN>;                                        \
+        auto kern = oss_conv1x1_wg_kernel<T, KS_, WT, PT_, RES_, (KS_ <= 6), LN, IMG_>;                                  \
         if (const int e = gate.ensure(reinterpret_cast<const void *>(kern), smem)) return e;                         \
-        hipLaunchKernelGGL(kern, grid, dim3(256), smem, s, x, w, bias, y, M, P, xsb, xsk, res, ln);                      \
+        hipLaunchKernelGGL(kern, grid, dim3(256), smem, s, x, w, bias, y, M, P, xsb, xsk, res, ln, img);                 \
     } while (0)
 #define OSS_WG(KS_)                                                                                                  \
     do {                                                                                                             \
-        if (pt == 128) OSS_WG3(KS_, 128, false); else OSS_WG3(KS_, 64, false);                                       \
+        if (img) { if (pt == 128) OSS_WG3(KS_, 128, false, true); else OSS_WG3(KS_, 64, false, true); }              \
+        else     { if (pt == 128) OSS_WG3(KS_, 128, false, false); else OSS_WG3(KS_, 64, false, false); }            \
     } while (0)
     switch (K / 16) {
         case 1: OSS_WG(1); break;
@@ -309,14 +316,14 @@
 }
 
 int conv1x1_wg(oss_dtype io, const void *x, const float *w, const float *bias, void *y, int B, int M, int K, int P, int64_t xsb,
-               int64_t xsk, int wt, hipStream_t s, const void *res) {
-    if (!conv1x1_wg_ok(io, M, K, P, xsb, xsk, x, y, w, res)) return OSS_ERR_SHAPE;
+               int64_t xsk, int wt, hipStream_t s, const void *res, const void *wimg) {
+    if (!conv1x1_wg_ok(io, M, K, P, xsb, xsk, x, y, w, res) || (reinterpret_cast<uintptr_t>(wimg) & 15u)) return OSS_ERR_SHAPE;
     return io_dispatch<IO_16>(io, [&](auto tag) {
         using T = typename decltype(tag)::type;
         const T *xp = reinterpret_cast<const T *>(x), *rp = reinterpret_cast<const T *>(res);
         T *yp = reinterpret_cast<T *>(y);
-        return wt ? wg_launch<T, true>(xp, w, bias, yp, B, M, K, P, xsb, xsk, rp, s)
-                  : wg_launch<T, false>(xp, w, bias, yp, B, M, K, P, xsb, xsk, rp, s);
+        return wt ? wg_launch<T, true>(xp, w, bias, yp, B, M, K, P, xsb, xsk, rp, s, WgLnArgs<T>{}, wimg)
+                  : wg_launch<T, false>(xp, w, bias, yp, B, M, K, P, xsb, xsk, rp, s, WgLnArgs<T>{}, wimg);
     });
 }
 
@@ -562,12 +569,15 @@
 }
 
 int ln_conv1x1_wg(oss_dtype io, const void *x, const float *ln_w, const float *ln_b, float eps, void *n, float *mean, float *rstd,
-                  const float *w, const float *bias, void *y, int B, int M, int K, int P, int64_t xsb, int64_t xsk, hipStream_t s) {
-    if (!conv1x1_wg_ok(io, M, K, P, xsb, xsk, x, y, w, nullptr) || (reinterpret_cast<uintptr_t>(n) & 15u)) return OSS_ERR_SHAPE;
+                  const float *w, const float *bias, void *y, int B, int M, int K, int P, int64_t xsb, int64_t xsk, hipStream_t s,
+                  const void *wimg) {
+    if (!conv1x1_wg_ok(io, M, K, P, xsb, xsk, x, y, w, nullptr) || ((reinterpret_cast<uintptr_t>(n) | reinterpret_cast<uintptr_t>(wimg)) & 15u))
+        return OSS_ERR_SHAPE;
     return io_dispatch<IO_16>(io, [&](auto tag) {
         using T = typename decltype(tag)::type;
         WgLnArgs<T> a{ln_w, ln_b, reinterpret_cast<T *>(n), mean, rstd, eps};
-        return wg_launch<T, false, true>(reinterpret_cast<const T *>(x), w, bias, reinterpret_cast<T *>(y), B, M, K, P, xsb, xsk, nullptr, s, a);
+        return wg_launch<T, false, true>(reinterpret_cast<const T *>(x), w, bias, reinterpret_cast<T *>(y), B, M, K, P, xsb, xsk, nullptr, s, a,
+                                         wimg);
     });
 }
 
diff --git a/vmambair_amd/csrc/oss_host.h b/vmambair_amd/csrc/oss_host.h
--- a/vmambair_amd/csrc/oss_host.h
+++ b/vmambair_amd/csrc/oss_host.h
@@ -124,7 +124,8 @@
                 float add_scale = 1.f);
 int merge4(oss_dtype io, const void *out, float *y, int B, int D, int H, int W, hipStream_t s);
 int ln_conv1x1_wg(oss_dtype io, const void *x, const float *ln_w, const float *ln_b, float eps, void *n, float *mean, float *rstd,
-                  const float *w, const float *bias, void *y, int B, int M, int K, int P, int64_t xsb, int64_t xsk, hipStream_t s);
+                  const float *w, const float *bias, void *y, int B, int M, int K, int P, int64_t xsb, int64_t xsk, hipStream_t s,
+                  const void *wimg = nullptr);
 size_t conv1x1_dgrad_lnbwd_partial_floats(int B, int M, int P);
 int conv1x1_dgrad_lnbwd_ok(oss_dtype io, int M, int K, int P, int B);
 int conv1x1_dgrad_lnbwd(oss_dtype io, const void *dy, const float *w, const void *x, const float *ln_w, int with_bias, const float *mean,
@@ -135,9 +136,15 @@
 int conv1x1_wg_ok(oss_dtype io, int M, int K, int P, int64_t xsb, int64_t xsk, const void *x, const void *y, const float *w,
                   const void *res = nullptr);
 int conv1x1_wg(oss_dtype io, const void *x, const float *w, const float *bias, void *y, int B, int M, int K, int P, int64_t xsb,
-               int64_t xsk, int wt, hipStream_t s, const void *res = nullptr);
+               int64_t xsk, int wt, hipStream_t s, const void *res = nullptr, const void *wimg = nullptr);
 int conv1x1(oss_dtype io, const void *x, const float *w, const float *bias, void *y, int B, int M, int K, int P, int64_t xsb,
-            int64_t xsk, int64_t ws_m, int64_t ws_k, hipStream_t s, const void *res = nullptr, int f32_split = 0);
+            int64_t xsk, int64_t ws_m, int64_t ws_k, hipStream_t s, const void *res = nullptr, int f32_split = 0,
+            const void *wimg = nullptr );
+size_t conv1x1_image_bytes(int M, int K);
+size_t conv1x1_pack_row_bytes();
+int conv1x1_pack_rows(int cout, int cin);
+int conv1x1_pack_fill(void *rows, const float *w, void *fwd_img, void *dgrad_img, int cout, int cin);
+int conv1x1_pack(oss_dtype io, const void *table, int n_rows, hipStream_t s);
 int conv1x1_wgrad_slabs(int P);
 void conv1x1_wgrad_set_tile(int mode);
 void conv1x1_wgrad_set_span(int mult);
diff --git a/vmambair_amd/ops/pointwise.py b/vmambair_amd/ops/pointwise.py
--- a/vmambair_amd/ops/pointwise.py
+++ b/vmambair_amd/ops/pointwise.py
@@ -2,13 +2,77 @@
 
 import contextlib
 import os
-from typing import List, Optional
+from typing import Dict, List, Optional, Sequence, Tuple
 
 import torch
 
 from .. import _capi, _precision
 from ._common import (_keep_operands, _recorded_before,
                       _DT, _LIB, _check, _f32c, _fork_for_wgrad, _keep, _keep_views, _planes, _ptr)
+
+
+_PACKED: Dict[int, Tuple[int, int, torch.dtype, torch.Tensor, torch.Tensor]] = {}
+
+
+def set_packed_images(images: Dict[int, Tuple[int, int, torch.dtype, torch.Tensor, torch.Tensor]]) -> None:
+    _PACKED.clear()
+    _PACKED.update(images)
+
+
+def clear_packed_images() -> None:
+    _PACKED.clear()
+
+
+def packed_images_active() -> int:
+    return len(_PACKED)
+
+
+def _packed_image(w: torch.Tensor, dtype: torch.dtype, direction: int) -> int:
+    if not _PACKED:
+        return 0
+    ent = _PACKED.get(w.data_ptr())
+    if ent is None or ent[0] != w.shape[0] or ent[1] != w.shape[1] or ent[2] != dtype or ent[3].device != w.device:
+        return 0
+    return ent[3 + direction].data_ptr()
+
+
+class PackedConv1x1Weights:
+
+    def __init__(self, weights: Sequence[torch.Tensor], dtype: torch.dtype):
+        _check(dtype in (torch.bfloat16, torch.float16), "packed weight images are 16-bit")
+        self.weights = list(weights)
+        _check(len(self.weights) > 0, "no weights to pack")
+        lib = _capi.load()
+        self.dtype, self.device = dtype, self.weights[0].device
+        shapes, off, rows = [], 0, 0
+        for w in self.weights:
+            _check(w.is_cuda and w.dtype == torch.float32 and w.is_contiguous() and w.dim() in (2, 4) and
+                   (w.dim() == 2 or (w.shape[2] == 1 and w.shape[3] == 1)), "packed weights: contiguous fp32 (Cout, Cin[, 1, 1]) on the GPU")
+            co, ci = int(w.shape[0]), int(w.shape[1])
+            fb, db = int(lib.oss_conv1x1_fwd_image_bytes(co, ci)), int(lib.oss_conv1x1_dgrad_image_bytes(co, ci))
+            shapes.append((co, ci, off, off + fb))
+            off += fb + db
+            rows += int(lib.oss_conv1x1_pack_rows(co, ci))
+        self.buffer = torch.zeros(off, dtype=torch.uint8, device=self.device)
+        _check(self.buffer.data_ptr() % 16 == 0, "image buffer must be 16-byte aligned")
+        rb = int(lib.oss_conv1x1_pack_row_bytes())
+        host = torch.zeros(rows * rb, dtype=torch.uint8)
+        self.images: Dict[int, Tuple[int, int, torch.dtype, torch.Tensor, torch.Tensor]] = {}
+        n = 0
+        for w, (co, ci, fo, do) in zip(self.weights, shapes):
+            fimg, dimg = self.buffer[fo:do], self.buffer[do:do + int(lib.oss_conv1x1_dgrad_image_bytes(co, ci))]
+            k = int(lib.oss_conv1x1_pack_fill(host.data_ptr() + n * rb, w.data_ptr(), fimg.data_ptr(), dimg.data_ptr(), co, ci))
+            _capi.check(min(k, 0), "oss_conv1x1_pack_fill")
+            n += k
+            self.images[w.data_ptr()] = (co, ci, dtype, fimg, dimg)
+        assert n == rows
+        self.n_rows = rows
+        self.table = host.to(self.device)
+
+    def refresh(self) -> None:
+        with torch.cuda.device(self.device):
+            _capi.check(_capi.load().oss_conv1x1_pack_weights(_DT[self.dtype], self.table.data_ptr(), self.n_rows,
+                                                             torch.cuda.current_stream().cuda_stream), "oss_conv1x1_pack_weights")
 
 
 def conv1x1_fwd(x: torch.Tensor, weight: torch.Tensor, bias: Optional[torch.Tensor],
@@ -33,6 +97,12 @@
         return y
     lib = _capi.load()
     with torch.cuda.device(x.device):
+        img = _packed_image(w, x.dtype, 0)
+        if img:
+            _capi.check(lib.oss_conv1x1_fwd_packed(_DT[x.dtype], x.data_ptr(), w.data_ptr(), img, _ptr(b), _ptr(residual), y.data_ptr(), B, Cout,
+                                                   Cin, H * W, x.stride(0), x.stride(1), torch.cuda.current_stream().cuda_stream),
+                        "oss_conv1x1_fwd_packed")
+            return y
         _capi.check(lib.oss_conv1x1_fwd(_precision.io_code(x.dtype), x.data_ptr(), w.data_ptr(), _ptr(b), _ptr(residual), y.data_ptr(), B, Cout, Cin,
                                         H * W, x.stride(0), x.stride(1), torch.cuda.current_stream().cuda_stream), "oss_conv1x1_fwd")
     return y
@@ -63,8 +133,13 @@
                                               torch.cuda.current_stream().cuda_stream), "oss_conv1x1_wgrad")
             _keep(part, dw, db)
             _keep_operands(rec0, dy, x)
+        img = _packed_image(w, x.dtype, 1)
         if f32 and CONV1X1_F32_WGRAD_ONLY:
             dx = torch.nn.functional.conv_transpose2d(dy, weight.detach().float())
+        elif img:
+            _capi.check(lib.oss_conv1x1_dgrad_packed(_DT[x.dtype], dy.data_ptr(), w.data_ptr(), img, dx.data_ptr(), B, Cout, Cin, P,
+                                                     dy.stride(0), dy.stride(1), torch.cuda.current_stream().cuda_stream),
+                        "oss_conv1x1_dgrad_packed")
         else:
             _capi.check(lib.oss_conv1x1_dgrad(_precision.io_code(x.dtype), dy.data_ptr(), w.data_ptr(), dx.data_ptr(), B, Cout, Cin, P,
                                               dy.stride(0), dy.stride(1), torch.cuda.current_stream().cuda_stream), "oss_conv1x1_dgrad")
@@ -140,9 +215,10 @@
     mean = torch.empty((B, P), dtype=torch.float32, device=x.device)
     rstd = torch.empty((B, P), dtype=torch.float32, device=x.device)
     with torch.cuda.device(x.device):
-        _capi.check(_capi.load().oss_ln_conv1x1_fwd(_DT[x.dtype], x.data_ptr(), lw.data_ptr(), _ptr(lb), 1e-5, n.data_ptr(), mean.data_ptr(),
-                                                    rstd.data_ptr(), w.data_ptr(), _ptr(b), y.data_ptr(), B, Cout, Cin, P, x.stride(0),
-                                                    x.stride(1), torch.cuda.current_stream().cuda_stream), "oss_ln_conv1x1_fwd")
+        _capi.check(_capi.load().oss_ln_conv1x1_fwd_packed(_DT[x.dtype], x.data_ptr(), lw.data_ptr(), _ptr(lb), 1e-5, n.data_ptr(),
+                                                           mean.data_ptr(), rstd.data_ptr(), w.data_ptr(), _packed_image(w, x.dtype, 0) or None,
+                                                           _ptr(b), y.data_ptr(), B, Cout, Cin, P, x.stride(0), x.stride(1),
+                                                           torch.cuda.current_stream().cuda_stream), "oss_ln_conv1x1_fwd")
     return [y, n, mean, rstd]
 
 
diff --git a/vmambair_amd/train_graph.py b/vmambair_amd/train_graph.py
--- a/vmambair_amd/train_graph.py
+++ b/vmambair_amd/train_graph.py
@@ -17,7 +17,7 @@
                  fused_optimizer: bool = True, split_graphs: bool = False, overlap_wgrads: bool = False,
                  defer_finishes: bool = True, micro_streams: int = 1, weight_decay: float = 0.0,
                  clip_grad_norm: Optional[float] = None, multi_shape: bool = False, grad_buckets: int = 1,
-                 allreduce_via_host: bool = False):
+                 allreduce_via_host: bool = False, packed_weights: bool = True):
         self.net = net
         self.params = [p for p in net.parameters() if p.requires_grad]
         self.device = self.params[0].device
@@ -33,6 +33,7 @@
         self.ema_decay = ema_decay
         self.warmup = warmup
         self.shadow = {}
+        packable = []
         if shadow_weights and autocast_dtype is not None:
             mods = dict(net.named_modules())
             for name, p in net.named_parameters():
@@ -43,6 +44,8 @@
                 dense_conv = isinstance(m, torch.nn.Conv2d) and m.groups == 1
                 if dense_conv and m.kernel_size == (1, 1) and _ops.pointwise.CONV1X1_IMPL == "mfma" and owner.rsplit(".", 1)[-1] in (
                         "in_conv", "out_conv", "project_in", "project_out", "reduce_chan_level2", "reduce_chan_level3"):
+                    if leaf == "weight":
+                        packable.append(p)
                     continue
                 if dense_conv and m.kernel_size == (3, 3) and min(m.in_channels, m.out_channels) <= 4 and _ops.conv3x3.THIN_IMPL:
                     continue
@@ -52,6 +55,11 @@
                 fused_proj = getattr(m, "fused_core", False) and getattr(m, "omni", False)
                 if dense_conv or (leaf in ("x_proj_weight", "dt_projs_weight") and not fused_proj):
                     self.shadow[name] = (p, torch.empty_like(p, dtype=autocast_dtype).requires_grad_())
+        self.packed = None
+        if packed_weights and autocast_dtype in (torch.bfloat16, torch.float16):
+            packable = [p for p in packable if p.dtype == torch.float32 and p.is_contiguous()]
+            if packable:
+                self.packed = _ops.pointwise.PackedConv1x1Weights(packable, autocast_dtype)
         self._masters = [m for m, _ in self.shadow.values()]
         self._shadows = [s for _, s in self.shadow.values()]
         self._master_grads = [torch.zeros_like(m) for m in self._masters]
@@ -245,8 +253,16 @@
             _ops.flush_finishes(self.ftables[slot])
 
     def _fwd_bwd(self):
-        if self.nmicro > 1:
-            return self._fwd_bwd_micro()
+        if self.packed is None:
+            return self._fwd_bwd_micro() if self.nmicro > 1 else self._fwd_bwd_single()
+        self.packed.refresh()
+        _ops.pointwise.set_packed_images(self.packed.images)
+        try:
+            return self._fwd_bwd_micro() if self.nmicro > 1 else self._fwd_bwd_single()
+        finally:
+            _ops.pointwise.clear_packed_images()
+
+    def _fwd_bwd_single(self):
         for p in self.params:
             p.grad = None
         for s_ in self._shadows:
```

Result: faster. 251.0 images/s, median of 6 (+2.7%).
